# peterdavidfagan/mujoco_robot_environments

Measured on AMD Instinct MI355X. Metric: env steps/sec (whole node), RearrangementEnv batch=4096 at 1/2/4/8 MI355X, higher is better.
Workload: dtype f32

## Files before the change

### mujoco_robot_environments_amd/csrc/mre_api.cpp

```cpp
#include <hip/hip_runtime.h>
#include <chrono>

#include <cmath>
#include <cstdio>
#include <cstdlib>
#include <cstring>
#include <string>
#include <algorithm>
#include <vector>

#include "../../include/mre.h"
#include "mre_dev.h"
#include "mre_records.h"

using namespace mre;

extern "C" void mre_launch_step(const StepArgs* args, hipStream_t stream);
extern "C" void mre_launch_settle(const StepArgs* args, hipStream_t stream);
extern "C" void mre_launch_step_large(const StepArgs* args, hipStream_t stream);
extern "C" void mre_launch_step_newton(const StepArgs* args, hipStream_t stream);
extern "C" void mre_launch_settle_newton(const StepArgs* args, hipStream_t stream);
extern "C" void mre_launch_step_queue(const StepArgs* args, int nwaves, hipStream_t stream);
extern "C" void mre_launch_step_queue_newton(const StepArgs* args, int nwaves, hipStream_t stream);
extern "C" void mre_launch_step_queue_large(const StepArgs* args, int nwaves, hipStream_t stream);
// ... 474 lines not shown
      for (size_t left = ng; left > 0;) {
        size_t pick = ng;
        for (size_t g = 0; g < ng && pick == ng; g++)
          if (!done[g] && (e->groups[g].nout <= (a.nsteps <= 50 ? e->ring - 1 : 0) ||
                           hipEventQuery(e->groups[g].out[e->groups[g].head].ev_info) == hipSuccess)) pick = g;
        (void)hipGetLastError();
        if (pick == ng) {
          for (size_t g = 0; g < ng && pick == ng; g++) if (!done[g]) pick = g;
        }
        int rc = launch_group(e, e->groups[pick], a);
        if (rc) return rc;
        done[pick] = true; left--;
      }
      return MRE_OK;
    }
    DRAIN_PENDING(e);
  }
  hipEvent_t e0 = nullptr, e1 = nullptr;
  if (e->profiling) {
    if (e->events_used == e->events.size()) {
      hipEvent_t x, y;
      HIPCHK(hipEventCreate(&x)); HIPCHK(hipEventCreate(&y));
      e->events.emplace_back(x, y);
    }
    e0 = e->events[e->events_used].first; e1 = e->events[e->events_used].second;
    e->events_used++;
    HIPCHK(hipEventRecord(e0, e->stream));
  }
  const bool guarded = e->fallback && a.nsteps > 0 && (a.flags & F_NO_CONSTRAINTS) == 0;
  if (!guarded) {
    launch_compact(e, a, e->stream, settle);
    HIPCHK(hipGetLastError());
  } else {
    const size_t N = (size_t)e->N;
    if (e->d_large_stale) {
      HIPCHK(hipMemcpyAsync(e->d_large, e->h_large.data(), N, hipMemcpyHostToDevice, e->stream));
      HIPCHK(hipStreamSynchronize(e->stream));
      e->d_large_stale = false;
    }
    StepArgs ac = a;
    guard_args(e, ac);
    ac.want_large = 0;
    e->n_large = 0;
    for (size_t i = 0; i < N; i++) e->n_large += e->h_large[i];
    const bool run_large = e->n_large > 0;
    if (run_large) {
      HIPCHK(hipEventRecord(e->ev_fork, e->stream));
      HIPCHK(hipStreamWaitEvent(e->stream2, e->ev_fork, 0));
      StepArgs al = ac;
      al.want_large = 1;
      launch_large(e, al, e->stream2);
      HIPCHK(hipGetLastError());
      HIPCHK(hipEventRecord(e->ev_join, e->stream2));
    }
    launch_compact(e, ac, e->stream, settle);
    HIPCHK(hipGetLastError());
    if (run_large) HIPCHK(hipStreamWaitEvent(e->stream, e->ev_join, 0));
    HIPCHK(hipStreamSynchronize(e->stream));
    memcpy(e->h_info_last, e->h_launch_info, N * 16);
    int nrerun = 0;
    bool changed = false;
    for (size_t i = 0; i < N; i++) {
      const int* li = e->h_launch_info + 4 * i;
      e->h_rerun[i] = 0;
      if (li[0] < 0) continue;
      const int hw_ncon = li[1] & 0xFFFF, hw_nefc = li[2], hw_nrrow = li[3] & 0xFFFF, hw_npp = li[3] >> 16;
      if (!e->h_large[i]) {
        if (li[0] > 0) {
          e->h_rerun[i] = 1; e->h_large[i] = 1; nrerun++; changed = true; e->n_large++; e->n_promotions++;
        } else if (!e->compact_only && near_compact_caps(e, hw_ncon, hw_nefc, hw_nrrow, hw_npp)) {
          e->h_large[i] = 1; changed = true; e->n_large++; e->n_promotions++;
        }
      } else if (!e->large_only && li[0] == 0 && 8 * hw_ncon <= 5 * NCON_MAX && 8 * hw_nefc <= 5 * NEFC_MAX &&
                 8 * hw_nrrow <= 5 * compact_nrrow_max(e) && 8 * hw_npp <= 5 * NPP_MAX) {
        e->h_large[i] = 0; changed = true; e->n_large--; e->n_demotions++;
      }
    }
    if (!e->use_order) {
      int kmax = 0;
      for (size_t i = 0; i < N; i++)
        if (e->h_launch_info[4 * i] >= 0) { const int k = e->h_launch_info[4 * i + 1] >> 16; if (k > kmax) kmax = k; }
      if (kmax > 0) {
        int count[258] = {0};
        auto bucket = [&](size_t i) {
          const int k = e->h_launch_info[4 * i] < 0 ? 0 : (e->h_launch_info[4 * i + 1] >> 16);
          return (int)((long long)k * 255 / kmax);
        };
        for (size_t i = 0; i < N; i++) count[255 - bucket(i) + 1]++;
        for (int k = 1; k <= 256; k++) count[k] += count[k - 1];
        for (size_t i = 0; i < N; i++) e->h_auto_order[count[255 - bucket(i)]++] = (int)i;
        HIPCHK(hipMemcpyAsync(e->auto_order, e->h_auto_order, N * 4, hipMemcpyHostToDevice, e->stream));
        e->have_auto_order = true;
      } else {
        e->have_auto_order = false;
      }
    }
    if (nrerun > 0) {
      HIPCHK(hipMemcpyAsync(e->mask_r, e->h_rerun.data(), N, hipMemcpyHostToDevice, e->stream));
      mre_launch_restore_rows(e->mask_r, 0, e->N, e->qpos, e->sv_qpos, e->qvel, e->sv_qvel, e->qacc_ws, e->sv_qacc_ws,
                              e->qfine, e->sv_qfine, e->ctrl, e->sv_ctrl, e->nstep, e->sv_nstep, e->status,
                              e->sv_status, e->converged, e->sv_converged, nullptr, e->stream);
      StepArgs ar = a;
      ar.env_mask = e->mask_r; ar.launch_info = nullptr;
      launch_large(e, ar, e->stream);
      HIPCHK(hipGetLastError());
      e->n_reruns += nrerun;
    }
    if (changed) {
      HIPCHK(hipMemcpyAsync(e->d_large, e->h_large.data(), N, hipMemcpyHostToDevice, e->stream));
      HIPCHK(hipStreamSynchronize(e->stream));
    }
  }
  if (e1) HIPCHK(hipEventRecord(e1, e->stream));
  return MRE_OK;
}

namespace {
struct Blob {
  const unsigned char* p;
  size_t n;
  bool find(const char* name, uint32_t* code, uint32_t* count, uint64_t* off) const {
    uint32_t ne;
    memcpy(&ne, p + 8, 4);
    const unsigned char* t = p + 16;
    for (uint32_t k = 0; k < ne; k++, t += 48)
      if (strncmp((const char*)t, name, 32) == 0) {
        memcpy(code, t + 32, 4); memcpy(count, t + 36, 4); memcpy(off, t + 40, 8);
        return *off + (size_t)(*count) * (*code ? 8 : 4) <= n;
      }
    return false;
  }
  bool ints(const char* name, int* dst, int expect) const {
    uint32_t c, cnt; uint64_t off;
    if (!find(name, &c, &cnt, &off) || c != 0 || (int)cnt != expect) return false;
    memcpy(dst, p + off, 4 * (size_t)cnt);
    return true;
  }
  bool flts(const char* name, float* dst, int expect) const {
    uint32_t c, cnt; uint64_t off;
    if (!find(name, &c, &cnt, &off) || c != 1 || (int)cnt != expect) return false;
    for (uint32_t k = 0; k < cnt; k++) {
      double v;
      memcpy(&v, p + off + 8 * (size_t)k, 8);
      dst[k] = (float)v;
    }
    return true;
  }
};
}

#define RI(name, dst, n) if (!b.ints(name, (int*)(dst), n)) return fail(MRE_ERR_MODEL, std::string("model entry ") + name)
#define RF(name, dst, n) if (!b.flts(name, (float*)(dst), n)) return fail(MRE_ERR_MODEL, std::string("model entry ") + name)

static int build_model(const void* blob, size_t nbytes, DevModel& m) {
  if (nbytes < 16) return fail(MRE_ERR_MODEL, "blob too small");
  Blob b{(const unsigned char*)blob, nbytes};
  uint32_t magic;
  memcpy(&magic, b.p, 4);
  if (magic != 0x4D524542u) return fail(MRE_ERR_MODEL, "bad blob magic");
  memset(&m, 0, sizeof(m));
  int nbody, nv, nq, nM, ngeom, nsite, npair, neq, nprop, nu;
  RI("nbody", &nbody, 1); RI("nv", &nv, 1); RI("nq", &nq, 1); RI("nM", &nM, 1); RI("ngeom", &ngeom, 1);
  RI("nsite", &nsite, 1); RI("npair", &npair, 1); RI("neq", &neq, 1); RI("nprop", &nprop, 1);
  RI("nu", &nu, 1);
  if (nbody != NB || nv != NV || nq != NQ || ngeom != NG || nsite != NSITE || npair > NPAIR ||
      neq != NEQ || nprop != NPROP || nu != NU)
    return fail(MRE_ERR_MODEL, "scene dimensions differ from the compiled kernels");
  RI("body_parentid", m.body_parent, NB); RI("body_jnttype", m.body_jnttype, NB);
  RI("body_dofadr", m.body_dofadr, NB); RI("body_qposadr", m.body_qposadr, NB);
  RI("body_propid", m.body_propid, NB);
  RF("body_pos", m.body_pos, NB * 3); RF("body_quat", m.body_quat, NB * 4);
  RF("body_ipos", m.body_ipos, NB * 3); RF("body_iquat", m.body_iquat, NB * 4);
  RF("body_mass", m.body_mass, NB); RF("body_inertia", m.body_inertia, NB * 3);
  RF("body_invweight0", m.body_invweight0, NB * 2);
  RF("jnt_pos", m.jnt_pos, NB * 3); RF("jnt_axis", m.jnt_axis, NB * 3); RF("jnt_range", m.jnt_range, NB * 2);
  RF("jnt_stiffness", m.jnt_stiffness, NB); RF("jnt_springref", m.jnt_springref, NB);
  RF("jnt_solref", m.jnt_solref, NB * 2); RF("jnt_solimp", m.jnt_solimp, NB * 5);
  RI("jnt_limited", m.jnt_limited, NB);
  RI("dof_bodyid", m.dof_body, NV); RI("dof_parentid", m.dof_parent, NV); RI("dof_Madr", m.dof_Madr, NV);
  m.dof_Madr[NV] = nM;
  RF("dof_armature", m.dof_armature, NV); RF("dof_damping", m.dof_damping, NV);
  RF("dof_invweight0", m.dof_invweight0, NV); RF("qpos0", m.qpos0, NQ);
  RI("geom_type", m.geom_type, NG); RI("geom_bodyid", m.geom_body, NG); RI("geom_propid", m.geom_propid, NG);
  RF("geom_size", m.geom_size, NG * 3); RF("geom_pos", m.geom_pos, NG * 3);
  RF("geom_quat", m.geom_quat, NG * 4); RF("geom_rbound", m.geom_rbound, NG);
  {
    std::vector<int> pg(2 * npair);
    RI("pair_geom", pg.data(), 2 * npair);
    for (int k = 0; k < NPAIR; k++) { m.pair_g1[k] = -1; m.pair_g2[k] = -1; }
    for (int k = 0; k < npair; k++) { m.pair_g1[k] = pg[2 * k]; m.pair_g2[k] = pg[2 * k + 1]; }
  }
  RI("pair_single", m.pair_single, npair);
  RF("pair_friction", m.pair_friction, npair * 3); RF("pair_solref", m.pair_solref, npair * 2);
  RF("pair_solimp", m.pair_solimp, npair * 5); RF("pair_margin", m.pair_margin, npair);
  RF("pair_gap", m.pair_gap, npair);
  for (int k = 0; k < NPAIR; k++) {
    PairRec& r = m.pair_rec[k];
    memset(&r, 0, sizeof(r));
    r.g1 = m.pair_g1[k]; r.g2 = m.pair_g2[k];
    if (r.g1 < 0) { r.g2 = -1; r.b1 = r.b2 = 0; r.pid1 = r.pid2 = -1; continue; }
    if (r.g1 >= NG || r.g2 < 0 || r.g2 >= NG) return fail(MRE_ERR_MODEL, "pair table names a geom that does not exist");
    r.b1 = m.geom_body[r.g1]; r.b2 = m.geom_body[r.g2];
    r.pid1 = m.geom_propid[r.g1]; r.pid2 = m.geom_propid[r.g2];
    r.type1 = m.geom_type[r.g1]; r.single = (m.pair_single[k] & 0xFF) | (m.geom_type[r.g2] << 8);
    if (m.geom_type[r.g1] == 2 || (m.geom_type[r.g2] == 2 && m.geom_type[r.g1] != 1))
      return fail(MRE_ERR_MODEL, "cylinder pairs: only box (geom 1) - cylinder (geom 2) is implemented");
    for (int c = 0; c < 3; c++) { r.pos1[c] = m.geom_pos[r.g1][c]; r.pos2[c] = m.geom_pos[r.g2][c];
                                  r.size1[c] = m.geom_size[r.g1][c]; r.size2[c] = m.geom_size[r.g2][c]; }
    for (int c = 0; c < 4; c++) { r.quat1[c] = m.geom_quat[r.g1][c]; r.quat2[c] = m.geom_quat[r.g2][c]; }
    r.rb1 = m.geom_rbound[r.g1]; r.rb2 = m.geom_rbound[r.g2];
    r.margin = m.pair_margin[k]; r.gap = m.pair_gap[k];
  }
  RI("site_bodyid", m.site_body, NSITE); RF("site_pos", m.site_pos, NSITE * 3);
  RF("site_quat", m.site_quat, NSITE * 4);
  RI("eef_site", &m.eef_site, 1); RI("tcp_site", &m.tcp_site, 1);
  RI("eq_type", m.eq_type, NEQ); RI("eq_obj", m.eq_obj, NEQ * 2); RF("eq_data", m.eq_data, NEQ * 8);
  RF("eq_solref", m.eq_solref, NEQ * 2); RF("eq_solimp", m.eq_solimp, NEQ * 5);
  RI("ten_dof", m.ten_dof, 2); RF("ten_coef", m.ten_coef, 2);
  RI("act_dof", m.act_dof, NU); RF("act_ctrlrange", m.act_ctrlrange, NU * 2);
  RF("grip_gainprm", &m.grip_gainprm, 1); RF("grip_biasprm", m.grip_biasprm, 3);
  RF("grip_forcerange", m.grip_forcerange, 2);
  for (int a = 0; a < NU; a++) { m.act_gain[a] = 1.f; m.act_forcelimited[a] = 0; }
  { uint32_t c, cnt; uint64_t off;
    if (b.find("act_gainprm", &c, &cnt, &off)) {
      RF("act_gainprm", m.act_gain, NU); RF("act_biasprm", m.act_bias, NU * 3);
      RF("act_forcerange", m.act_forcerange, NU * 2); RI("act_forcelimited", m.act_forcelimited, NU);
    } }
  RF("opt_timestep", &m.timestep, 1); RF("opt_gravity", m.gravity, 3); RF("opt_impratio", &m.impratio, 1);
  RF("opt_tolerance", &m.tolerance, 1); RI("opt_iterations", &m.iterations, 1);
  m.solver = MRE_SOLVER_PGS;
  { uint32_t c, cnt; uint64_t off; if (b.find("opt_solver", &c, &cnt, &off)) RI("opt_solver", &m.solver, 1); }
  if (m.solver != MRE_SOLVER_PGS && m.solver != MRE_SOLVER_NEWTON) return fail(MRE_ERR_MODEL, "opt_solver must be 0 (PGS) or 2 (Newton)");
  { uint32_t c, cnt; uint64_t off; int cone = 1;
    if (b.find("opt_cone", &c, &cnt, &off)) RI("opt_cone", &cone, 1);
    if (cone != 0 && cone != 1) return fail(MRE_ERR_MODEL, "opt_cone must be 0 (pyramidal) or 1 (elliptic)");
    m.cone = cone; }
  RF("home_qpos", m.home_qpos, 7);
  float M0d[NV];
  RF("M0_diag", M0d, NV);

  for (int bb = 1; bb < NB; bb++) {
    bool ok = bb < NRB ? (m.body_jnttype[bb] == 1 && m.body_dofadr[bb] == bb - 1 && m.body_qposadr[bb] == bb - 1 &&
                          m.body_propid[bb] < 0 && m.body_parent[bb] < bb)
                       : (m.body_jnttype[bb] == 2 && m.body_dofadr[bb] == NRV + 6 * (bb - NRB) &&
                          m.body_qposadr[bb] == NRV + 7 * (bb - NRB) && m.body_propid[bb] == bb - NRB &&
                          m.body_parent[bb] == 0);
    if (!ok) return fail(MRE_ERR_MODEL, "body layout differs from the compiled kernels");
  }
  if (m.dof_Madr[NRV] != NMR) return fail(MRE_ERR_MODEL, "robot mass-matrix size differs");
  for (int a = 0; a < 7; a++)
    if (m.act_dof[a] != a) return fail(MRE_ERR_MODEL, "arm actuators must drive dofs 0..6");

  m.body_level[0] = 0;
  for (int bb = 1; bb < NB; bb++) m.body_level[bb] = m.body_level[m.body_parent[bb]] + 1;
  for (int bb = 0; bb < NB; bb++) {
    if (m.body_level[bb] > MAXCHAIN) return fail(MRE_ERR_MODEL, "tree deeper than MAXCHAIN");
    m.body_desc_mask[bb] = 0;
  }
  for (int c = 1; c < NB; c++)
    for (int a = c; a > 0; a = m.body_parent[a]) m.body_desc_mask[a] |= (1u << c);
  m.robot_mass = 0;
  for (int bb = 1; bb < NRB; bb++) {
    m.robot_mass += m.body_mass[bb];
    int chain[MAXCHAIN], n = 0;
    for (int d = m.body_dofadr[bb]; d >= 0; d = m.dof_parent[d]) {
      if (n >= MAXCHAIN) return fail(MRE_ERR_MODEL, "dof chain too long");
      chain[n++] = d;
    }
    m.chain_len[bb] = n;
    for (int k = 0; k < n; k++) m.chain_dof[bb][k] = chain[n - 1 - k];
  }
  for (int i = 0; i < NRV; i++) {
    int adr = m.dof_Madr[i];
    for (int j = i; j >= 0; j = m.dof_parent[j], adr++) { m.M_i[adr] = i; m.M_j[adr] = j; }
    if (adr != m.dof_Madr[i + 1]) return fail(MRE_ERR_MODEL, "dof_Madr inconsistent");
  }
  for (int i = 0; i < NRV; i++)
    if (m.dof_parent[i] != ROBOT_DOF_PARENT[i] || m.dof_Madr[i] != robot_dof_madr(i))
      return fail(MRE_ERR_MODEL, "robot dof tree differs from the one the kernels are unrolled for (mre_dev.h)");
  {
    int depth[NRV];
    m.sol_maxdepth = 0;
    for (int i = 0; i < NRV; i++) {
      depth[i] = m.dof_parent[i] < 0 ? 0 : depth[m.dof_parent[i]] + 1;
      m.sol_depth[i] = depth[i];
      if (depth[i] > m.sol_maxdepth) m.sol_maxdepth = depth[i];
    }
    m.sol_depth[NRV] = -1;
    for (int i = 0; i <= NRV; i++) {
      uint16_t desc[14], anc[8];
      for (auto& v : desc) v = 0xFFFF;
      for (auto& v : anc) v = 0xFFFF;
      if (i < NRV) {
        int nd = 0, na = 0;
        for (int c = NRV - 1; c > i; c--) {
          bool is_desc = false;
          for (int j = m.dof_parent[c]; j >= 0; j = m.dof_parent[j]) if (j == i) is_desc = true;
          if (!is_desc) continue;
          if (nd >= 14) return fail(MRE_ERR_MODEL, "solve table: too many descendants");
          desc[nd++] = (uint16_t)(c | ((m.dof_Madr[c] + depth[c] - depth[i]) << 8));
        }
        for (int a = m.dof_Madr[i] + 1; a < m.dof_Madr[i + 1]; a++) {
          if (na >= 8) return fail(MRE_ERR_MODEL, "solve table: too many ancestors");
          int j = i;
          for (int k = 0; k < a - m.dof_Madr[i]; k++) j = m.dof_parent[j];
          anc[na++] = (uint16_t)(j | (a << 8));
        }
      }
      for (int k = 0; k < 7; k++) m.sol_desc[i][k] = desc[2 * k] | ((uint32_t)desc[2 * k + 1] << 16);
      for (int k = 0; k < 4; k++) m.sol_anc[i][k] = anc[2 * k] | ((uint32_t)anc[2 * k + 1] << 16);
    }
  }
  for (int k = 0; k < NRV; k++) {
    int anc[MAXCHAIN + 1], n = 0;
    for (int j = m.dof_parent[k]; j >= 0; j = m.dof_parent[j]) anc[++n] = j;
    int cnt = 0;
    for (int p = 1; p <= n; p++)
      for (int q = p; q <= n; q++) {
        if (cnt >= MAXFAC) return fail(MRE_ERR_MODEL, "factor table overflow");
        m.fac_dst[k][cnt] = (uint8_t)(m.dof_Madr[anc[p]] + (q - p));
        m.fac_a[k][cnt] = (uint8_t)p;
        m.fac_b[k][cnt] = (uint8_t)q;
        cnt++;
      }
    m.fac_n[k] = cnt;
  }
  m.M0_diag_robot_sum = 0;
  for (int i = 0; i < NRV; i++) m.M0_diag_robot_sum += M0d[i];
  for (int p = 0; p < NPROP; p++) {
    m.park_pos[p][0] = 2.0f + 0.5f * p; m.park_pos[p][1] = 2.0f; m.park_pos[p][2] = -5.0f;
  }
  return MRE_OK;
}

extern "C" const char* mre_last_error(void) { return g_err.c_str(); }

static int create_buffers(mre_env* e, int num_envs, int device_id) {
  e->N = num_envs;
  e->device = device_id;
  HIPCHK(hipSetDevice(device_id));
  HIPCHK(hipStreamCreateWithFlags(&e->stream, hipStreamNonBlocking));
  const size_t N = (size_t)num_envs;
  HIPCHK(hipMalloc(&e->dM, sizeof(DevModel)));
  HIPCHK(hipMemcpy(e->dM, &e->hM, sizeof(DevModel), hipMemcpyHostToDevice));
  HIPCHK(hipMalloc(&e->qpos, N * NQP * 4)); HIPCHK(hipMalloc(&e->qvel, N * NVP * 4));
  HIPCHK(hipMalloc(&e->qacc_ws, N * NVP * 4)); HIPCHK(hipMalloc(&e->ctrl, N * NU * 4));
  HIPCHK(hipMalloc(&e->qfine, N * QFINE_ROW * 4)); HIPCHK(hipMalloc(&e->sv_qfine, N * QFINE_ROW * 4));
  HIPCHK(hipMemsetAsync(e->qfine, 0, N * QFINE_ROW * 4, e->stream));
  HIPCHK(hipMalloc(&e->nstep, N * 4)); HIPCHK(hipMalloc(&e->sv_nstep, N * 4));
  HIPCHK(hipMemsetAsync(e->nstep, 0, N * 4, e->stream));
  HIPCHK(hipMalloc(&e->nprops, N * 4)); HIPCHK(hipMalloc(&e->prop_size, N * NPROP * 3 * 4));
  HIPCHK(hipMalloc(&e->osc_target, N * 16 * 4)); HIPCHK(hipMalloc(&e->grip_closed, N));
  HIPCHK(hipMalloc(&e->converged, N)); HIPCHK(hipMalloc(&e->mask, N));
  HIPCHK(hipMalloc(&e->sites, N * 16 * 4));
  HIPCHK(hipMalloc(&e->status, N * 4)); HIPCHK(hipMalloc(&e->stats, N * 4 * 4));
  HIPCHK(hipMalloc(&e->order, N * 4)); HIPCHK(hipMalloc(&e->auto_order, N * 4));
  HIPCHK(hipHostMalloc((void**)&e->h_auto_order, N * 4, hipHostMallocDefault));
  HIPCHK(hipStreamCreateWithFlags(&e->stream2, hipStreamNonBlocking));
  HIPCHK(hipEventCreateWithFlags(&e->ev_fork, hipEventDisableTiming));
  HIPCHK(hipEventCreateWithFlags(&e->ev_join, hipEventDisableTiming));
  HIPCHK(hipMalloc(&e->d_large, N)); HIPCHK(hipMalloc(&e->mask_r, N));
  HIPCHK(hipMalloc(&e->sv_qpos, N * NQP * 4)); HIPCHK(hipMalloc(&e->sv_qvel, N * NVP * 4));
  HIPCHK(hipMalloc(&e->sv_qacc_ws, N * NVP * 4)); HIPCHK(hipMalloc(&e->sv_ctrl, N * NU * 4));
  HIPCHK(hipMalloc(&e->sv_status, N * 4));
  HIPCHK(hipMalloc(&e->sv_converged, N));
  HIPCHK(hipHostMalloc((void**)&e->h_launch_info, mre_env::RING * N * 16, hipHostMallocMapped | hipHostMallocCoherent));
  HIPCHK(hipHostGetDevicePointer((void**)&e->d_launch_info, e->h_launch_info, 0));
  memset(e->h_launch_info, 0xFF, mre_env::RING * N * 16);
  HIPCHK(hipHostMalloc((void**)&e->h_info_last, N * 16, hipHostMallocDefault));
  memset(e->h_info_last, 0xFF, N * 16);
  HIPCHK(hipHostMalloc((void**)&e->h_large_stage, mre_env::NSTAGE * N, hipHostMallocMapped | hipHostMallocCoherent));
  HIPCHK(hipHostGetDevicePointer((void**)&e->d_large_stage, e->h_large_stage, 0));
  memset(e->h_large_stage, 0, mre_env::NSTAGE * N);
  HIPCHK(hipMalloc(&e->d_pending, N));
  HIPCHK(hipMemsetAsync(e->d_pending, 0, N, e->stream));
  HIPCHK(hipMemsetAsync(e->d_large, 0, N, e->stream));
  e->h_large.assign(N, 0); e->h_rerun.assign(N, 0);
  {
    int ng = 4, min_envs = 512;
    if (const char* g = getenv("MRE_GROUPS")) ng = atoi(g);
    if (const char* g = getenv("MRE_GROUP_MIN")) min_envs = atoi(g);
    if (ng < 1) ng = 1;
    if (ng > 8) ng = 8;
    if (const char* r = getenv("MRE_RING")) { e->ring = atoi(r); if (e->ring < 2) e->ring = 2; if (e->ring > mre_env::RING) e->ring = mre_env::RING; }
    while (ng > 1 && num_envs < min_envs * ng) ng--;
    HIPCHK(hipHostMalloc((void**)&e->h_grp_order, mre_env::NSTAGE * N * 4, hipHostMallocMapped | hipHostMallocCoherent));
    HIPCHK(hipHostGetDevicePointer((void**)&e->d_grp_order, e->h_grp_order, 0));
    for (int k = 0; k < mre_env::NSTAGE; k++)
      for (int i = 0; i < num_envs; i++) e->h_grp_order[(size_t)k * N + i] = i;
    HIPCHK(hipEventCreateWithFlags(&e->ev_main, hipEventDisableTiming));
    e->groups.resize(ng);
    {
      auto& Q = e->qgroup;
      Q.lo = 0; Q.n = num_envs;
      HIPCHK(hipHostMalloc((void**)&e->h_qgrp_order, mre_env::NSTAGE * N * 4, hipHostMallocMapped | hipHostMallocCoherent));
      Q.h_order = e->h_qgrp_order;
      HIPCHK(hipHostGetDevicePointer((void**)&Q.d_order, Q.h_order, 0));
      for (int k = 0; k < mre_env::NSTAGE; k++)
        for (int i = 0; i < num_envs; i++) Q.h_order[(size_t)k * N + i] = i;
      {
        int least = 0, greatest = 0;
        HIPCHK(hipDeviceGetStreamPriorityRange(&least, &greatest));
        HIPCHK(hipStreamCreateWithPriority(&Q.st, hipStreamNonBlocking, least));
        HIPCHK(hipStreamCreateWithPriority(&Q.st2, hipStreamNonBlocking, greatest));
      }
      HIPCHK(hipEventCreateWithFlags(&Q.ev_fork, hipEventDisableTiming));
      HIPCHK(hipEventCreateWithFlags(&Q.ev_join, hipEventDisableTiming));
      for (auto& o : Q.out) HIPCHK(hipEventCreateWithFlags(&o.ev_info, hipEventDisableTiming));
      if (const char* q = getenv("MRE_QUEUE")) e->queue_ok = atoi(q) != 0;
      if (const char* q = getenv("MRE_QUEUE_TICKS")) { const int v = atoi(q); if (v >= 2 && v <= QUEUE_TICKS_MAX) e->queue_ticks = v; }
      if (e->queue_run_ticks > e->queue_ticks) e->queue_run_ticks = e->queue_ticks;
      hipDeviceProp_t prop;
      HIPCHK(hipGetDeviceProperties(&prop, e->device));
      {
        const int a_ = mre_queue_waves_per_cu(), b_ = mre_queue_waves_per_cu_newton();
        e->queue_waves = prop.multiProcessorCount * (a_ < b_ ? a_ : b_);
      }
      if (const char* q = getenv("MRE_QUEUE_WAVES")) { const int v = atoi(q); if (v > 0) e->queue_waves = v; }
      if (const char* q = getenv("MRE_QUEUE_SHARDS")) { const int v = atoi(q); if (v >= 1 && v <= QUEUE_SHARDS_MAX) e->queue_shards = v; }
      if (const char* q = getenv("MRE_QUEUE_MIN_TICKS")) { const int v = atoi(q); if (v >= 2) e->queue_min_ticks = v; }
      if (const char* q = getenv("MRE_QUEUE_TAIL_MIN")) { const float v = (float)atof(q); if (v > 0.f) e->queue_tail_min = v; }
      if (const char* q = getenv("MRE_QUEUE_TEST_SERIAL")) e->queue_test_serial = atoi(q) != 0;
      if (const char* q = getenv("MRE_QUEUE_SPARE_LARGE")) { const int v = atoi(q); if (v >= 0) e->queue_spare_large = v; }
      e->queue_large_waves_max = 2 * prop.multiProcessorCount;
      if (const char* q = getenv("MRE_QUEUE_LSHARDS")) { const int v = atoi(q); if (v >= 1 && v <= QUEUE_LSHARDS_MAX) e->queue_lshards = v; }
      HIPCHK(hipMalloc(&e->q_ws, ((2 * (size_t)(QUEUE_SHARDS_MAX + QUEUE_LSHARDS_MAX) * QUEUE_TICKS_MAX + 16 + 4 * N +
                                   (size_t)QUEUE_TICKS_MAX * (2 * N + QUEUE_SHARDS_MAX + QUEUE_LSHARDS_MAX)) * 4 + 15) / 16 * 16));
      HIPCHK(hipMalloc(&e->q_gen, 64));
      HIPCHK(hipMemsetAsync(e->q_gen, 0, 64, e->stream));
      HIPCHK(hipHostMalloc((void**)&e->h_qlist, (size_t)(mre_env::RING + 1) * (N + 32) * 4, hipHostMallocDefault));
      HIPCHK(hipHostMalloc((void**)&e->h_q_err, 64, hipHostMallocMapped | hipHostMallocCoherent));
      *e->h_q_err = 0;
    }
    for (int g = 0; g < ng; g++) {
      auto& G = e->groups[g];
      G.h_order = e->h_grp_order; G.d_order = e->d_grp_order;
      G.lo = (int)((long long)num_envs * g / ng);
      G.n = (int)((long long)num_envs * (g + 1) / ng) - G.lo;
      int pr = 0;
      {
        int least = 0, greatest = 0;
        HIPCHK(hipDeviceGetStreamPriorityRange(&least, &greatest));
        const char* gp = getenv("MRE_GROUP_PRIORITY");
        if (!(gp && atoi(gp) == 0)) { pr = greatest + g; if (pr > least) pr = least; }
        if (const char* map = getenv("MRE_GROUP_PRIO_MAP")) {
          if ((int)strlen(map) > g && map[g] >= '0' && map[g] <= '9') { pr = greatest + (map[g] - '0'); if (pr > least) pr = least; }
        }
      }
      HIPCHK(hipStreamCreateWithPriority(&G.st, hipStreamNonBlocking, pr));
      HIPCHK(hipStreamCreateWithPriority(&G.st2, hipStreamNonBlocking, pr));
      HIPCHK(hipEventCreateWithFlags(&G.ev_fork, hipEventDisableTiming));
      HIPCHK(hipEventCreateWithFlags(&G.ev_join, hipEventDisableTiming));
      for (auto& o : G.out) HIPCHK(hipEventCreateWithFlags(&o.ev_info, hipEventDisableTiming));
    }
  }
  if (const char* fb = getenv("MRE_NO_FALLBACK")) e->fallback = atoi(fb) == 0;
  if (const char* fl = getenv("MRE_FORCE_LARGE")) {
    if (atoi(fl) != 0) {
      e->h_large.assign(N, 1); e->n_large = num_envs;
      HIPCHK(hipMemsetAsync(e->d_large, 1, N, e->stream));
    }
  }
  HIPCHK(hipMemsetAsync(e->status, 0, N * 4, e->stream)); HIPCHK(hipMemsetAsync(e->stats, 0, N * 16, e->stream));
  HIPCHK(hipMemsetAsync(e->grip_closed, 0, N, e->stream)); HIPCHK(hipMemsetAsync(e->osc_target, 0, N * 64, e->stream));
  HIPCHK(hipMemsetAsync(e->sites, 0, N * 64, e->stream));
  std::vector<int> np(N, NPROP);
  std::vector<float> ps(N * NPROP * 3, 0.0155f);
  HIPCHK(hipMemcpy(e->nprops, np.data(), N * 4, hipMemcpyHostToDevice));
  HIPCHK(hipMemcpy(e->prop_size, ps.data(), ps.size() * 4, hipMemcpyHostToDevice));
  e->osc = OscConfig{350.f, 20.f, 500.f, 100.f, 200.f, 30.f, {0.f, -0.785f, 0.f, -2.356f, 0.f, 1.571f, 0.785f},
                     5e-3f, 68e-3f, 0};
  HIPCHK(hipMalloc(&e->d_osc, sizeof(OscConfig)));
  HIPCHK(hipMemcpy(e->d_osc, &e->osc, sizeof(OscConfig), hipMemcpyHostToDevice));
  HIPCHK(hipStreamSynchronize(e->stream));
  int rc = mre_reset(e, nullptr);
  if (rc != MRE_OK) return rc;
  return mre_sync(e);
}

extern "C" int mre_create(const void* blob, size_t nbytes, int num_envs, int device_id, mre_env** out) {
  if (!blob || !out || num_envs <= 0) return fail(MRE_ERR_ARG, "mre_create: bad argument");
  *out = nullptr;
  mre_env* e = new mre_env();
  int rc = build_model(blob, nbytes, e->hM);
  if (rc != MRE_OK) { delete e; return rc; }
// ... 1087 lines not shown
```

### mujoco_robot_environments_amd/csrc/mre_dev.h

```cpp
#pragma once
#include <stdint.h>

namespace mre {

constexpr int NB = 20;
constexpr int NRB = 16;
constexpr int GRIP_BODY0 = 8;
constexpr int NV = 39;
constexpr int NRV = 15;
constexpr int NQ = 43;
constexpr int NQP = 44;
constexpr int TRACE_W = 88;
constexpr int TRACE_QVEL = 48;
constexpr int NVP = 40;
constexpr int NU = 8;
constexpr int QFINE = 32;
constexpr int QFINE_ROW = 96;
constexpr int QFINE_CUBE_Q = 32;
constexpr int QFINE_CUBE_V = 60;
static_assert(QFINE_CUBE_Q + 7 * 4 == QFINE_CUBE_V && QFINE_CUBE_V + 6 * 4 <= QFINE_ROW, "qfine row layout");
constexpr int NPROP = 4;
constexpr int NG = 20;
constexpr int PROP_GEOM0 = 12;
constexpr int NPAIR = 128;
constexpr int NMR = 96;
constexpr int NSITE = 2;
constexpr int NEQ = 3;
constexpr int CONTACT_EXPORT = 32;
constexpr int MAXCHAIN = 9;
constexpr int MAXFAC = 45;
constexpr int ROBOT_DOF_PARENT[NRV] = {-1, 0, 1, 2, 3, 4, 5, 6, 7, 6, 9, 6, 11, 6, 13};
constexpr int robot_dof_depth(int i) { return ROBOT_DOF_PARENT[i] < 0 ? 0 : 1 + robot_dof_depth(ROBOT_DOF_PARENT[i]); }
constexpr int robot_dof_madr(int i) { return i == 0 ? 0 : robot_dof_madr(i - 1) + robot_dof_depth(i - 1) + 1; }
constexpr int robot_dof_anc(int i, int k) {
  int j = ROBOT_DOF_PARENT[i];
  for (int t = 0; t < k && j >= 0; t++) j = ROBOT_DOF_PARENT[j];
  return j;
}
static_assert(robot_dof_madr(NRV) == NMR, "robot mass-matrix size");

#if defined(MRE_LARGE_CAPS) && defined(MRE_NEWTON)
constexpr int NCON_MAX = 48;
constexpr int NEFC_MAX = 160;
constexpr int NRROW_MAX = 100;
constexpr int NPP_MAX = 16;
constexpr int MAXBLK = 58;
#elif defined(MRE_LARGE_CAPS)
constexpr int NCON_MAX = 44;
constexpr int NEFC_MAX = 148;
constexpr int NRROW_MAX = 83;
constexpr int NPP_MAX = 16;
constexpr int MAXBLK = 52;
#elif defined(MRE_NEWTON)
constexpr int NCON_MAX = 32;
constexpr int NEFC_MAX = 112;
constexpr int NRROW_MAX = 69;
constexpr int NPP_MAX = 8;
constexpr int MAXBLK = 40;
#else
constexpr int NCON_MAX = 32;
constexpr int NEFC_MAX = 112;
constexpr int NRROW_MAX = 62;
constexpr int NPP_MAX = 8;
constexpr int MAXBLK = 40;
#endif
constexpr int NRROW_MAX_COMPACT_PGS = 62, NRROW_MAX_COMPACT_NEWTON = 69;
#if !defined(MRE_LARGE_CAPS)
static_assert(NRROW_MAX ==
#ifdef MRE_NEWTON
              NRROW_MAX_COMPACT_NEWTON,
#else
              NRROW_MAX_COMPACT_PGS,
#endif
              "host-side copy of the compact robot-row capacity");
#endif
static_assert(NEFC_MAX <= 256 && NRROW_MAX < 127 && NPP_MAX <= 16 && MAXBLK >= 8 + NCON_MAX,
              "capacities must fit the block descriptor fields (mre_solver.h)");

struct alignas(16) PairRec {
  int g1, g2, b1, b2;
  int pid1, pid2, type1, single;
  float pos1[3], rb1;
  float pos2[3], rb2;
  float quat1[4], quat2[4];
  float size1[3], margin;
  float size2[3], gap;
};
static_assert(sizeof(PairRec) == 128, "PairRec is eight 16-byte words");

struct DevModel {
  int body_parent[NB], body_level[NB], body_jnttype[NB], body_dofadr[NB], body_qposadr[NB];
  int body_propid[NB];
  unsigned body_desc_mask[NB];
  int chain_len[NB];
  int chain_dof[NB][MAXCHAIN];
  float body_pos[NB][3], body_quat[NB][4], body_ipos[NB][3], body_iquat[NB][4];
  float body_mass[NB], body_inertia[NB][3], body_invweight0[NB][2];
  float jnt_pos[NB][3], jnt_axis[NB][3], jnt_range[NB][2], jnt_stiffness[NB], jnt_springref[NB];
  float jnt_solref[NB][2], jnt_solimp[NB][5];
  int jnt_limited[NB];
  int dof_body[NV], dof_parent[NV], dof_Madr[NV + 1];
  float dof_armature[NV], dof_damping[NV], dof_invweight0[NV], qpos0[NQP];
  int M_i[NMR], M_j[NMR];
  int fac_n[NRV];
  uint8_t fac_dst[NRV][MAXFAC], fac_a[NRV][MAXFAC], fac_b[NRV][MAXFAC];
  int sol_depth[NRV + 1], sol_maxdepth;
  uint32_t sol_desc[NRV + 1][7], sol_anc[NRV + 1][4];
  float robot_mass;
  float M0_diag_robot_sum;
  int geom_type[NG], geom_body[NG], geom_propid[NG];
  float geom_size[NG][3], geom_pos[NG][3], geom_quat[NG][4], geom_rbound[NG];
  int pair_g1[NPAIR], pair_g2[NPAIR], pair_single[NPAIR];
  float pair_friction[NPAIR][3], pair_solref[NPAIR][2], pair_solimp[NPAIR][5];
  float pair_margin[NPAIR], pair_gap[NPAIR];
  PairRec pair_rec[NPAIR];
  int site_body[NSITE];
  float site_pos[NSITE][3], site_quat[NSITE][4];
  int eef_site, tcp_site;
  int eq_type[NEQ], eq_obj[NEQ][2];
  float eq_data[NEQ][8], eq_solref[NEQ][2], eq_solimp[NEQ][5];
  int ten_dof[2];
  float ten_coef[2];
  int act_dof[NU];
  float act_ctrlrange[NU][2], grip_gainprm, grip_biasprm[3], grip_forcerange[2];
  float act_gain[NU], act_bias[NU][3], act_forcerange[NU][2];
  int act_forcelimited[NU];
  float timestep, gravity[3], impratio, tolerance;
  int iterations;
  int solver;
  int cone;
  float home_qpos[7];
  float park_pos[NPROP][3];
};

struct OscConfig {
  float kp_pos, kd_pos, kp_ori, kd_ori, kp_null, kd_null;
  float null_q[7];
  float pos_thresh, ori_thresh;
  int pinv_always;
};

enum StepFlags : unsigned { F_NO_CONSTRAINTS = 1u, F_FREEZE_ROBOT = 2u, F_CONV_CONTINUE = 4u, F_CONV_OPEN = 8u,
                            F_OSC_EVAL = 16u, F_DETECT = 32u, F_SETTLE_EXIT = 64u };
enum CtrlMode : int { CTRL_HELD = 0, CTRL_SEQ = 1, CTRL_OSC = 2 };

struct StepArgs {
  const DevModel* M;
  int N;
  float* qpos;
  float* qvel;
  float* qacc_ws;
  float* qfine;
  float* ctrl;
  const float* ctrl_seq;
  int seq_stride;
  const int* nprops;
  const float* prop_size;
  int nsteps, control_steps, mode;
  unsigned flags;
  const OscConfig* osc;
  int osc_stride;
  const float* osc_target;
  const uint8_t* grip_closed;
  uint8_t* converged;
  float* sites;
  uint32_t* status;
  int* nstep;
  int* stats;
  float* trace;
  int trace_nenv, trace_max, trace_base;
  const uint8_t* env_mask;
  const int* env_order;
  float* geoms;
  float* contacts;
  int* settle_steps;
  int min_settle_steps;
  const uint8_t* large;
  int want_large;
  float *sv_qpos, *sv_qvel, *sv_qacc_ws, *sv_qfine, *sv_ctrl;
  int* sv_nstep;
  uint32_t* sv_status;
  uint8_t* sv_converged;
  int* launch_info;
  uint8_t* pending;
  int* q_head;
  int* q_tail;
  int* q_buf;
  int* q_acc;
  int* q_done;
  int* q_started;
  const int* q_gen;
  int q_gen_expect;
  int q_wait;
  int* q_err;
  int q_nticks, q_shards, q_cap, q_stride;
  int q_lshards, q_capl;
};
constexpr int QUEUE_TICKS_MAX = 256;
constexpr int QUEUE_SHARDS_MAX = 32;
constexpr int QUEUE_LSHARDS_MAX = 16;

struct SearchArgs {
  const DevModel* M;
  int N;
  float* qpos;
  const int* nprops;
  const float* prop_size;
  const uint8_t* env_mask;
  const long long* env_ids;
  long long env_id_offset;
  unsigned long long seed;
  const int* prop;
  int fixed_prop;
  const double* bounds;
  double shared_bounds[6];
  const int* tick_base;
  long long tick0;
  int max_attempts;
  int yaw_mode;
  double fixed_quat[4];
  float max_dist;
  int commit;
  float* qfine;
  double* pose;
  int* attempts;
};

struct SortArgs {
  const DevModel* M;
  int N;
  const float* qpos;
  const int* nprops;
  const double* zones;
  double place_z;
  int* which;
  double* pick;
  double* bounds;
};

struct RenderArgs {
  int N, height, width;
  const float* geoms;
  const int* nprops;
  const uint8_t* prop_rgb;
  float geom_rgb[NG][3];
  float cam_pos[3], cam_mat[9];
  float fy;
  float light_pos[3];
  float ambient, head_diffuse, light_diffuse;
  float checker[2][3], checker_size;
  float zfar;
  uint8_t* rgb;
  float* depth;
  uint8_t* seg;
  const uint8_t* env_mask;
  int g0, g1;
  const float* bg_depth;
  const uint8_t* bg_rgb;
  const uint8_t* bg_seg;
};

}
```

### mujoco_robot_environments_amd/csrc/mre_kernels.hip

```cpp
#include <hip/hip_runtime.h>

#include "mre_dev.h"
#include "mre_math.h"
#include "mre_collide.h"

namespace mre {
using ModelP = MRE_MODEL_PTR(DevModel);
#if defined(MRE_PHASE_STAMPS) && MRE_PHASE_STAMPS >= 4
__shared__ unsigned long long dbg_acc[4];
#endif

struct OscSm {
  float J[6][7], M[7][7], MiJt[7][6], Li[6][6], Lam[6][6], V[6][6], Jbar[7][6];
  float ep[3], eo[3], F[6], LF[6], tn[7], Jbt[6], xd[6], w[6];
};

struct alignas(8) Blk {
  uint16_t row0;
  uint8_t type, nrows;
  uint8_t rslot;
  uint8_t pa, pb;
  uint8_t primary : 4;
  uint8_t bslot : 4;
};

constexpr int TAB_BYTES = 8 * (MAXBLK * 5 + 1) + 4 * 48;
constexpr int FRAME_BYTES = (int)sizeof(OscSm) > 4 * (NB * 16) ? (int)sizeof(OscSm) : 4 * (NB * 16);
constexpr int R1_MIN = TAB_BYTES - FRAME_BYTES > 0 ? TAB_BYTES - FRAME_BYTES : 4;
constexpr int MD_LD = 17;

struct Sm {
  float qpos[NQP], qvel[NVP], qlo[QFINE], ctrl[NU];
  float qfrc_smooth[NVP], qacc_smooth[NVP], qacc[NVP], qfrc_bias[NVP], qfrc_con[NVP];
  union {
    struct { float xpos[NB][3], xquat[NB][4], xmat[NB][9]; };
    OscSm osc;
#ifdef MRE_NEWTON
    struct { float nw_Ma[NVP], nw_grad[NVP], nw_search[NVP], nw_Mv[NVP]; };
#endif
  };
#ifndef MRE_NEWTON
  char tab_room[R1_MIN];
#endif
  float cdof[NRV][6];
  union {
    struct { float con_pos[NCON_MAX][3], con_frame[NCON_MAX][9], con_dist[NCON_MAX]; };
#ifdef MRE_NEWTON
    struct { float jar[NEFC_MAX], frc[NEFC_MAX], jv[NEFC_MAX]; };
#else
    struct { float jar[NEFC_MAX], frc[NEFC_MAX], pyr_f[4 * NCON_MAX]; };
#endif
  };
  float com_robot[3];
  float site_xpos[NSITE][3], site_xmat[1][9];
#ifdef MRE_NEWTON
  float qM[NMR];
#else
  float qM[NMR], qLD[NMR], qLDinv[NRV + 1];
#endif
  float prop_mass[NPROP], prop_inertia[NPROP][3], prop_size[NPROP][3];
  union { float scratch[64]; int iscr[64]; };
  float osc_tgt[16];
  int nprops;
  int ncon, nefc, nl, nrrow, npp, overflow, solver_iters;
  int finger_contact;
  uint8_t con_pair[NCON_MAX], con_rslot[NCON_MAX], con_bslot[NCON_MAX], con_b1[NCON_MAX], con_b2[NCON_MAX];
  uint16_t lim_info[NRV + 1];
  union {
    float JpA[3 * NCON_MAX][6];
    struct {
      float cinert[NB][10], crb[NRB][10], gP[NRB - GRIP_BODY0][6], gC[NRB - GRIP_BODY0][6];
      double gpose[NRB - GRIP_BODY0][7];
    };
  };
  float JpB[3 * NPP_MAX][6];
  union {
    float Jr[NRROW_MAX][NRV];
    struct {
      float cdof_dot[NV][6], cvel[NB][6], cfrc[NB][6];
      alignas(8) double gI[NRB - GRIP_BODY0][10];
      double gS[NRB - GRIP_BODY0][6];
    };
  };
#ifdef MRE_NEWTON
  float efc_R[NEFC_MAX], efc_aref[NEFC_MAX];
  float frc_r[NRROW_MAX];
  float con_fric[NCON_MAX];
  float hc[NCON_MAX][6];
  float Md[NRV][MD_LD];
  alignas(8) float W[NV * (NV + 1) / 2];
  uint8_t rstate[NEFC_MAX];
  uint8_t clist[NPROP][NCON_MAX];
  uint8_t ccount[NPROP], cpl_robot, cpl_cubes;
  alignas(8) uint16_t jdesc[NEFC_MAX][4];
  float zrow[24];
#else
  float Br[NRROW_MAX][NRV];
  alignas(16) float blkrec[MAXBLK][16];
  Blk blk[MAXBLK];
  uint8_t sched[MAXBLK][8];
#endif
  uint16_t hdr[NEFC_MAX];

  int nblk, nsched;
};

#if defined(MRE_LARGE_CAPS)
static_assert(sizeof(Sm) <= 27136, "large-capacity Sm must fit 6 workgroups per CU");
#else
static_assert(sizeof(Sm) <= 20480, "compact Sm must fit 8 workgroups per CU");
#endif

#ifdef MRE_NEWTON
MRE_DEV float* mh_store(Sm& s) { return &s.JpA[0][0]; }
static_assert(sizeof(((Sm*)0)->JpA) >= sizeof(float) * NMR, "M - h dF/dv fits the head of the constraint block");
#else
MRE_DEV float* mh_store(Sm& s) { return s.qLD; }
#endif

struct BodyRegs {
  float anchor[3], axis[3], xipos[3], ximat[9];
};

MRE_DEV double robot_q(const Sm& s, int d) { return (double)s.qpos[d] + (double)s.qlo[d]; }
MRE_DEV double robot_v(const Sm& s, int d) { return (double)s.qvel[d] + (double)s.qlo[QFINE / 2 + d]; }

MRE_DEV bool body_is_active(ModelP M, const Sm& s, int b) {
  int p = M->body_propid[b];
  return p < 0 || p < s.nprops;
}

MRE_DEV void sincos_poly_d(double x, double& sn, double& cs) {
  const double z = x * x;
  double ps = -1.0 / 1307674368000.0;
  ps = ps * z + 1.0 / 6227020800.0;
  ps = ps * z - 1.0 / 39916800.0;
  ps = ps * z + 1.0 / 362880.0;
  ps = ps * z - 1.0 / 5040.0;
  ps = ps * z + 1.0 / 120.0;
  ps = ps * z - 1.0 / 6.0;
  sn = x + x * (z * ps);
  double pc = 1.0 / 20922789888000.0;
  pc = pc * z - 1.0 / 87178291200.0;
  pc = pc * z + 1.0 / 479001600.0;
  pc = pc * z - 1.0 / 3628800.0;
  pc = pc * z + 1.0 / 40320.0;
  pc = pc * z - 1.0 / 720.0;
  pc = pc * z + 1.0 / 24.0;
  pc = pc * z - 0.5;
  cs = 1.0 + z * pc;
}
MRE_DEV void dq_mul(double* r, const double* a, const double* b) {
  const double w = a[0] * b[0] - a[1] * b[1] - a[2] * b[2] - a[3] * b[3];
  const double x = a[0] * b[1] + a[1] * b[0] + a[2] * b[3] - a[3] * b[2];
  const double y = a[0] * b[2] - a[1] * b[3] + a[2] * b[0] + a[3] * b[1];
  const double z = a[0] * b[3] + a[1] * b[2] - a[2] * b[1] + a[3] * b[0];
  r[0] = w; r[1] = x; r[2] = y; r[3] = z;
}
MRE_DEV void dq_rot(double* r, const double* q, const double* v) {
  const double ux = q[1], uy = q[2], uz = q[3], w = q[0];
  const double cx = uy * v[2] - uz * v[1], cy = uz * v[0] - ux * v[2], cz = ux * v[1] - uy * v[0];
  const double dx = uy * cz - uz * cy, dy = uz * cx - ux * cz, dz = ux * cy - uy * cx;
  r[0] = v[0] + 2.0 * (w * cx + dx); r[1] = v[1] + 2.0 * (w * cy + dy); r[2] = v[2] + 2.0 * (w * cz + dz);
}
MRE_DEV void hinge_local_d(ModelP M, const Sm& s, int b, double* p, double* q) {
  double q0[4], ql[4], ax[3], jp[3], t0[3], t1[3];
  for (int k = 0; k < 4; k++) q0[k] = (double)M->body_quat[b][k];
  for (int k = 0; k < 3; k++) { ax[k] = (double)M->jnt_axis[b][k]; jp[k] = (double)M->jnt_pos[b][k]; }
  const int qa = M->body_qposadr[b];
  double s4, c4;
  sincos_poly_d(0.25 * (robot_q(s, qa) - (double)M->qpos0[qa]), s4, c4);
  const double sn = 2.0 * s4 * c4, cs = 1.0 - 2.0 * s4 * s4;
  ql[0] = cs; ql[1] = ax[0] * sn; ql[2] = ax[1] * sn; ql[3] = ax[2] * sn;
  dq_mul(q, q0, ql);
  const double n = rsq64(q[0] * q[0] + q[1] * q[1] + q[2] * q[2] + q[3] * q[3]);
  for (int k = 0; k < 4; k++) q[k] *= n;
  dq_rot(t0, q0, jp);
  dq_rot(t1, q, jp);
  for (int k = 0; k < 3; k++) p[k] = (double)M->body_pos[b][k] + t0[k] - t1[k];
}
template <int CTRL>
MRE_DEV double dpp_row_d(double v, double fill) {
  const long long b = __builtin_bit_cast(long long, v), f = __builtin_bit_cast(long long, fill);
  const int lo = __builtin_amdgcn_update_dpp((int)(f & 0xFFFFFFFFll), (int)(b & 0xFFFFFFFFll), CTRL, 0xF, 0xF, false);
  const int hi = __builtin_amdgcn_update_dpp((int)(f >> 32), (int)(b >> 32), CTRL, 0xF, 0xF, false);
  return __builtin_bit_cast(double, ((long long)hi << 32) | (long long)(unsigned)lo);
}
MRE_DEV double readlane_d(double v, int lane) {
  const long long b = __builtin_bit_cast(long long, v);
  const int lo = __builtin_amdgcn_readlane((int)(b & 0xFFFFFFFFll), lane), hi = __builtin_amdgcn_readlane((int)(b >> 32), lane);
  return __builtin_bit_cast(double, ((long long)hi << 32) | (long long)(unsigned)lo);
}
MRE_DEV void dq2mat(double* m, const double* q) {
  const double w = q[0], x = q[1], y = q[2], z = q[3];
  m[0] = w * w + x * x - y * y - z * z; m[1] = 2 * (x * y - w * z); m[2] = 2 * (x * z + w * y);
  m[3] = 2 * (x * y + w * z); m[4] = w * w - x * x + y * y - z * z; m[5] = 2 * (y * z - w * x);
  m[6] = 2 * (x * z - w * y); m[7] = 2 * (y * z + w * x); m[8] = w * w - x * x - y * y + z * z;
}
MRE_DEV double dpp_shr1_d(double v) {
  const long long b = __builtin_bit_cast(long long, v);
  const int lo = __builtin_amdgcn_update_dpp(0, (int)(b & 0xFFFFFFFFll), 0x111, 0xF, 0xF, false);
  const int hi = __builtin_amdgcn_update_dpp(0, (int)(b >> 32), 0x111, 0xF, 0xF, false);
  return __builtin_bit_cast(double, ((long long)hi << 32) | (long long)(unsigned)lo);
}
MRE_DEV double dpp_shl1_d(double v) {
  const long long b = __builtin_bit_cast(long long, v);
  const int lo = __builtin_amdgcn_update_dpp(0, (int)(b & 0xFFFFFFFFll), 0x101, 0xF, 0xF, false);
  const int hi = __builtin_amdgcn_update_dpp(0, (int)(b >> 32), 0x101, 0xF, 0xF, false);
  return __builtin_bit_cast(double, ((long long)hi << 32) | (long long)(unsigned)lo);
}

struct Frame { float p[3], q[4], m[9]; };

MRE_DEV float dpp_shr(float v, float fill, int sh) {
  int r;
  const int vi = __builtin_bit_cast(int, v), fi = __builtin_bit_cast(int, fill);
  if (sh == 1) r = __builtin_amdgcn_update_dpp(fi, vi, 0x111, 0xF, 0xF, false);
  else if (sh == 2) r = __builtin_amdgcn_update_dpp(fi, vi, 0x112, 0xF, 0xF, false);
  else r = __builtin_amdgcn_update_dpp(fi, vi, 0x114, 0xF, 0xF, false);
  return __builtin_bit_cast(float, r);
}
template <int CTRL>
MRE_DEV void chain_step_d(double (&q)[4], double (&p)[3]) {
  double aq[4], ap[3], nq[4], t[3];
  aq[0] = dpp_row_d<CTRL>(q[0], 1.0);
#pragma unroll
  for (int c = 1; c < 4; c++) aq[c] = dpp_row_d<CTRL>(q[c], 0.0);
#pragma unroll
  for (int c = 0; c < 3; c++) ap[c] = dpp_row_d<CTRL>(p[c], 0.0);
  dq_mul(nq, aq, q);
  dq_rot(t, aq, p);
#pragma unroll
  for (int c = 0; c < 4; c++) q[c] = nq[c];
#pragma unroll
  for (int c = 0; c < 3; c++) p[c] = ap[c] + t[c];
}
template <bool WRITEBACK>
MRE_DEV void kinematics(ModelP M, Sm& s, int l, BodyRegs& br) {
  constexpr int LINK7 = GRIP_BODY0 - 1;
  const bool arm = l >= 1 && l <= LINK7, fin = l >= GRIP_BODY0 && l < NRB;
  double q[4] = {1.0, 0.0, 0.0, 0.0}, p[3] = {0.0, 0.0, 0.0};
  if (arm || fin) hinge_local_d(M, s, l, p, q);
  {
    double pp[3], pq[4];
#pragma unroll
    for (int k = 0; k < 3; k++) pp[k] = dpp_shr1_d(p[k]);
#pragma unroll
    for (int k = 0; k < 4; k++) pq[k] = dpp_shr1_d(q[k]);
    if (fin) {
      if (M->body_parent[l] >= GRIP_BODY0) {
        double t[3], q2[4];
        dq_rot(t, pq, p);
#pragma unroll
        for (int k = 0; k < 3; k++) p[k] = pp[k] + t[k];
        dq_mul(q2, pq, q);
#pragma unroll
        for (int k = 0; k < 4; k++) q[k] = q2[k];
      }
#pragma unroll
      for (int k = 0; k < 3; k++) s.gpose[l - GRIP_BODY0][k] = p[k];
#pragma unroll
      for (int k = 0; k < 4; k++) s.gpose[l - GRIP_BODY0][3 + k] = q[k];
    }
  }
  double wq[4], wp[3];
#pragma unroll
  for (int k = 0; k < 4; k++) wq[k] = arm ? q[k] : (k == 0 ? 1.0 : 0.0);
#pragma unroll
  for (int k = 0; k < 3; k++) wp[k] = arm ? p[k] : 0.0;
  chain_step_d<0x111>(wq, wp);
  chain_step_d<0x112>(wq, wp);
  chain_step_d<0x114>(wq, wp);
  {
    double q7[4], p7[3];
#pragma unroll
    for (int k = 0; k < 4; k++) q7[k] = readlane_d(wq[k], LINK7);
#pragma unroll
    for (int k = 0; k < 3; k++) p7[k] = readlane_d(wp[k], LINK7);
    if (fin) {
      double t[3];
      dq_rot(t, q7, p);
      dq_mul(wq, q7, q);
#pragma unroll
      for (int k = 0; k < 3; k++) wp[k] = p7[k] + t[k];
    }
  }
  Frame mine;
  v3zero(br.anchor); v3zero(br.axis);
  v3zero(br.xipos);
  const int b = l < NB ? l : 0;
  if (arm || fin) {
    const double n = rsq64(wq[0] * wq[0] + wq[1] * wq[1] + wq[2] * wq[2] + wq[3] * wq[3]);
#pragma unroll
    for (int k = 0; k < 4; k++) wq[k] *= n;
    double Rm[9], t[3], qi[4];
    dq2mat(Rm, wq);
#pragma unroll
    for (int k = 0; k < 4; k++) mine.q[k] = (float)wq[k];
#pragma unroll
    for (int k = 0; k < 3; k++) mine.p[k] = (float)wp[k];
#pragma unroll
    for (int k = 0; k < 9; k++) mine.m[k] = (float)Rm[k];
    const double jp[3] = {(double)M->jnt_pos[b][0], (double)M->jnt_pos[b][1], (double)M->jnt_pos[b][2]};
    const double ax[3] = {(double)M->jnt_axis[b][0], (double)M->jnt_axis[b][1], (double)M->jnt_axis[b][2]};
    const double ip[3] = {(double)M->body_ipos[b][0], (double)M->body_ipos[b][1], (double)M->body_ipos[b][2]};
    const double iq[4] = {(double)M->body_iquat[b][0], (double)M->body_iquat[b][1], (double)M->body_iquat[b][2], (double)M->body_iquat[b][3]};
#pragma unroll
    for (int r = 0; r < 3; r++) {
      br.anchor[r] = (float)(wp[r] + Rm[3 * r] * jp[0] + Rm[3 * r + 1] * jp[1] + Rm[3 * r + 2] * jp[2]);
      br.axis[r] = (float)(Rm[3 * r] * ax[0] + Rm[3 * r + 1] * ax[1] + Rm[3 * r + 2] * ax[2]);
      br.xipos[r] = (float)(wp[r] + Rm[3 * r] * ip[0] + Rm[3 * r + 1] * ip[1] + Rm[3 * r + 2] * ip[2]);
    }
    dq_mul(qi, wq, iq);
    dq2mat(Rm, qi);
#pragma unroll
    for (int k = 0; k < 9; k++) br.ximat[k] = (float)Rm[k];
    (void)t;
  }
  if (l >= NRB && l < NB) {
    const int qa = M->body_qposadr[b];
    v3copy(mine.p, &s.qpos[qa]);
    for (int k = 0; k < 4; k++) mine.q[k] = s.qpos[qa + 3 + k];
    const float n2 = mine.q[0] * mine.q[0] + mine.q[1] * mine.q[1] + mine.q[2] * mine.q[2] + mine.q[3] * mine.q[3];
    qnormalize(mine.q);
    if (WRITEBACK && fabsf(n2 - 1.f) > 1e-5f) for (int k = 0; k < 4; k++) s.qpos[qa + 3 + k] = mine.q[k];
    q2mat(mine.m, mine.q);
    v3copy(br.anchor, mine.p);
    br.axis[0] = 0.f; br.axis[1] = 0.f; br.axis[2] = 1.f;
  }
  if (l == 0) {
    v3zero(mine.p);
    mine.q[0] = 1.f; mine.q[1] = mine.q[2] = mine.q[3] = 0.f;
    q2mat(mine.m, mine.q);
    q2mat(br.ximat, mine.q);
  }
  if (l < NB) {
    v3copy(s.xpos[b], mine.p);
    for (int k = 0; k < 4; k++) s.xquat[b][k] = mine.q[k];
    for (int k = 0; k < 9; k++) s.xmat[b][k] = mine.m[k];
    if (l >= NRB) {
      float tmp[3], qi[4];
      m3mulv(tmp, mine.m, M->body_ipos[b]);
      v3add(br.xipos, mine.p, tmp);
      qmul(qi, mine.q, M->body_iquat[b]);
      q2mat(br.ximat, qi);
    }
  }
  MRE_SYNC();
  if (l < NSITE) {
    const int b = M->site_body[l];
    float tmp[3], q[4];
    m3mulv(tmp, s.xmat[b], M->site_pos[l]);
    v3add(s.site_xpos[l], s.xpos[b], tmp);
    qmul(q, s.xquat[b], M->site_quat[l]);
    if (l == M->eef_site) q2mat(s.site_xmat[0], q);
  }
}

MRE_DEV void com_pos(ModelP M, Sm& s, int l, const BodyRegs& br) {
  const bool robot = (l >= 1 && l < NRB);
  float mass = 0.f;
  if (l < NB) mass = (M->body_propid[l] >= 0) ? s.prop_mass[M->body_propid[l]] : M->body_mass[l];
  float c0 = robot ? mass * br.xipos[0] : 0.f;
  float c1 = robot ? mass * br.xipos[1] : 0.f;
  float c2 = robot ? mass * br.xipos[2] : 0.f;
  wave_sum3(c0, c1, c2);
  const float inv = 1.0f / M->robot_mass;
  float com[3] = {c0 * inv, c1 * inv, c2 * inv};
  if (l == 0) v3copy(s.com_robot, com);
  if (l >= 1 && l < NB) {
    const int b = l, pid = M->body_propid[b];
    if (pid >= 0) v3copy(com, br.xipos);
    float inertia[3];
    if (pid >= 0) v3copy(inertia, s.prop_inertia[pid]); else v3copy(inertia, M->body_inertia[b]);
    float dif[3], tmp[9];
    v3sub(dif, br.xipos, com);
    const float* mat = br.ximat;
#pragma unroll
    for (int r = 0; r < 3; r++)
#pragma unroll
      for (int c = 0; c < 3; c++)
        tmp[3 * r + c] = mat[3 * r] * inertia[0] * mat[3 * c] + mat[3 * r + 1] * inertia[1] * mat[3 * c + 1] +
                         mat[3 * r + 2] * inertia[2] * mat[3 * c + 2];
    float* ci = s.cinert[b];
    ci[0] = tmp[0] + mass * (dif[1] * dif[1] + dif[2] * dif[2]);
    ci[1] = tmp[4] + mass * (dif[0] * dif[0] + dif[2] * dif[2]);
    ci[2] = tmp[8] + mass * (dif[0] * dif[0] + dif[1] * dif[1]);
    ci[3] = tmp[1] - mass * dif[0] * dif[1];
    ci[4] = tmp[2] - mass * dif[0] * dif[2];
    ci[5] = tmp[5] - mass * dif[1] * dif[2];
    ci[6] = mass * dif[0]; ci[7] = mass * dif[1]; ci[8] = mass * dif[2]; ci[9] = mass;
    const int da = M->body_dofadr[b];
    float off[3];
    v3sub(off, com, br.anchor);
    if (pid < 0) {
      v3copy(s.cdof[da], br.axis);
      v3cross(s.cdof[da] + 3, br.axis, off);
    }
  }
  if (l == 0) for (int k = 0; k < 10; k++) s.cinert[0][k] = 0.f;
}

MRE_PHASE_FN void position_stage(ModelP M, Sm& s, int l) {
  MRE_DBG_T0();
  BodyRegs br;
  kinematics<true>(M, s, l, br);
  MRE_DBG_STAMP(5, 0);
  com_pos(M, s, l, br);
  MRE_SYNC();
  MRE_DBG_STAMP(5, 1);
}
MRE_PHASE_FN void kinematics_only(ModelP M, Sm& s, int l) {
  BodyRegs br;
  kinematics<false>(M, s, l, br);
  MRE_SYNC();
}

MRE_DEV void prop_cdof(const Sm& s, int b, int j, float* c) {
  c[0] = c[1] = c[2] = c[3] = c[4] = c[5] = 0.f;
  if (j < 3) {
    c[3 + j] = 1.f;
  } else {
    const int k = j - 3;
    c[0] = s.xmat[b][k]; c[1] = s.xmat[b][3 + k]; c[2] = s.xmat[b][6 + k];
  }
}

MRE_DEV void inert_about_d(ModelP M, int c, const double* p, const double* q, const double* O, double* ci) {
  double ip[3] = {(double)M->body_ipos[c][0], (double)M->body_ipos[c][1], (double)M->body_ipos[c][2]}, t[3], qi[4];
  double iq[4] = {(double)M->body_iquat[c][0], (double)M->body_iquat[c][1], (double)M->body_iquat[c][2], (double)M->body_iquat[c][3]};
  dq_rot(t, q, ip);
  const double d[3] = {p[0] + t[0] - O[0], p[1] + t[1] - O[1], p[2] + t[2] - O[2]};
  dq_mul(qi, q, iq);
  double R[9];
  {
    const double w = qi[0], x = qi[1], y = qi[2], z = qi[3];
    R[0] = w * w + x * x - y * y - z * z; R[1] = 2 * (x * y - w * z); R[2] = 2 * (x * z + w * y);
    R[3] = 2 * (x * y + w * z); R[4] = w * w - x * x + y * y - z * z; R[5] = 2 * (y * z - w * x);
    R[6] = 2 * (x * z - w * y); R[7] = 2 * (y * z + w * x); R[8] = w * w - x * x - y * y + z * z;
  }
  const double m = (double)M->body_mass[c];
  const double in[3] = {(double)M->body_inertia[c][0], (double)M->body_inertia[c][1], (double)M->body_inertia[c][2]};
  double T[9];
  for (int r = 0; r < 3; r++)
    for (int k = 0; k < 3; k++)
      T[3 * r + k] = R[3 * r] * in[0] * R[3 * k] + R[3 * r + 1] * in[1] * R[3 * k + 1] + R[3 * r + 2] * in[2] * R[3 * k + 2];
  ci[0] += T[0] + m * (d[1] * d[1] + d[2] * d[2]);
  ci[1] += T[4] + m * (d[0] * d[0] + d[2] * d[2]);
  ci[2] += T[8] + m * (d[0] * d[0] + d[1] * d[1]);
  ci[3] += T[1] - m * d[0] * d[1];
  ci[4] += T[2] - m * d[0] * d[2];
  ci[5] += T[5] - m * d[1] * d[2];
  ci[6] += m * d[0]; ci[7] += m * d[1]; ci[8] += m * d[2]; ci[9] += m;
}

MRE_PHASE_FN void gripper_local(ModelP M, Sm& s, int l) {
  const bool fin = l >= GRIP_BODY0 && l < NRB;
  const int b = fin ? l : GRIP_BODY0;
  const double* pose = s.gpose[b - GRIP_BODY0];
  const double p[3] = {pose[0], pose[1], pose[2]}, q[4] = {pose[3], pose[4], pose[5], pose[6]};
  const int ts = M->tcp_site;
  const double O[3] = {(double)M->site_pos[ts][0], (double)M->site_pos[ts][1], (double)M->site_pos[ts][2]};
  double ci[10] = {0, 0, 0, 0, 0, 0, 0, 0, 0, 0};
  if (fin) inert_about_d(M, b, p, q, O, ci);
  double up[10];
#pragma unroll
  for (int k = 0; k < 10; k++) up[k] = dpp_shl1_d(ci[k]);
  if (fin) {
#pragma unroll
    for (int k = 0; k < 10; k++) s.gI[b - GRIP_BODY0][k] = ci[k];
    if (M->body_parent[b] < GRIP_BODY0 && b + 1 < NRB && M->body_parent[b + 1] == b) {
#pragma unroll
      for (int k = 0; k < 10; k++) ci[k] += up[k];
    }
    double ax[3] = {(double)M->jnt_axis[b][0], (double)M->jnt_axis[b][1], (double)M->jnt_axis[b][2]};
    double jp[3] = {(double)M->jnt_pos[b][0], (double)M->jnt_pos[b][1], (double)M->jnt_pos[b][2]};
    double u[3], a[3];
    dq_rot(u, q, ax);
    dq_rot(a, q, jp);
    const double r[3] = {O[0] - p[0] - a[0], O[1] - p[1] - a[1], O[2] - p[2] - a[2]};
    const double cd[6] = {u[0], u[1], u[2], u[1] * r[2] - u[2] * r[1], u[2] * r[0] - u[0] * r[2], u[0] * r[1] - u[1] * r[0]};
    double P[6];
    P[0] = ci[0] * cd[0] + ci[3] * cd[1] + ci[4] * cd[2] - ci[8] * cd[4] + ci[7] * cd[5];
    P[1] = ci[3] * cd[0] + ci[1] * cd[1] + ci[5] * cd[2] + ci[8] * cd[3] - ci[6] * cd[5];
    P[2] = ci[4] * cd[0] + ci[5] * cd[1] + ci[2] * cd[2] - ci[7] * cd[3] + ci[6] * cd[4];
    P[3] = ci[8] * cd[1] - ci[7] * cd[2] + ci[9] * cd[3];
    P[4] = ci[6] * cd[2] - ci[8] * cd[0] + ci[9] * cd[4];
    P[5] = ci[7] * cd[0] - ci[6] * cd[1] + ci[9] * cd[5];
    for (int k = 0; k < 6; k++) { s.gC[b - GRIP_BODY0][k] = (float)cd[k]; s.gP[b - GRIP_BODY0][k] = (float)P[k]; s.gS[b - GRIP_BODY0][k] = cd[k]; }
  }
  MRE_SYNC();
}

MRE_DEV void connect_side_d(ModelP M, const Sm& s, int b, const float* a, double sign, double* x,
                            double (*vec)[3]) {
  const double* pose = s.gpose[b - GRIP_BODY0];
  const double al[3] = {(double)a[0], (double)a[1], (double)a[2]};
  double t[3];
  dq_rot(t, pose + 3, al);
  for (int k = 0; k < 3; k++) x[k] = pose[k] + t[k];
  const int par = M->body_parent[b];
  for (int m = 0; m < 2; m++) {
    vec[m][0] = vec[m][1] = vec[m][2] = 0.0;
    const int c = m == 0 ? b : par;
    if (c < GRIP_BODY0) break;
    const double* cp = s.gpose[c - GRIP_BODY0];
    const double ax[3] = {(double)M->jnt_axis[c][0], (double)M->jnt_axis[c][1], (double)M->jnt_axis[c][2]};
    const double jp[3] = {(double)M->jnt_pos[c][0], (double)M->jnt_pos[c][1], (double)M->jnt_pos[c][2]};
    double u[3], ja[3];
    dq_rot(u, cp + 3, ax);
    dq_rot(ja, cp + 3, jp);
    const double r[3] = {x[0] - cp[0] - ja[0], x[1] - cp[1] - ja[1], x[2] - cp[2] - ja[2]};
    vec[m][0] = sign * (u[1] * r[2] - u[2] * r[1]);
    vec[m][1] = sign * (u[2] * r[0] - u[0] * r[2]);
    vec[m][2] = sign * (u[0] * r[1] - u[1] * r[0]);
  }
}

MRE_PHASE_FN void connect_rows_local(ModelP M, Sm& s, int l) {
  if (l < 2 && M->eq_type[l] == 0) {
    double x1[3], x2[3], v1[2][3], v2[2][3];
    connect_side_d(M, s, M->eq_obj[l][0], M->eq_data[l], 1.0, x1, v1);
    connect_side_d(M, s, M->eq_obj[l][1], M->eq_data[l] + 3, -1.0, x2, v2);
    float* o = &s.qfrc_con[16 * l];
    for (int k = 0; k < 3; k++) {
      o[k] = (float)(x1[k] - x2[k]);
      o[4 + k] = (float)v1[0][k]; o[7 + k] = (float)v1[1][k];
      o[10 + k] = (float)v2[0][k]; o[13 + k] = (float)v2[1][k];
    }
  }
  MRE_SYNC();
}

constexpr bool robot_tree_is_chain_plus_two_body_fingers() {
  for (int d = 0; d < NRV; d++) {
    const int b = d + 1;
    const int want = b < GRIP_BODY0 ? d - 1 : ((b & 1) ? d - 1 : GRIP_BODY0 - 2);
    if (ROBOT_DOF_PARENT[d] != want) return false;
  }
  return true;
}
static_assert(GRIP_BODY0 % 2 == 0 && NRB == 16 && robot_tree_is_chain_plus_two_body_fingers(),
              "tree_prefix / tree_suffix / the prefix kinematics are written for this body tree");
template <int CTRL>
MRE_DEV float dpp_row(float v) {
  return __builtin_bit_cast(float, __builtin_amdgcn_update_dpp(0, __builtin_bit_cast(int, v), CTRL, 0xF, 0xF, false));
}
template <int N>
MRE_DEV void tree_prefix(float (&x)[N], int l) {
  constexpr int LINK7 = GRIP_BODY0 - 1;
  float own[N], par[N];
#pragma unroll
  for (int c = 0; c < N; c++) { own[c] = x[c]; par[c] = dpp_row<0x111>(x[c]); }
#pragma unroll
  for (int c = 0; c < N; c++) x[c] += dpp_row<0x111>(x[c]);
#pragma unroll
  for (int c = 0; c < N; c++) x[c] += dpp_row<0x112>(x[c]);
#pragma unroll
  for (int c = 0; c < N; c++) x[c] += dpp_row<0x114>(x[c]);
  const bool finger = l >= GRIP_BODY0 && l < NRB, leaf = (l & 1) != 0;
#pragma unroll
  for (int c = 0; c < N; c++) {
    const float p7 = __builtin_bit_cast(float, __builtin_amdgcn_readlane(__builtin_bit_cast(int, x[c]), LINK7));
    x[c] = finger ? (p7 + (leaf ? par[c] : 0.f)) + own[c] : x[c];
  }
}
template <int N>
MRE_DEV void tree_suffix(float (&x)[N], int l) {
  float own[N], nxt[N];
#pragma unroll
  for (int c = 0; c < N; c++) { own[c] = x[c]; nxt[c] = dpp_row<0x101>(x[c]); }
#pragma unroll
  for (int c = 0; c < N; c++) x[c] += dpp_row<0x101>(x[c]);
#pragma unroll
  for (int c = 0; c < N; c++) x[c] += dpp_row<0x102>(x[c]);
#pragma unroll
  for (int c = 0; c < N; c++) x[c] += dpp_row<0x104>(x[c]);
#pragma unroll
  for (int c = 0; c < N; c++) x[c] += dpp_row<0x108>(x[c]);
  const bool finger = l >= GRIP_BODY0 && l < NRB, leaf = (l & 1) != 0;
#pragma unroll
  for (int c = 0; c < N; c++) x[c] = finger ? (leaf ? own[c] : own[c] + nxt[c]) : x[c];
}

MRE_DEV void crb_mass_matrix(ModelP M, Sm& s, int l) {
  {
    float acc[10];
#pragma unroll
    for (int k = 0; k < 10; k++) acc[k] = (l >= 1 && l < NRB) ? s.cinert[l][k] : 0.f;
    tree_suffix(acc, l);
    if (l >= 1 && l < NRB) {
#pragma unroll
      for (int k = 0; k < 10; k++) s.crb[l][k] = acc[k];
    }
  }
  MRE_SYNC();
  for (int e = l; e < NMR; e += 64) {
    const int i = M->M_i[e], j = M->M_j[e];
    float v;
    if (i >= GRIP_BODY0 - 1) {
      const int root = GRIP_BODY0 - 1;
      float cj[6];
      if (j >= GRIP_BODY0 - 1) {
        for (int k = 0; k < 6; k++) cj[k] = s.gC[j - (GRIP_BODY0 - 1)][k];
      } else {
        float off[3], t[3], lin[3];
        v3sub(off, s.site_xpos[M->tcp_site], s.com_robot);
        v3cross(t, s.cdof[j], off);
        v3add(lin, s.cdof[j] + 3, t);
        m3tmulv(cj, s.xmat[root], s.cdof[j]);
        m3tmulv(cj + 3, s.xmat[root], lin);
      }
      v = dot6(cj, s.gP[i - (GRIP_BODY0 - 1)]);
    } else {
      float buf[6];
      mul_inert_vec(buf, s.crb[M->dof_body[i]], s.cdof[i]);
      v = dot6(s.cdof[j], buf);
    }
    if (i == j) v += M->dof_armature[i];
    s.qM[e] = v;
  }
}

typedef const __attribute__((address_space(3))) float* lds_cfloat_p;
template <int I, int K, class F>
MRE_DEV void solve_regs_back(float (&x)[NRV], const F& LD, float xi) {
  constexpr int j = robot_dof_anc(I, K);
  if constexpr (j >= 0) {
    constexpr int adr = robot_dof_madr(I) + 1 + K;
    x[j] -= LD[adr] * xi;
    solve_regs_back<I, K + 1, F>(x, LD, xi);
  }
}
template <int I, class F>
MRE_DEV void solve_regs_back_rows(float (&x)[NRV], const F& LD) {
  solve_regs_back<I, 0, F>(x, LD, x[I]);
  __builtin_amdgcn_sched_barrier(0);
  if constexpr (I > 0) solve_regs_back_rows<I - 1, F>(x, LD);
}
template <int I, int K, class F>
MRE_DEV void solve_regs_fwd(float (&x)[NRV], const F& LD, float& xi) {
  constexpr int j = robot_dof_anc(I, K);
  if constexpr (j >= 0) {
    constexpr int adr = robot_dof_madr(I) + 1 + K;
    xi -= LD[adr] * x[j];
    solve_regs_fwd<I, K + 1, F>(x, LD, xi);
  }
}
template <int I, class F>
MRE_DEV void solve_regs_fwd_rows(float (&x)[NRV], const F& LD) {
  float xi = x[I];
  solve_regs_fwd<I, 0, F>(x, LD, xi);
  x[I] = xi;
  __builtin_amdgcn_sched_barrier(0);
  if constexpr (I + 1 < NRV) solve_regs_fwd_rows<I + 1, F>(x, LD);
}
MRE_DEV void solve_robot_regs(const float* LD_, const float* dinv_, float (&x)[NRV]) {
  lds_cfloat_p LD = (lds_cfloat_p)LD_;
  lds_cfloat_p dinv = (lds_cfloat_p)dinv_;
  asm volatile("" : "+v"(LD), "+v"(dinv));
  solve_regs_back_rows<NRV - 1, lds_cfloat_p>(x, LD);
#pragma unroll
  for (int i = 0; i < NRV; i++) x[i] *= dinv[i];
  solve_regs_fwd_rows<0, lds_cfloat_p>(x, LD);
}

typedef __attribute__((address_space(3))) float* lds_float_p;
template <int K, int P, int Q>
MRE_DEV void factor_regs_upd(float (&A)[NMR], float tmp) {
  if constexpr (Q <= robot_dof_depth(K)) {
    constexpr int i = robot_dof_anc(K, P - 1);
    constexpr int dst = robot_dof_madr(i) + (Q - P), src = robot_dof_madr(K) + Q;
    A[dst] -= tmp * A[src];
    factor_regs_upd<K, P, Q + 1>(A, tmp);
  }
}
template <int K, int P>
MRE_DEV void factor_regs_anc(float (&A)[NMR], float inv) {
  if constexpr (P <= robot_dof_depth(K)) {
    constexpr int kp = robot_dof_madr(K) + P;
    const float tmp = A[kp] * inv;
    factor_regs_upd<K, P, P>(A, tmp);
    A[kp] = tmp;
    factor_regs_anc<K, P + 1>(A, inv);
  }
}
template <int K, class D>
MRE_DEV void factor_regs_rows(float (&A)[NMR], D& dinv) {
  constexpr int kk = robot_dof_madr(K);
  const float inv = 1.0f / A[kk];
  dinv[K] = inv;
  factor_regs_anc<K, 1>(A, inv);
  if constexpr (K > 0) factor_regs_rows<K - 1, D>(A, dinv);
}
MRE_DEV void factor_robot_regs(const float* src_, float* LD_, float* dinv_) {
  lds_cfloat_p src = (lds_cfloat_p)src_;
  lds_float_p LD = (lds_float_p)LD_, dinv = (lds_float_p)dinv_;
  asm volatile("" : "+v"(src), "+v"(LD), "+v"(dinv));
  float A[NMR];
#pragma unroll
  for (int e = 0; e < NMR; e++) A[e] = src[e];
  factor_regs_rows<NRV - 1, lds_float_p>(A, dinv);
#pragma unroll
  for (int e = 0; e < NMR; e++) LD[e] = A[e];
  MRE_SYNC();
}

MRE_DEV void solve_robot_one(const float* LD, const float* dinv, float* xv, int l) {
  float x[NRV];
#pragma unroll
  for (int i = 0; i < NRV; i++) x[i] = xv[i];
  solve_robot_regs(LD, dinv, x);
  MRE_SYNC();
  float mine = 0.f;
#pragma unroll
  for (int i = 0; i < NRV; i++) mine = (l == i) ? x[i] : mine;
  if (l < NRV) xv[l] = mine;
  MRE_SYNC();
}

MRE_DEV void factor_solve_robot(const float* src_, float* xv, int l) {
  lds_cfloat_p src = (lds_cfloat_p)src_;
  asm volatile("" : "+v"(src));
  float A[NMR], dv[NRV], x[NRV];
#pragma unroll
  for (int e = 0; e < NMR; e++) A[e] = src[e];
#pragma unroll
  for (int i = 0; i < NRV; i++) x[i] = xv[i];
  factor_regs_rows<NRV - 1, float[NRV]>(A, dv);
  solve_regs_back_rows<NRV - 1, float[NMR]>(x, A);
#pragma unroll
  for (int i = 0; i < NRV; i++) x[i] *= dv[i];
  solve_regs_fwd_rows<0, float[NMR]>(x, A);
  MRE_SYNC();
  float mine = 0.f;
#pragma unroll
  for (int i = 0; i < NRV; i++) mine = (l == i) ? x[i] : mine;
  if (l < NRV) xv[l] = mine;
  MRE_SYNC();
}

}
#include "mre_solver.h"
#ifdef MRE_NEWTON
#include "mre_newton.h"
#endif
#include "mre_osc.h"
namespace mre {

MRE_PHASE_FN void velocity_stage(ModelP M, Sm& s, int l) {
  constexpr int LINK7 = GRIP_BODY0 - 1;
  const bool rob = l >= 1 && l < NRB;
  float cd[6] = {0.f, 0.f, 0.f, 0.f, 0.f, 0.f}, qv = 0.f;
  if (rob) {
#pragma unroll
    for (int t = 0; t < 6; t++) cd[t] = s.cdof[l - 1][t];
    qv = s.qvel[l - 1];
  }
  float cv[6];
#pragma unroll
  for (int t = 0; t < 6; t++) cv[t] = cd[t] * qv;
  tree_prefix(cv, l);
  float pv[6];
  {
    const bool off7 = l >= GRIP_BODY0 && l < NRB && (l & 1) == 0;
#pragma unroll
    for (int t = 0; t < 6; t++) {
      const float below = dpp_row<0x111>(cv[t]);
      const float v7 = __builtin_bit_cast(float, __builtin_amdgcn_readlane(__builtin_bit_cast(int, cv[t]), LINK7));
      pv[t] = off7 ? v7 : below;
    }
  }
  float cdd[6], ca[6];
  cross_motion(cdd, pv, cd);
#pragma unroll
  for (int t = 0; t < 6; t++) ca[t] = cdd[t] * qv;
  tree_prefix(ca, l);
  if (l >= NRB && l < NB) {
    const int b = l;
#pragma unroll
    for (int t = 0; t < 6; t++) { cv[t] = 0.f; ca[t] = 0.f; }
    const int da = M->body_dofadr[b];
#pragma unroll
    for (int j = 0; j < 3; j++) cv[3 + j] += s.qvel[da + j];
    float cdot[3][6];
#pragma unroll
    for (int j = 3; j < 6; j++) {
      float c6[6];
      prop_cdof(s, b, j, c6);
      cross_motion(cdot[j - 3], cv, c6);
    }
#pragma unroll
    for (int j = 3; j < 6; j++) {
      float c6[6];
      prop_cdof(s, b, j, c6);
      const float q = s.qvel[da + j];
      for (int t = 0; t < 3; t++) cv[t] += c6[t] * q;
      for (int t = 0; t < 6; t++) ca[t] += cdot[j - 3][t] * q;
    }
  }
  float f[6] = {0.f, 0.f, 0.f, 0.f, 0.f, 0.f};
  if (l >= 1 && l < NB) {
    const int b = l;
    ca[3] -= M->gravity[0]; ca[4] -= M->gravity[1]; ca[5] -= M->gravity[2];
    if (l == LINK7) {
#pragma unroll
      for (int t = 0; t < 6; t++) { s.scratch[t] = cv[t]; s.scratch[6 + t] = ca[t]; }
    }
    float t0[6], t1[6], g[6];
    mul_inert_vec(t0, s.cinert[b], cv);
    cross_force(t1, cv, t0);
    mul_inert_vec(g, s.cinert[b], ca);
#pragma unroll
    for (int t = 0; t < 6; t++) f[t] = g[t] + t1[t];
    if (b >= NRB) {
#pragma unroll
      for (int t = 0; t < 6; t++) s.cfrc[b][t] = f[t];
    }
  }
  tree_suffix(f, l);
  float tot[6];
#pragma unroll
  for (int t = 0; t < 6; t++) tot[t] = dpp_row<0x101>(f[t]);
  MRE_SYNC();
  if (l < NV) {
    const int b = M->dof_body[l];
    float c6[6];
    if (b < NRB) {
#pragma unroll
      for (int t = 0; t < 6; t++) c6[t] = s.cdof[l][t];
    } else {
#pragma unroll
      for (int t = 0; t < 6; t++) tot[t] = s.cfrc[b][t];
      prop_cdof(s, b, l - M->body_dofadr[b], c6);
    }
    const bool act = body_is_active(M, s, b);
    s.qfrc_bias[l] = act ? dot6(c6, tot) : 0.f;
  }
}

MRE_DEV void dcross3(double* r, const double* a, const double* b) {
  const double x = a[1] * b[2] - a[2] * b[1], y = a[2] * b[0] - a[0] * b[2], z = a[0] * b[1] - a[1] * b[0];
  r[0] = x; r[1] = y; r[2] = z;
}
MRE_DEV void dcross_motion(double* r, const double* vel, const double* v) {
  double a[3], b[3];
  dcross3(r, vel, v);
  dcross3(a, vel, v + 3);
  dcross3(b, vel + 3, v);
  for (int k = 0; k < 3; k++) r[3 + k] = a[k] + b[k];
}
MRE_DEV void dcross_force(double* r, const double* vel, const double* f) {
  double a[3], b[3];
  dcross3(a, vel, f);
  dcross3(b, vel + 3, f + 3);
  for (int k = 0; k < 3; k++) r[k] = a[k] + b[k];
  dcross3(r + 3, vel, f + 3);
}
MRE_DEV void dmul_inert_vec(double* r, const double* i, const double* v) {
  r[0] = i[0] * v[0] + i[3] * v[1] + i[4] * v[2] - i[8] * v[4] + i[7] * v[5];
  r[1] = i[3] * v[0] + i[1] * v[1] + i[5] * v[2] + i[8] * v[3] - i[6] * v[5];
  r[2] = i[4] * v[0] + i[5] * v[1] + i[2] * v[2] - i[7] * v[3] + i[6] * v[4];
  r[3] = i[8] * v[1] - i[7] * v[2] + i[9] * v[3];
  r[4] = i[6] * v[2] - i[8] * v[0] + i[9] * v[4];
  r[5] = i[7] * v[0] - i[6] * v[1] + i[9] * v[5];
}
MRE_PHASE_FN void finger_bias(ModelP M, Sm& s, int l) {
  constexpr int LINK7 = GRIP_BODY0 - 1;
  const bool fin = l >= GRIP_BODY0 && l < NRB;
  const int i = fin ? l - GRIP_BODY0 : 0;
  double V7[6], A7[6];
  {
    const float* R = s.xmat[LINK7];
    float r[3];
    v3sub(r, s.site_xpos[M->tcp_site], s.com_robot);
    const double rd[3] = {(double)r[0], (double)r[1], (double)r[2]};
    for (int h = 0; h < 2; h++) {
      const float* c = &s.scratch[6 * h];
      const double w[3] = {(double)c[0], (double)c[1], (double)c[2]};
      double t[3];
      dcross3(t, w, rd);
      const double lin[3] = {(double)c[3] + t[0], (double)c[4] + t[1], (double)c[5] + t[2]};
      double* o = h == 0 ? V7 : A7;
      for (int k = 0; k < 3; k++) {
        o[k] = (double)R[k] * w[0] + (double)R[3 + k] * w[1] + (double)R[6 + k] * w[2];
        o[3 + k] = (double)R[k] * lin[0] + (double)R[3 + k] * lin[1] + (double)R[6 + k] * lin[2];
      }
    }
  }
  double S[6], I[10];
#pragma unroll
  for (int k = 0; k < 6; k++) S[k] = fin ? s.gS[i][k] : 0.0;
#pragma unroll
  for (int k = 0; k < 10; k++) I[k] = fin ? s.gI[i][k] : 0.0;
  const double qd = fin ? robot_v(s, l - 1) : 0.0;
  const bool child = fin && M->body_parent[l] >= GRIP_BODY0;
  double v[6], a0[6], sd[6];
  dcross_motion(sd, V7, S);
#pragma unroll
  for (int k = 0; k < 6; k++) { v[k] = V7[k] + S[k] * qd; a0[k] = A7[k] + sd[k] * qd; }
  double pv[6], pa[6];
#pragma unroll
  for (int k = 0; k < 6; k++) { pv[k] = dpp_shr1_d(v[k]); pa[k] = dpp_shr1_d(a0[k]); }
  if (child) {
    dcross_motion(sd, pv, S);
#pragma unroll
    for (int k = 0; k < 6; k++) { v[k] = pv[k] + S[k] * qd; a0[k] = pa[k] + sd[k] * qd; }
  }
  double f[6], t0[6], t1[6];
  dmul_inert_vec(t0, I, v);
  dcross_force(t1, v, t0);
  dmul_inert_vec(f, I, a0);
#pragma unroll
  for (int k = 0; k < 6; k++) f[k] += t1[k];
  double up[6];
#pragma unroll
  for (int k = 0; k < 6; k++) up[k] = dpp_shl1_d(f[k]);
  if (fin && !child) {
#pragma unroll
    for (int k = 0; k < 6; k++) f[k] += up[k];
  }
  if (fin) {
    double b = 0.0;
#pragma unroll
    for (int k = 0; k < 6; k++) b += S[k] * f[k];
    s.qfrc_bias[l - 1] = (float)b;
  }
  MRE_SYNC();
}

MRE_PHASE_FN unsigned arm_actuation(ModelP M, Sm& s, int l) {
  bool arm_clamped = false;
  if (l < 7) {
    float fa = (float)((double)(M->act_gain[l] * clampf(s.ctrl[l], M->act_ctrlrange[l][0], M->act_ctrlrange[l][1]) + M->act_bias[l][0]) +
                       (double)M->act_bias[l][1] * robot_q(s, l) + (double)M->act_bias[l][2] * robot_v(s, l));
    if (M->act_forcelimited[l]) {
      if (fa <= M->act_forcerange[l][0]) { fa = M->act_forcerange[l][0]; arm_clamped = true; }
      if (fa >= M->act_forcerange[l][1]) { fa = M->act_forcerange[l][1]; arm_clamped = true; }
    }
    s.qfrc_smooth[l] = fa;
  }
  return (unsigned)__ballot(arm_clamped) & 0x7Fu;
}

MRE_PHASE_FN unsigned smooth_forces_assemble(ModelP M, Sm& s, int l, unsigned arm_mask) {
  const double ten_len = (double)M->ten_coef[0] * robot_q(s, M->ten_dof[0]) + (double)M->ten_coef[1] * robot_q(s, M->ten_dof[1]);
  const double ten_vel = (double)M->ten_coef[0] * robot_v(s, M->ten_dof[0]) + (double)M->ten_coef[1] * robot_v(s, M->ten_dof[1]);
  const float cg = clampf(s.ctrl[NU - 1], M->act_ctrlrange[NU - 1][0], M->act_ctrlrange[NU - 1][1]);
  float fg = (float)((double)(M->grip_gainprm * cg + M->grip_biasprm[0]) + (double)M->grip_biasprm[1] * ten_len +
                     (double)M->grip_biasprm[2] * ten_vel);
  bool clamped = false;
  if (fg <= M->grip_forcerange[0]) { fg = M->grip_forcerange[0]; clamped = true; }
  if (fg >= M->grip_forcerange[1]) { fg = M->grip_forcerange[1]; clamped = true; }
  if (l < NV) {
    const int b = M->dof_body[l];
    float f = 0.f;
    if (b < NRB) {
      double fd = -(double)M->jnt_stiffness[b] * (robot_q(s, l) - (double)M->jnt_springref[b]) - (double)M->dof_damping[l] * robot_v(s, l);
      if (l < 7) fd += (double)s.qfrc_smooth[l];
      if (l == M->ten_dof[0]) fd += (double)M->ten_coef[0] * (double)fg;
      if (l == M->ten_dof[1]) fd += (double)M->ten_coef[1] * (double)fg;
      f = (float)(fd - (double)s.qfrc_bias[l]);
    }
    const bool act = body_is_active(M, s, b);
    f = act ? (b < NRB ? f : f - s.qfrc_bias[l]) : 0.f;
    s.qfrc_smooth[l] = f;
    s.qacc_smooth[l] = f;
  }
  MRE_SYNC();
  return arm_mask | (clamped ? 1u << (NU - 1) : 0u);
}
MRE_DEV unsigned smooth_forces(ModelP M, Sm& s, int l) {
  const unsigned arm_mask = arm_actuation(M, s, l);
  const unsigned mask = smooth_forces_assemble(M, s, l, arm_mask);
#ifndef MRE_NEWTON
  solve_robot_one(s.qLD, s.qLDinv, s.qacc_smooth, l);
#else
  factor_solve_robot(s.qM, s.qacc_smooth, l);
#endif
  if (l >= NRV && l < NV) {
    const int p = (l - NRV) / 6, k = (l - NRV) % 6;
    const float md = (k < 3) ? s.prop_mass[p] : s.prop_inertia[p][k - 3];
    s.qacc_smooth[l] = s.qacc_smooth[l] / md;
  }
  MRE_SYNC();
  return mask;
}

MRE_PHASE_FN void integrate_setup(ModelP M, Sm& s, int l, unsigned act_clamped) {
  const bool grip_clamped = (act_clamped >> (NU - 1)) & 1u;
  const float h = M->timestep;
  for (int e = l; e < NMR; e += 64) {
    float v = s.qM[e];
    const int i = M->M_i[e];
    if (i == M->M_j[e]) {
      v += h * M->dof_damping[i];
      if (i < 7 && ((act_clamped >> i) & 1u) == 0u) v -= h * M->act_bias[i][2];
      if (!grip_clamped) {
        if (i == M->ten_dof[0]) v -= h * M->grip_biasprm[2] * M->ten_coef[0] * M->ten_coef[0];
        if (i == M->ten_dof[1]) v -= h * M->grip_biasprm[2] * M->ten_coef[1] * M->ten_coef[1];
      }
    }
    mh_store(s)[e] = v;
#ifdef MRE_NEWTON
    if (i == M->M_j[e]) s.scratch[i] = (s.qM[e] - v) * s.qacc[i];
#endif
  }
#ifndef MRE_NEWTON
  if (l < NRV) s.scratch[l] = s.qfrc_smooth[l] + s.qfrc_con[l];
#endif
  MRE_SYNC();
}

MRE_PHASE_FN void integrate(ModelP M, Sm& s, int l, unsigned flags, bool polished, float* clo) {
  const float h = M->timestep;
  const bool freeze = (flags & F_FREEZE_ROBOT) != 0;
  if (l < NV) {
    const int b = M->dof_body[l];
    if (b < NRB) {
      if (!freeze) {
#ifdef MRE_NEWTON
        const double acc = polished ? reinterpret_cast<const double*>(&s.nw_Mv[0])[l] : (double)s.qacc[l];
        const double v = robot_v(s, l) + (double)h * (acc + (double)s.scratch[l]);
#else
        const double v = robot_v(s, l) + (double)h * (double)s.scratch[l];
#endif
        const float hi = (float)v;
        s.qvel[l] = hi; s.qlo[QFINE / 2 + l] = (float)(v - (double)hi);
      }
    } else if (body_is_active(M, s, b)) {
      if (clo != nullptr) {
        float* const vl = clo + (QFINE_CUBE_V - QFINE_CUBE_Q) + (l - NRV);
        const double v = (double)s.qvel[l] + (double)*vl + (double)h * (double)s.qacc[l];
        const float hi = (float)v, lo = (float)(v - (double)hi);
        s.qvel[l] = hi; *vl = lo;
        s.scratch[l] = lo;
      } else {
        s.qvel[l] += h * s.qacc[l];
      }
    }
  }
  MRE_SYNC();
  if (l >= 1 && l < NB) {
    const int b = l, qa = M->body_qposadr[b], da = M->body_dofadr[b];
    if (b < NRB) {
      if (!freeze) {
        const double q = robot_q(s, qa) + (double)h * robot_v(s, da);
        const float hi = (float)q;
        s.qpos[qa] = hi; s.qlo[qa] = (float)(q - (double)hi);
      }
    } else if (body_is_active(M, s, b) && clo != nullptr) {
      float* const ql = clo + 7 * (b - NRB);
      double vv[6];
      for (int k = 0; k < 6; k++) vv[k] = (double)s.qvel[da + k] + (double)s.scratch[da + k];
      for (int k = 0; k < 3; k++) {
        const double x = (double)s.qpos[qa + k] + (double)ql[k] + (double)h * vv[k];
        const float hi = (float)x;
        s.qpos[qa + k] = hi; ql[k] = (float)(x - (double)hi);
      }
      double q0[4], qn[4];
      for (int k = 0; k < 4; k++) q0[k] = (double)s.qpos[qa + 3 + k] + (double)ql[3 + k];
      const double wn2 = vv[3] * vv[3] + vv[4] * vv[4] + vv[5] * vv[5];
      if (wn2 > 1e-60) {
        const double inv = rsq64(wn2), half = 0.5 * (double)h * wn2 * inv;
        double sn, cs;
        sincos_poly_d(half, sn, cs);
        const double ax = vv[3] * inv * sn, ay = vv[4] * inv * sn, az = vv[5] * inv * sn;
        qn[0] = q0[0] * cs - q0[1] * ax - q0[2] * ay - q0[3] * az;
        qn[1] = q0[0] * ax + q0[1] * cs + q0[2] * az - q0[3] * ay;
        qn[2] = q0[0] * ay - q0[1] * az + q0[2] * cs + q0[3] * ax;
        qn[3] = q0[0] * az + q0[1] * ay - q0[2] * ax + q0[3] * cs;
      } else {
        for (int k = 0; k < 4; k++) qn[k] = q0[k];
      }
      const double nn = qn[0] * qn[0] + qn[1] * qn[1] + qn[2] * qn[2] + qn[3] * qn[3];
      const double sc = nn > 1e-30 ? rsq64(nn) : 1.0;
      for (int k = 0; k < 4; k++) {
        const double x = qn[k] * sc;
        const float hi = (float)x;
        s.qpos[qa + 3 + k] = hi; ql[3 + k] = (float)(x - (double)hi);
      }
    } else if (body_is_active(M, s, b)) {
      for (int k = 0; k < 3; k++) s.qpos[qa + k] += h * s.qvel[da + k];
      float w[3] = {s.qvel[da + 3], s.qvel[da + 4], s.qvel[da + 5]};
      const float ang = v3normalize(w) * h;
      float qr[4], qn[4], q0[4];
      axisangle2q(qr, w, ang);
      for (int k = 0; k < 4; k++) q0[k] = s.qpos[qa + 3 + k];
      qmul(qn, q0, qr);
      qnormalize(qn);
      for (int k = 0; k < 4; k++) s.qpos[qa + 3 + k] = qn[k];
    }
  }
  MRE_SYNC();
}

#ifdef MRE_PHASE_STAMPS
#define MRE_STAMP(k)                                                         \
  do {                                                                       \
    if ((k) < 12 || MRE_PHASE_STAMPS == 3) {                                 \
      const unsigned long long now_ = __builtin_amdgcn_s_memtime();          \
      if ((k) / 4 == MRE_PHASE_STAMPS) stamp_acc[(k) % 4] += now_ - stamp_t; \
      stamp_t = now_;                                                        \
    }                                                                        \
  } while (0)
#else
#define MRE_STAMP(k) do {} while (0)
#endif

MRE_DEV int q_load(const int* p) { return __hip_atomic_load(p, __ATOMIC_RELAXED, __HIP_MEMORY_SCOPE_AGENT); }

#ifdef MRE_LARGE_CAPS
constexpr bool Q_LARGE = true;
#else
constexpr bool Q_LARGE = false;
#endif
MRE_DEV int* q_bucket(const StepArgs& a, int t, int sh) {
  const int S = a.q_shards;
  return a.q_buf + (size_t)t * a.q_stride + (sh < S ? (size_t)sh * a.q_cap : (size_t)S * a.q_cap + (size_t)(sh - S) * a.q_capl);
}

MRE_DEV int queue_pop_shard(const StepArgs& a, int l, int sh, int& env, int& tick) {
  const int S = a.q_shards;
  const bool order0 = sh < S;
  const int n0 = (a.N - sh + S - 1) / S;
  int* const head = a.q_head + sh * QUEUE_TICKS_MAX;
  const int* const tail = a.q_tail + sh * QUEUE_TICKS_MAX;
  for (;;) {
    int h[QUEUE_TICKS_MAX / 64], tl[QUEUE_TICKS_MAX / 64];
#pragma unroll
    for (int c = 0; c < QUEUE_TICKS_MAX / 64; c++) {
      const int b = c * 64 + l;
      h[c] = 0; tl[c] = 0;
      if (b < a.q_nticks) { h[c] = q_load(head + b); tl[c] = (b == 0 && order0) ? n0 : q_load(tail + b); }
    }
    int t = -1, ht = 0;
#pragma unroll
    for (int c = 0; c < QUEUE_TICKS_MAX / 64; c++) {
      if (t < 0 && c * 64 < a.q_nticks) {
        const unsigned long long ready = __ballot(h[c] < tl[c]);
        if (ready != 0ull) {
          const int k = __ffsll((long long)ready) - 1;
          t = c * 64 + k;
          ht = __builtin_amdgcn_readlane(h[c], k);
        }
      }
    }
    if (t < 0) return 0;
    int got = -1;
    if (l == 0) {
      if (t == 0 && order0) {
        const int i = __hip_atomic_fetch_add(head, 1, __ATOMIC_RELAXED, __HIP_MEMORY_SCOPE_AGENT);
        if (i < n0) got = a.env_order != nullptr ? a.env_order[sh + S * i] : sh + S * i;
      } else {
        int expect = ht;
        if (__hip_atomic_compare_exchange_strong(head + t, &expect, ht + 1, __ATOMIC_RELAXED, __ATOMIC_RELAXED,
                                                 __HIP_MEMORY_SCOPE_AGENT)) {
          const int* slot = q_bucket(a, t, sh) + ht;
          int v = q_load(slot);
          for (unsigned spin = 0; v == 0; ++spin) {
            if (spin > (1u << 20)) { *a.q_err = 1; v = -1; break; }
            __builtin_amdgcn_s_sleep(4);
            v = q_load(slot);
          }
          got = v < 0 ? -2 : v - 1;
        }
      }
    }
    got = __builtin_amdgcn_readfirstlane(got);
    if (got == -2) return -1;
    if (got < 0) continue;
    env = got; tick = t;
    return 1;
  }
}
MRE_DEV bool queue_pop(const StepArgs& a, int l, int home, int& env, int& tick, int& shard) {
  const int S = a.q_shards;
  if (Q_LARGE) {
    const int SL = a.q_lshards;
    for (unsigned idle = 0;; ++idle) {
      int r = 0;
      for (int k = 0; k < SL && r == 0; ++k) {
        const int sh = S + (home + k < SL ? home + k : home + k - SL);
        r = queue_pop_shard(a, l, sh, env, tick);
        if (r != 0) shard = sh;
      }
      if (r != 0) return r > 0;
      if (a.q_wait == 0 || q_load(a.q_done) >= a.N) return false;
      if (idle > 512u && q_load(a.q_started) == 0) return false;
      if (idle > (1u << 18)) return false;
      __builtin_amdgcn_s_sleep(127);
    }
  }
  for (int k = 0; k < S; ++k) {
    const int sh = home + k < S ? home + k : home + k - S;
    const int r = queue_pop_shard(a, l, sh, env, tick);
    if (r != 0) { shard = sh; return r > 0; }
  }
  return false;
}
MRE_DEV void queue_push(const StepArgs& a, int l, int env, int tick, int shard) {
  __builtin_amdgcn_fence(__ATOMIC_RELEASE, "agent");
  asm volatile("s_waitcnt vmcnt(0)" ::: "memory");
  if (l == 0) {
    const int i = __hip_atomic_fetch_add(a.q_tail + shard * QUEUE_TICKS_MAX + tick, 1, __ATOMIC_RELAXED, __HIP_MEMORY_SCOPE_AGENT);
    __hip_atomic_store(q_bucket(a, tick, shard) + i, env + 1, __ATOMIC_RELAXED, __HIP_MEMORY_SCOPE_AGENT);
  }
}

template <bool QUEUE>
MRE_DEV void step_body(const StepArgs& a, Sm& s) {
  OscSm& osc = s.osc;
  const int l = threadIdx.x;
  int env = 0, qtick = 0, qshard = 0;
  if (!QUEUE) {
    if ((int)blockIdx.x >= a.N) return;
    env = a.env_order != nullptr ? a.env_order[blockIdx.x] : (int)blockIdx.x;
  }
  if (QUEUE && !Q_LARGE && l == 0) __hip_atomic_fetch_add(a.q_started, 1, __ATOMIC_RELAXED, __HIP_MEMORY_SCOPE_AGENT);
  if (QUEUE && Q_LARGE && a.q_wait != 0) {
    for (unsigned idle = 0; q_load(a.q_gen) != a.q_gen_expect; ++idle) {
      if (idle > 1024u) return;
      __builtin_amdgcn_s_sleep(127);
    }
  }
 for (;;) {
  if (QUEUE) {
    if (!queue_pop(a, l, (int)(blockIdx.x % (unsigned)(Q_LARGE ? a.q_lshards : a.q_shards)), env, qtick, qshard)) return;
    if (qtick > 0 || Q_LARGE) __builtin_amdgcn_fence(__ATOMIC_ACQUIRE, "agent");
  }
  const int step_lo = QUEUE ? qtick * a.control_steps : 0, step_hi = QUEUE ? step_lo + a.control_steps : a.nsteps;
  if (QUEUE && !Q_LARGE && qtick == 0 && a.large != nullptr && a.large[env] != 0) continue;
  if (!QUEUE || (!Q_LARGE && qtick == 0)) {
#define MRE_PASS_SKIP { if (QUEUE) { if (l == 0) __hip_atomic_fetch_add(a.q_done, 1, __ATOMIC_RELAXED, __HIP_MEMORY_SCOPE_AGENT); continue; } return; }
  if (!QUEUE && a.large != nullptr && (a.large[env] != 0) != (a.want_large != 0)) return;
// ... 646 lines not shown
```

### mujoco_robot_environments_amd/csrc/mre_math.h

```cpp
#pragma once
#include <hip/hip_runtime.h>

#define MRE_DEV __device__ __forceinline__
#if defined(MRE_PHASE_STAMPS) && MRE_PHASE_STAMPS >= 4
#define MRE_DBG_T0() unsigned long long dbg_t_ = __builtin_amdgcn_s_memtime()
#define MRE_DBG_STAMP(SET, K)                                                      \
  do {                                                                             \
    const unsigned long long n_ = __builtin_amdgcn_s_memtime();                    \
    if (MRE_PHASE_STAMPS == (SET) && threadIdx.x == 0) dbg_acc[K] += n_ - dbg_t_;  \
    dbg_t_ = n_;                                                                   \
  } while (0)
#else
#define MRE_DBG_T0() do {} while (0)
#define MRE_DBG_STAMP(SET, K) do {} while (0)
#endif
#define MRE_PHASE_FN __device__ __attribute__((noinline))
#define MRE_SYNC()                                        \
  do {                                                    \
    __builtin_amdgcn_fence(__ATOMIC_ACQ_REL, "wavefront"); \
    __builtin_amdgcn_wave_barrier();                      \
  } while (0)
#if defined(__HIP_DEVICE_COMPILE__)
#define MRE_MODEL_PTR(T) const T __attribute__((address_space(1)))*
#else
#define MRE_MODEL_PTR(T) const T*
#endif

namespace mre {

constexpr float kMinVal = 1e-15f;

MRE_DEV void v3copy(float* r, const float* a) { r[0] = a[0]; r[1] = a[1]; r[2] = a[2]; }
MRE_DEV void v3zero(float* r) { r[0] = r[1] = r[2] = 0.f; }
MRE_DEV void v3add(float* r, const float* a, const float* b) {
  r[0] = a[0] + b[0]; r[1] = a[1] + b[1]; r[2] = a[2] + b[2];
}
MRE_DEV void v3sub(float* r, const float* a, const float* b) {
  r[0] = a[0] - b[0]; r[1] = a[1] - b[1]; r[2] = a[2] - b[2];
}
MRE_DEV float v3dot(const float* a, const float* b) { return a[0] * b[0] + a[1] * b[1] + a[2] * b[2]; }
MRE_DEV void v3cross(float* r, const float* a, const float* b) {
  float x = a[1] * b[2] - a[2] * b[1], y = a[2] * b[0] - a[0] * b[2], z = a[0] * b[1] - a[1] * b[0];
  r[0] = x; r[1] = y; r[2] = z;
}
MRE_DEV void v3addscl(float* r, const float* a, float s) { r[0] += a[0] * s; r[1] += a[1] * s; r[2] += a[2] * s; }
MRE_DEV float v3norm(const float* a) { return sqrtf(v3dot(a, a)); }
MRE_DEV float v3normalize(float* a) {
  float n = v3norm(a);
  if (n < kMinVal) { a[0] = 1.f; a[1] = 0.f; a[2] = 0.f; return n; }
  float inv = 1.0f / n;
  a[0] *= inv; a[1] *= inv; a[2] *= inv;
  return n;
}
MRE_DEV void m3mulv(float* r, const float* m, const float* v) {
  float x = m[0] * v[0] + m[1] * v[1] + m[2] * v[2];
  float y = m[3] * v[0] + m[4] * v[1] + m[5] * v[2];
  float z = m[6] * v[0] + m[7] * v[1] + m[8] * v[2];
  r[0] = x; r[1] = y; r[2] = z;
}
MRE_DEV void m3tmulv(float* r, const float* m, const float* v) {
  float x = m[0] * v[0] + m[3] * v[1] + m[6] * v[2];
  float y = m[1] * v[0] + m[4] * v[1] + m[7] * v[2];
  float z = m[2] * v[0] + m[5] * v[1] + m[8] * v[2];
  r[0] = x; r[1] = y; r[2] = z;
}
MRE_DEV void qmul(float* r, const float* a, const float* b) {
  float w = a[0] * b[0] - a[1] * b[1] - a[2] * b[2] - a[3] * b[3];
  float x = a[0] * b[1] + a[1] * b[0] + a[2] * b[3] - a[3] * b[2];
  float y = a[0] * b[2] - a[1] * b[3] + a[2] * b[0] + a[3] * b[1];
  float z = a[0] * b[3] + a[1] * b[2] - a[2] * b[1] + a[3] * b[0];
  r[0] = w; r[1] = x; r[2] = y; r[3] = z;
}
MRE_DEV void qnormalize(float* q) {
  float n = sqrtf(q[0] * q[0] + q[1] * q[1] + q[2] * q[2] + q[3] * q[3]);
  if (n < kMinVal) { q[0] = 1.f; q[1] = q[2] = q[3] = 0.f; return; }
  float inv = 1.0f / n;
  q[0] *= inv; q[1] *= inv; q[2] *= inv; q[3] *= inv;
}
MRE_DEV void q2mat(float* m, const float* q) {
  float w = q[0], x = q[1], y = q[2], z = q[3];
  m[0] = w * w + x * x - y * y - z * z; m[1] = 2 * (x * y - w * z); m[2] = 2 * (x * z + w * y);
  m[3] = 2 * (x * y + w * z); m[4] = w * w - x * x + y * y - z * z; m[5] = 2 * (y * z - w * x);
  m[6] = 2 * (x * z - w * y); m[7] = 2 * (y * z + w * x); m[8] = w * w - x * x - y * y + z * z;
}
MRE_DEV void qrotv(float* r, const float* q, const float* v) {
  float m[9];
  q2mat(m, q);
  m3mulv(r, m, v);
}
MRE_DEV void sincos_small(float x, float* sn, float* cs) {
  const float j = rintf(x * 0.6366197723675814f);
  float r = fmaf(-j, 1.5703125f, x);
  r = fmaf(-j, 4.837512969970703125e-4f, r);
  r = fmaf(-j, 7.54978995489188192e-8f, r);
  const float z = r * r;
  const float ps = fmaf(fmaf(fmaf(-1.9515295891e-4f, z, 8.3321608736e-3f), z, -1.6666654611e-1f), z * r, r);
  const float pc = fmaf(fmaf(fmaf(2.443315711809948e-5f, z, -1.388731625493765e-3f), z, 4.166664568298827e-2f), z * z,
                        fmaf(-0.5f, z, 1.0f));
  const int q = (int)j & 3;
  const float a = (q & 1) ? pc : ps, b = (q & 1) ? ps : pc;
  *sn = (q & 2) ? -a : a;
  *cs = ((q + 1) & 2) ? -b : b;
}
MRE_DEV void axisangle2q(float* q, const float* axis, float angle) {
  float s, c;
  sincos_small(0.5f * angle, &s, &c);
  q[0] = c; q[1] = axis[0] * s; q[2] = axis[1] * s; q[3] = axis[2] * s;
}
MRE_DEV void mat2q(float* q, const float* m) {
  float t = m[0] + m[4] + m[8];
  if (t > 0) {
    float s = sqrtf(t + 1.0f) * 2;
    q[0] = 0.25f * s; q[1] = (m[7] - m[5]) / s; q[2] = (m[2] - m[6]) / s; q[3] = (m[3] - m[1]) / s;
  } else if (m[0] > m[4] && m[0] > m[8]) {
    float s = sqrtf(1.0f + m[0] - m[4] - m[8]) * 2;
    q[0] = (m[7] - m[5]) / s; q[1] = 0.25f * s; q[2] = (m[1] + m[3]) / s; q[3] = (m[2] + m[6]) / s;
  } else if (m[4] > m[8]) {
    float s = sqrtf(1.0f + m[4] - m[0] - m[8]) * 2;
    q[0] = (m[2] - m[6]) / s; q[1] = (m[1] + m[3]) / s; q[2] = 0.25f * s; q[3] = (m[5] + m[7]) / s;
  } else {
    float s = sqrtf(1.0f + m[8] - m[0] - m[4]) * 2;
    q[0] = (m[3] - m[1]) / s; q[1] = (m[2] + m[6]) / s; q[2] = (m[5] + m[7]) / s; q[3] = 0.25f * s;
  }
  qnormalize(q);
}
MRE_DEV void mul_inert_vec(float* r, const float* i, const float* v) {
  r[0] = i[0] * v[0] + i[3] * v[1] + i[4] * v[2] - i[8] * v[4] + i[7] * v[5];
  r[1] = i[3] * v[0] + i[1] * v[1] + i[5] * v[2] + i[8] * v[3] - i[6] * v[5];
  r[2] = i[4] * v[0] + i[5] * v[1] + i[2] * v[2] - i[7] * v[3] + i[6] * v[4];
  r[3] = i[8] * v[1] - i[7] * v[2] + i[9] * v[3];
  r[4] = i[6] * v[2] - i[8] * v[0] + i[9] * v[4];
  r[5] = i[7] * v[0] - i[6] * v[1] + i[9] * v[5];
}
MRE_DEV void cross_motion(float* r, const float* vel, const float* v) {
  float a[3], b[3];
  v3cross(r, vel, v);
  v3cross(a, vel, v + 3);
  v3cross(b, vel + 3, v);
  v3add(r + 3, a, b);
}
MRE_DEV void cross_force(float* r, const float* vel, const float* f) {
  float a[3], b[3];
  v3cross(a, vel, f);
  v3cross(b, vel + 3, f + 3);
  v3add(r, a, b);
  v3cross(r + 3, vel, f + 3);
}
MRE_DEV float dot6(const float* a, const float* b) {
  return a[0] * b[0] + a[1] * b[1] + a[2] * b[2] + a[3] * b[3] + a[4] * b[4] + a[5] * b[5];
}
template <int CTRL, int ROW_MASK>
MRE_DEV float dpp_add(float v) {
  const int t = __builtin_amdgcn_update_dpp(0, __builtin_bit_cast(int, v), CTRL, ROW_MASK, 0xF, false);
  return v + __builtin_bit_cast(float, t);
}
MRE_DEV float wave_sum(float v) {
  v = dpp_add<0xB1, 0xF>(v);
  v = dpp_add<0x4E, 0xF>(v);
  v = dpp_add<0x141, 0xF>(v);
  v = dpp_add<0x140, 0xF>(v);
  v = dpp_add<0x142, 0xA>(v);
  v = dpp_add<0x143, 0xC>(v);
  return __builtin_bit_cast(float, __builtin_amdgcn_readlane(__builtin_bit_cast(int, v), 63));
}
MRE_DEV void wave_sum3(float& a, float& b, float& c) {
  asm volatile(
      "s_nop 1\n\t"
      "v_add_f32_dpp %0, %0, %0 quad_perm:[1,0,3,2] row_mask:0xf bank_mask:0xf bound_ctrl:1\n\t"
      "v_add_f32_dpp %1, %1, %1 quad_perm:[1,0,3,2] row_mask:0xf bank_mask:0xf bound_ctrl:1\n\t"
      "v_add_f32_dpp %2, %2, %2 quad_perm:[1,0,3,2] row_mask:0xf bank_mask:0xf bound_ctrl:1\n\t"
      "v_add_f32_dpp %0, %0, %0 quad_perm:[2,3,0,1] row_mask:0xf bank_mask:0xf bound_ctrl:1\n\t"
      "v_add_f32_dpp %1, %1, %1 quad_perm:[2,3,0,1] row_mask:0xf bank_mask:0xf bound_ctrl:1\n\t"
      "v_add_f32_dpp %2, %2, %2 quad_perm:[2,3,0,1] row_mask:0xf bank_mask:0xf bound_ctrl:1\n\t"
      "v_add_f32_dpp %0, %0, %0 row_half_mirror row_mask:0xf bank_mask:0xf bound_ctrl:1\n\t"
      "v_add_f32_dpp %1, %1, %1 row_half_mirror row_mask:0xf bank_mask:0xf bound_ctrl:1\n\t"
      "v_add_f32_dpp %2, %2, %2 row_half_mirror row_mask:0xf bank_mask:0xf bound_ctrl:1\n\t"
      "v_add_f32_dpp %0, %0, %0 row_mirror row_mask:0xf bank_mask:0xf bound_ctrl:1\n\t"
      "v_add_f32_dpp %1, %1, %1 row_mirror row_mask:0xf bank_mask:0xf bound_ctrl:1\n\t"
      "v_add_f32_dpp %2, %2, %2 row_mirror row_mask:0xf bank_mask:0xf bound_ctrl:1\n\t"
      "v_add_f32_dpp %0, %0, %0 row_bcast:15 row_mask:0xa bank_mask:0xf\n\t"
      "v_add_f32_dpp %1, %1, %1 row_bcast:15 row_mask:0xa bank_mask:0xf\n\t"
      "v_add_f32_dpp %2, %2, %2 row_bcast:15 row_mask:0xa bank_mask:0xf\n\t"
      "v_add_f32_dpp %0, %0, %0 row_bcast:31 row_mask:0xc bank_mask:0xf\n\t"
// ... 38 lines not shown
```

### mujoco_robot_environments_amd/csrc/mre_solver.h

```cpp
#pragma once

namespace mre {

constexpr int HDR_NONE = 0xFF;
constexpr int BLK_NONE = 0x7F;
constexpr int SCHED_NONE = 0xFF;
constexpr int TAB_OFF = MAXBLK * 5;
constexpr int TAB_ZEROS = 48;
static_assert(TAB_BYTES == 8 * (TAB_OFF + 1) + 4 * TAB_ZEROS, "operand table size");

#ifndef MRE_NEWTON
MRE_DEV void build_schedule(ModelP M, Sm& s);
#endif
MRE_DEV constexpr int cube_pair_bit(int p, int q) {
  const int a = p < q ? p : q, b = p < q ? q : p;
  return a == 0 ? b - 1 : (a == 1 ? b + 1 : 5);
}

MRE_DEV float prop_invM(const Sm& s, int p, int k) {
  return 1.0f / ((k < 3) ? s.prop_mass[p] : s.prop_inertia[p][k - 3]);
}

MRE_DEV void geom_pose(ModelP M, const Sm& s, int g, float* p, float* R, float* size,
                       float* rbound) {
// ... 111 lines not shown
      tot += __popcll(m) << bit;
    }
    if (l == 0) {
      s.ncon = tot < NCON_MAX ? tot : NCON_MAX;
      if (tot > NCON_MAX) s.overflow = 1;
    }
    if (single) {
      const float incw = M->pair_rec[pr].margin - M->pair_rec[pr].gap;
      float wsum = 0.f, px = 0.f, py = 0.f, pz = 0.f, dmin = cand_dist(buf, 0);
      int best = 0;
      for (int c = 0; c < ncand; c++) {
        const float dc = cand_dist(buf, c);
        if (dc < dmin) { dmin = dc; best = c; }
        const float w = incw - dc;
        if (w > 0.f) { wsum += w; px += w * cand_xyz(buf, c)[0]; py += w * cand_xyz(buf, c)[1]; pz += w * cand_xyz(buf, c)[2]; }
      }
      if (wsum > 0.f) { const float iw = 1.0f / wsum; px *= iw; py *= iw; pz *= iw; }
      else { px = cand_xyz(buf, best)[0]; py = cand_xyz(buf, best)[1]; pz = cand_xyz(buf, best)[2]; }
      cand_xyz(buf, 0)[0] = px; cand_xyz(buf, 0)[1] = py; cand_xyz(buf, 0)[2] = pz;
      cand_dist(buf, 0) = dmin;
    }
    if (n > 0) {
      float f[9];
      v3copy(f, normal);
      make_frame(f);
      for (int c = 0; c < n; c++) {
        const int id = off + c;
        if (id >= NCON_MAX) break;
        const float cx0 = cand_xyz(buf, c)[0], cx1 = cand_xyz(buf, c)[1], cx2 = cand_xyz(buf, c)[2];
        s.con_pos[id][0] = cx0; s.con_pos[id][1] = cx1; s.con_pos[id][2] = cx2;
        for (int k = 0; k < 9; k++) s.con_frame[id][k] = f[k];
        s.con_dist[id] = cand_dist(buf, c);
        s.con_pair[id] = (uint8_t)pr;
      }
    }
    MRE_SYNC();
    MRE_DBG_STAMP(6, 3);
    if (tot > NCON_MAX) break;
    base = tot;
  }
}

MRE_DEV float impedance(const float* solimp, float pos, float margin) {
  const float dmin = clampf(solimp[0], 0.0001f, 0.9999f), dmax = clampf(solimp[1], 0.0001f, 0.9999f);
  const float width = fmaxf(solimp[2], kMinVal), mid = clampf(solimp[3], 0.0001f, 0.9999f);
  const float power = fmaxf(solimp[4], 1.0f);
  if (dmin == dmax) return 0.5f * (dmin + dmax);
  const float x = fabsf((pos - margin) / width);
  if (x >= 1.0f) return dmax;
  if (x <= 0.0f) return dmin;
  float y;
  if (power == 1.0f) y = x;
  else if (power == 2.0f) {
    y = (x <= mid) ? x * x / mid : 1.0f - (1.0f - x) * (1.0f - x) / (1.0f - mid);
  }
  else if (x <= mid) y = powf(x, power) / powf(mid, power - 1.0f);
  else y = 1.0f - powf(1.0f - x, power) / powf(1.0f - mid, power - 1.0f);
  return dmin + y * (dmax - dmin);
}

MRE_DEV void jac_robot(ModelP M, Sm& s, int rs, int b, const float* p, const float* ax, float sg) {
  float off[3];
  v3sub(off, p, s.com_robot);
  const int n = M->chain_len[b];
  for (int k = 0; k < n; k++) {
    const int j = M->chain_dof[b][k];
    const float* c = s.cdof[j];
    float t[3];
    v3cross(t, c, off);
    s.Jr[rs][j] += sg * (ax[0] * (c[3] + t[0]) + ax[1] * (c[4] + t[1]) + ax[2] * (c[5] + t[2]));
  }
}
MRE_DEV int row_blk(const Sm& s, int i, int& r) {
  const int ns = 7 + s.nl;
  if (i < ns) { r = i % 3; return i / 3; }
  const int cr = i - ns;
  r = cr % 3;
  return 8 + cr / 3;
}
#ifdef MRE_NEWTON
MRE_DEV float& rowR(Sm& s, int i) { return s.efc_R[i]; }
MRE_DEV float& rowB(Sm& s, int i) { return s.efc_aref[i]; }
#else
MRE_DEV float& rowR(Sm& s, int i) { int r; const int b = row_blk(s, i, r); return s.blkrec[b][r]; }
MRE_DEV float& rowB(Sm& s, int i) { int r; const int b = row_blk(s, i, r); return s.blkrec[b][3 + r]; }
MRE_DEV float& rowAinv(Sm& s, int i) { int r; const int b = row_blk(s, i, r); return s.blkrec[b][6 + r]; }
#endif

MRE_DEV float* jpA(Sm& s, int i) { return s.JpA[i - 7 - s.nl]; }
MRE_DEV const float* jpA(const Sm& s, int i) { return s.JpA[i - 7 - s.nl]; }
MRE_DEV float* jpB(Sm& s, int i) { const int cr = i - 7 - s.nl; return s.JpB[3 * s.con_bslot[cr / 3] + cr % 3]; }
MRE_DEV const float* jpB(const Sm& s, int i) { const int cr = i - 7 - s.nl; return s.JpB[3 * s.con_bslot[cr / 3] + cr % 3]; }
MRE_DEV void jac_prop(Sm& s, int i, int slot, int b, const float* p, const float* ax, float sg) {
  float off[3];
  v3sub(off, p, s.xpos[b]);
  float* J = slot == 0 ? jpA(s, i) : jpB(s, i);
  for (int k = 0; k < 3; k++) {
    J[k] = sg * ax[k];
    float axk[3] = {s.xmat[b][k], s.xmat[b][3 + k], s.xmat[b][6 + k]}, t[3];
    v3cross(t, axk, off);
    J[3 + k] = sg * v3dot(ax, t);
  }
}

MRE_DEV float row_dot(const Sm& s, int i, const float* vec) {
  const int h = s.hdr[i];
  const int rs = h & 0xFF, pa = (h >> 8) & 0xF, pb = (h >> 12) & 0xF;
  float acc = 0.f;
  if (rs != HDR_NONE)
    for (int j = 0; j < NRV; j++) acc += s.Jr[rs][j] * vec[j];
  if (pa < NPROP)
    { const float* ja = jpA(s, i); for (int k = 0; k < 6; k++) acc += ja[k] * vec[NRV + 6 * pa + k]; }
  if (pb < NPROP)
    { const float* jb = jpB(s, i); for (int k = 0; k < 6; k++) acc += jb[k] * vec[NRV + 6 * pb + k]; }
  return acc;
}

MRE_DEV void row_dot2(const Sm& s, int i, const float* v1, const float* v2, float& r1, float& r2) {
  const int h = s.hdr[i];
  const int rs = h & 0xFF, pa = (h >> 8) & 0xF, pb = (h >> 12) & 0xF;
  float a1 = 0.f, a2 = 0.f;
  if (rs != HDR_NONE)
    for (int j = 0; j < NRV; j++) { const float jv = s.Jr[rs][j]; a1 += jv * v1[j]; a2 += jv * v2[j]; }
  if (pa < NPROP) {
    const float* ja = jpA(s, i);
    for (int k = 0; k < 6; k++) { const float jv = ja[k]; a1 += jv * v1[NRV + 6 * pa + k]; a2 += jv * v2[NRV + 6 * pa + k]; }
  }
  if (pb < NPROP) {
    const float* jb = jpB(s, i);
    for (int k = 0; k < 6; k++) { const float jv = jb[k]; a1 += jv * v1[NRV + 6 * pb + k]; a2 += jv * v2[NRV + 6 * pb + k]; }
  }
  r1 = a1; r2 = a2;
}

#ifndef MRE_NEWTON
MRE_PHASE_FN void solve_robot_rows(Sm& s, int l) {
  for (int rs = l; rs < s.nrrow; rs += 64) {
    float x[NRV];
#pragma unroll
    for (int k = 0; k < NRV; k++) x[k] = s.Jr[rs][k];
    solve_robot_regs(s.qLD, s.qLDinv, x);
#pragma unroll
    for (int k = 0; k < NRV; k++) s.Br[rs][k] = x[k];
  }
  MRE_SYNC();
}

#endif

constexpr int GRIP0 = GRIP_BODY0;

MRE_PHASE_FN void assemble_constraints(ModelP M, Sm& s, int l) {
  int lim = 0, lim_side = 0;
  if (l >= 1 && l < NRB && M->jnt_limited[l]) {
    const double q = robot_q(s, l - 1);
    if (q - (double)M->jnt_range[l][0] < 0.0) { lim = 1; lim_side = -1; }
    else if ((double)M->jnt_range[l][1] - q < 0.0) { lim = 1; lim_side = 1; }
  }
  const unsigned long long limm = __ballot(lim != 0);
  const int lim_idx = __popcll(limm & ((1ull << l) - 1ull));
  if (l == 0) s.nl = __popcll(limm);
  if (lim) s.lim_info[lim_idx] = l | ((lim_side > 0 ? 1 : 0) << 8);
  if (l < s.ncon) {
    const int pr = s.con_pair[l];
    s.con_b1[l] = (uint8_t)M->pair_rec[pr].b1;
    s.con_b2[l] = (uint8_t)M->pair_rec[pr].b2;
  }
  MRE_SYNC();
#ifndef MRE_NEWTON
  {
    static_assert(sizeof(s.sched) % 4 == 0, "schedule cleared by words");
    unsigned* w = reinterpret_cast<unsigned*>(&s.sched[0][0]);
    for (int e = l; e < (int)(sizeof(s.sched) / 4); e += 64) w[e] = 0x01010101u * (unsigned)SCHED_NONE;
  }
#endif
  {
    const int base = 7 + s.nl, ncon0 = s.ncon;
    const bool on = l < ncon0;
    const int cb1 = on ? s.con_b1[l] : 0, cb2 = on ? s.con_b2[l] : 0;
    const bool rob_any = on && ((cb1 < NRB && cb1 > 0) || (cb2 < NRB && cb2 > 0));
    const bool fing = on && ((cb1 >= GRIP_BODY0 && cb1 < NRB) || (cb2 >= GRIP_BODY0 && cb2 < NRB));
    const unsigned long long fingm = __ballot(fing);
    const bool two_props = on && cb1 >= NRB && cb2 >= NRB;
    const unsigned long long lt = (1ull << l) - 1ull;
    const unsigned long long rmask = __ballot(rob_any), tmask = __ballot(two_props);
    const int my_r = base + 3 * __popcll(rmask & lt), my_b = __popcll(tmask & lt);
    const bool fail = on && (base + 3 * (l + 1) > NEFC_MAX || (rob_any && my_r + 3 > NRROW_MAX) ||
                             (two_props && my_b >= NPP_MAX));
    const unsigned long long fmask = __ballot(fail);
    const int kept = fmask != 0ull ? (int)__builtin_ctzll(fmask) : ncon0;
    if (l < kept) {
      s.con_rslot[l] = rob_any ? my_r : HDR_NONE;
      s.con_bslot[l] = two_props ? my_b : 0;
    }
    MRE_SYNC();
    if (l == 0) {
      const unsigned long long below = kept >= 64 ? ~0ull : ((1ull << kept) - 1ull);
      if (fmask != 0ull) s.overflow = 1;
      s.ncon = kept;
      s.nefc = base + 3 * kept;
      s.nrrow = base + 3 * __popcll(rmask & below);
      s.npp = __popcll(tmask & below);
      s.finger_contact = (fingm & below) != 0ull;
#ifdef MRE_NEWTON
      s.nsched = 0; s.nblk = 0;
#else
      build_schedule(M, s);
#endif
    }
  }
  MRE_SYNC();
  const int nefc = s.nefc, nl = s.nl;
  for (int e = l; e < s.nrrow * NRV; e += 64) (&s.Jr[0][0])[e] = 0.f;
#ifndef MRE_NEWTON
  for (int e = l; e < 8 * 16; e += 64) (&s.blkrec[0][0])[e] = 0.f;
#endif
  MRE_SYNC();
  for (int i = l; i < nefc; i += 64) {
    int rs = HDR_NONE, pa = 0xF, pb = 0xF;
    float pos = 0.f, margin = 0.f, diag = 0.f, imp_pos = 0.f;
    const float *solref, *solimp;
    bool fric_row = false;
    float R0scale = 1.0f;
    if (i < 7) {
      rs = i;
      const int e = i < 6 ? i / 3 : 2;
      solref = M->eq_solref[e]; solimp = M->eq_solimp[e];
      if (e < 2) {
        const int b1 = M->eq_obj[e][0], b2 = M->eq_obj[e][1], k = i % 3;
        int root = b1;
        while (root >= GRIP0) root = M->body_parent[root];
        const float* loc = &s.qfrc_con[16 * e];
        const float* R = s.xmat[root];
        float cp[3];
        m3mulv(cp, R, loc);
        const float rk[3] = {R[3 * k], R[3 * k + 1], R[3 * k + 2]};
        const int pb1 = M->body_parent[b1], pb2 = M->body_parent[b2];
        s.Jr[rs][b1 - 1] += v3dot(rk, loc + 4);
        if (pb1 >= GRIP0) s.Jr[rs][pb1 - 1] += v3dot(rk, loc + 7);
        s.Jr[rs][b2 - 1] += v3dot(rk, loc + 10);
        if (pb2 >= GRIP0) s.Jr[rs][pb2 - 1] += v3dot(rk, loc + 13);
        {
          const int n = M->chain_len[root];
          for (int c = 0; c < n; c++) {
            const int j = M->chain_dof[root][c];
            float t[3];
            v3cross(t, s.cdof[j], cp);
            s.Jr[rs][j] += sel3(t, k);
          }
        }
        pos = sel3(cp, k);
        imp_pos = v3norm(cp);
        diag = M->body_invweight0[b1][0] + M->body_invweight0[b2][0];
      } else {
        const int b1 = M->eq_obj[e][0], b2 = M->eq_obj[e][1];
        const int d1 = b1 - 1, d2 = b2 - 1;
        const float* pc = M->eq_data[e];
        const double dif64 = robot_q(s, d2) - (double)M->qpos0[d2];
        pos = (float)(robot_q(s, d1) - (double)M->qpos0[d1] -
                      ((double)pc[0] + dif64 * ((double)pc[1] + dif64 * ((double)pc[2] + dif64 * ((double)pc[3] + dif64 * (double)pc[4])))));
        const float dif = (float)dif64;
        const float deriv = pc[1] + dif * (2.f * pc[2] + dif * (3.f * pc[3] + dif * 4.f * pc[4]));
        s.Jr[rs][d1] += 1.f;
        s.Jr[rs][d2] -= deriv;
        imp_pos = pos;
        diag = M->dof_invweight0[d1] + M->dof_invweight0[d2];
      }
    } else if (i < 7 + nl) {
      rs = i;
      const int info = s.lim_info[i - 7], b = info & 0xFF, hi = (info >> 8) & 1;
      const double q = robot_q(s, b - 1);
      pos = (float)(hi ? ((double)M->jnt_range[b][1] - q) : (q - (double)M->jnt_range[b][0]));
      s.Jr[rs][b - 1] = hi ? -1.f : 1.f;
      imp_pos = pos;
      diag = M->dof_invweight0[b - 1];
      solref = M->jnt_solref[b]; solimp = M->jnt_solimp[b];
    } else {
      const int c = (i - 7 - nl) / 3, r = (i - 7 - nl) % 3;
      const int pr = s.con_pair[c];
      const int b1 = s.con_b1[c], b2 = s.con_b2[c];
      const float* ax = &s.con_frame[c][3 * r];
      const float* p = s.con_pos[c];
      const int rs0 = s.con_rslot[c];
      if (rs0 != HDR_NONE) rs = rs0 + r;
      int slot = 0;
      float dg = 0.f;
      if (b1 > 0) {
        if (b1 < NRB) { jac_robot(M, s, rs, b1, p, ax, -1.f); dg += M->body_invweight0[b1][0]; }
        else { pa = b1 - NRB; jac_prop(s, i, slot++, b1, p, ax, -1.f); dg += 1.0f / s.prop_mass[pa]; }
      }
      if (b2 > 0) {
        if (b2 < NRB) { jac_robot(M, s, rs, b2, p, ax, 1.f); dg += M->body_invweight0[b2][0]; }
        else {
          const int pid = b2 - NRB;
          if (slot == 0) pa = pid; else pb = pid;
          jac_prop(s, i, slot++, b2, p, ax, 1.f);
          dg += 1.0f / s.prop_mass[pid];
        }
      }
      diag = dg;
      solref = M->pair_solref[pr]; solimp = M->pair_solimp[pr];
      margin = M->pair_margin[pr] - M->pair_gap[pr];
      imp_pos = s.con_dist[c];
      if (r == 0) pos = s.con_dist[c];
      else {
        fric_row = true;
        pos = 0.f;
        R0scale = 1.0f / fmaxf(M->impratio, kMinVal);
      }
      if (M->cone == 0) {
        const float fr = M->pair_friction[pr][0];
        diag = dg * (1.f + fr * fr);
        R0scale = 2.f * fr * fr / fmaxf(M->impratio, kMinVal);
      }
    }
    s.hdr[i] = rs | (pa << 8) | (pb << 12);
    const float imp = impedance(solimp, imp_pos, margin);
    float tc = solref[0];
    const float dr = solref[1], dmax = clampf(solimp[1], 0.0001f, 0.9999f);
    float K, B;
    if (tc > 0.f) {
      tc = fmaxf(tc, 2.f * M->timestep);
      K = 1.0f / (dmax * dmax * tc * tc * dr * dr);
      B = 2.0f / (dmax * tc);
    } else { K = -tc / (dmax * dmax); B = -dr / dmax; }
    if (fric_row) K = 0.f;
    float R = fmaxf((1.f - imp) * diag / imp, kMinVal) * R0scale;
    if (M->cone == 0) R = fmaxf(R, kMinVal);
    const float vel = row_dot(s, i, s.qvel);
    const float efc_margin = fric_row ? 0.f : margin;
    const float aref = -B * vel - K * imp * (pos - efc_margin);
    rowR(s, i) = R; rowB(s, i) = aref;
#ifdef MRE_NEWTON
    if (i >= 7 + nl && (i - 7 - nl) % 3 == 0) s.con_fric[(i - 7 - nl) / 3] = M->pair_friction[s.con_pair[(i - 7 - nl) / 3]][0];
#else
    if (i >= 7 + nl && (i - 7 - nl) % 3 == 0) s.blkrec[8 + (i - 7 - nl) / 3][15] = M->pair_friction[s.con_pair[(i - 7 - nl) / 3]][0];
#endif
  }
  MRE_SYNC();
}

#ifndef MRE_NEWTON
MRE_PHASE_FN void assemble_blocks(ModelP M, Sm& s, int l) {
  const int nefc = s.nefc, nl = s.nl;
  for (int i = l; i < nefc; i += 64) {
    const int h = s.hdr[i];
    const int rs = h & 0xFF, pa = (h >> 8) & 0xF, pb = (h >> 12) & 0xF;
    const bool scalar = i < 7 + nl;
    const int r = scalar ? i % 3 : (i - 7 - nl) % 3;
    const int i0 = i - r;
    const int nb = scalar ? ((7 + nl - i0) < 3 ? (7 + nl - i0) : 3) : 3;
    const int slot = scalar ? i / 3 : 8 + (i - 7 - nl) / 3;
    float acc[3] = {0.f, 0.f, 0.f};
#pragma unroll
    for (int cc = 0; cc < 3; cc++) {
      float a = 0.f;
      if (cc < nb) {
        if (rs != HDR_NONE) {
          const int rs2 = rs - r + cc;
          for (int j = 0; j < NRV; j++) a += s.Jr[rs][j] * s.Br[rs2][j];
        }
        if (pa < NPROP)
          { const float *x = jpA(s, i), *y = jpA(s, i0 + cc); for (int k = 0; k < 6; k++) a += x[k] * y[k] * prop_invM(s, pa, k); }
        if (pb < NPROP)
          { const float *x = jpB(s, i), *y = jpB(s, i0 + cc); for (int k = 0; k < 6; k++) a += x[k] * y[k] * prop_invM(s, pb, k); }
      }
      acc[cc] = a;
    }
    const float diag = (r == 0 ? acc[0] : (r == 1 ? acc[1] : acc[2])) + rowR(s, i);
    if (r == 0) acc[0] = scalar ? acc[0] : diag;
    if (r == 1) acc[1] = scalar ? acc[1] : diag;
    if (r == 2) acc[2] = scalar ? acc[2] : diag;
    if (r == 0) { s.blkrec[slot][9] = acc[0]; s.blkrec[slot][10] = acc[1]; s.blkrec[slot][11] = acc[2]; }
    if (r == 1) { s.blkrec[slot][12] = acc[1]; s.blkrec[slot][13] = acc[2]; }
    if (r == 2) { s.blkrec[slot][14] = acc[2]; }
    s.blkrec[slot][6 + r] = 1.0f / diag;
  }
  MRE_SYNC();
}

MRE_DEV float fast_rcp(float x) { return __builtin_amdgcn_rcpf(x); }

MRE_DEV bool qcqp2(float* res, const float* A, const float* b, float d0, float d1, float r) {
  const float b1 = b[0] * d0, b2 = b[1] * d1;
  const float A11 = A[0] * d0 * d0, A22 = A[3] * d1 * d1, A12 = A[1] * d0 * d1;
  float la = 0.f, v1 = 0.f, v2 = 0.f;
  const float r2 = r * r;
  for (int iter = 0; iter < 20; iter++) {
    const float det = (A11 + la) * (A22 + la) - A12 * A12;
    if (det < 1e-10f) { res[0] = res[1] = 0.f; return false; }
    const float di = fast_rcp(det);
    const float P11 = (A22 + la) * di, P22 = (A11 + la) * di, P12 = -A12 * di;
    v1 = -P11 * b1 - P12 * b2;
    v2 = -P12 * b1 - P22 * b2;
    const float val = v1 * v1 + v2 * v2 - r * r;
    if (val < fmaxf(1e-10f, 1e-6f * r2)) break;
    const float deriv = -2.0f * (P11 * v1 * v1 + 2.0f * P12 * v1 * v2 + P22 * v2 * v2);
    const float delta = -val * fast_rcp(deriv);
    if (delta < 1e-10f) break;
    la += delta;
  }
  res[0] = v1 * d0;
  res[1] = v2 * d1;
  return la != 0.f;
}

MRE_DEV int lane_island(int l) { return l < 16 ? 0 : (l < 48 ? 1 + ((l - 16) >> 3) : -1); }
MRE_DEV int lane_dof(int l) {
  if (l < NRV) return l;
  if (l >= 16 && l < 48 && ((l - 16) & 7) < 6) return NRV + 6 * ((l - 16) >> 3) + ((l - 16) & 7);
  return -1;
}
MRE_DEV void island_sum3(float& x, float& y, float& z) {
  asm volatile(
      "s_nop 1\n\t"
      "v_add_f32_dpp %0, %0, %0 quad_perm:[1,0,3,2] row_mask:0xf bank_mask:0xf bound_ctrl:1\n\t"
      "v_add_f32_dpp %1, %1, %1 quad_perm:[1,0,3,2] row_mask:0xf bank_mask:0xf bound_ctrl:1\n\t"
      "v_add_f32_dpp %2, %2, %2 quad_perm:[1,0,3,2] row_mask:0xf bank_mask:0xf bound_ctrl:1\n\t"
      "v_add_f32_dpp %0, %0, %0 quad_perm:[2,3,0,1] row_mask:0xf bank_mask:0xf bound_ctrl:1\n\t"
      "v_add_f32_dpp %1, %1, %1 quad_perm:[2,3,0,1] row_mask:0xf bank_mask:0xf bound_ctrl:1\n\t"
      "v_add_f32_dpp %2, %2, %2 quad_perm:[2,3,0,1] row_mask:0xf bank_mask:0xf bound_ctrl:1\n\t"
      "v_add_f32_dpp %0, %0, %0 row_half_mirror row_mask:0xf bank_mask:0xf bound_ctrl:1\n\t"
      "v_add_f32_dpp %1, %1, %1 row_half_mirror row_mask:0xf bank_mask:0xf bound_ctrl:1\n\t"
      "v_add_f32_dpp %2, %2, %2 row_half_mirror row_mask:0xf bank_mask:0xf bound_ctrl:1\n\t"
      "v_add_f32_dpp %0, %0, %0 row_mirror row_mask:0x1 bank_mask:0xf\n\t"
      "v_add_f32_dpp %1, %1, %1 row_mirror row_mask:0x1 bank_mask:0xf\n\t"
      "v_add_f32_dpp %2, %2, %2 row_mirror row_mask:0x1 bank_mask:0xf\n\t"
      "s_nop 1"
      : "+v"(x), "+v"(y), "+v"(z));
}

MRE_DEV void lane_JB(const Sm& s, int row, int rs, int l, int lk, int slot, float linvM, float& j, float& b) {
  j = 0.f; b = 0.f;
  if (l < NRV) {
    if (rs != BLK_NONE) { j = s.Jr[rs][l]; b = s.Br[rs][l]; }
  } else if (slot >= 0) {
    j = (slot == 0 ? jpA(s, row) : jpB(s, row))[lk];
    b = j * linvM;
  }
}


MRE_DEV void build_schedule(ModelP M, Sm& s) {
  int* last = s.iscr;
  for (int k = 0; k < 5; k++) last[k] = 0;
  const int nscalar = 7 + s.nl;
  int nb = 0, nst = 0;
  for (int i = 0; i < nscalar; i += 3) {
    Blk b;
    b.row0 = (uint16_t)i; b.type = 0; b.nrows = (uint8_t)((nscalar - i) < 3 ? (nscalar - i) : 3);
    b.rslot = (uint8_t)i; b.pa = 0xF; b.pb = 0xF; b.primary = 0; b.bslot = 0;
    const int st = last[0]++;
    s.sched[st][0] = (uint8_t)nb;
    s.blk[nb++] = b;
    if (last[0] > nst) nst = last[0];
  }
  for (int c = 0; c < s.ncon; c++) {
    const int b1 = s.con_b1[c], b2 = s.con_b2[c];
    const int rs = s.con_rslot[c];
    int pa = 0xF, pb = 0xF;
    if (b1 >= NRB) pa = b1 - NRB;
    if (b2 >= NRB) { if (pa == 0xF) pa = b2 - NRB; else pb = b2 - NRB; }
    const bool hr = rs != HDR_NONE, ha = pa != 0xF, hb = pb != 0xF;
    int st = 0;
    if (hr && last[0] > st) st = last[0];
    if (ha && last[1 + pa] > st) st = last[1 + pa];
    if (hb && last[1 + pb] > st) st = last[1 + pb];
    Blk b;
    b.row0 = (uint16_t)(nscalar + 3 * c); b.type = 2; b.nrows = 3;
    b.rslot = (uint8_t)(hr ? rs : BLK_NONE); b.pa = (uint8_t)pa; b.pb = (uint8_t)pb;
    b.primary = (uint8_t)(hr ? 0 : 1 + pa); b.bslot = (uint8_t)(hb ? s.con_bslot[c] : 0);
    if (hr) { last[0] = st + 1; s.sched[st][0] = (uint8_t)nb; }
    if (ha) { last[1 + pa] = st + 1; s.sched[st][1 + pa] = (uint8_t)nb; }
    if (hb) { last[1 + pb] = st + 1; s.sched[st][1 + pb] = (uint8_t)nb; }
    if (st + 1 > nst) nst = st + 1;
    s.blk[nb++] = b;
  }
  s.nblk = nb;
  s.nsched = nst;
}

template <bool PYR>
MRE_DEV void solve_constraints_impl(ModelP M, Sm& s, int l) {
  const int nefc = s.nefc, nl = s.nl;
  const int isl = lane_island(l);
  const int ldof = lane_dof(l);
  const int lp = (isl > 0) ? isl - 1 : -1;
  const int lk = (isl > 0) ? ((l - 16) & 7) : 0;
  const bool lvalid = ldof >= 0;
// ... 398 lines not shown
```

Measured before the change: 23.79 million.

## Pack per-body, per-dof and per-row model parameters into aligned device records

Adds 16-byte-aligned packed record structs (body, dof, mass-matrix entry, constraint row, equality, site, options) to the device model, filled and bit-verified on the host. Kernels load each record up front, so scattered per-field loads from many separate arrays become a few contiguous loads. Equality chains become fully unrolled bounded loops, and keep_live hints stop the compiler from re-materialising values. This costs a larger model struct and possibly more registers from loading all fields eagerly, including fields a given branch does not use.

Measured after the change: 24.49 million, median of 6. 3.0% higher.

```diff
diff --git a/mujoco_robot_environments_amd/csrc/mre_api.cpp b/mujoco_robot_environments_amd/csrc/mre_api.cpp
--- a/mujoco_robot_environments_amd/csrc/mre_api.cpp
+++ b/mujoco_robot_environments_amd/csrc/mre_api.cpp
@@ -650,6 +650,193 @@
 #define RI(name, dst, n) if (!b.ints(name, (int*)(dst), n)) return fail(MRE_ERR_MODEL, std::string("model entry ") + name)
 #define RF(name, dst, n) if (!b.flts(name, (float*)(dst), n)) return fail(MRE_ERR_MODEL, std::string("model entry ") + name)
 
+static bool same_bits(const void* a, const void* b, size_t n) { return memcmp(a, b, n) == 0; }
+static int pack_records(DevModel& m) {
+  if (m.ten_dof[0] == m.ten_dof[1] || m.ten_dof[0] < 0 || m.ten_dof[0] >= NRV || m.ten_dof[1] < 0 || m.ten_dof[1] >= NRV)
+    return fail(MRE_ERR_MODEL, "the gripper tendon must couple two different robot dofs");
+  for (int e = 0; e < NEQ; e++)
+    for (int k = 0; k < 2; k++)
+      if (m.eq_obj[e][k] < 1 || m.eq_obj[e][k] >= NRB) return fail(MRE_ERR_MODEL, "equality constraints must couple robot bodies");
+  if (m.tcp_site < 0 || m.tcp_site >= NSITE || m.eef_site < 0 || m.eef_site >= NSITE) return fail(MRE_ERR_MODEL, "tcp_site / eef_site name no site");
+  for (int b = 1; b < NRB; b++)
+    if (m.body_parent[b] != ROBOT_DOF_PARENT[b - 1] + 1) return fail(MRE_ERR_MODEL, "robot body tree differs from the one the kernels are unrolled for (mre_dev.h)");
+  for (int d = 0; d < NV; d++)
+    if (m.dof_body[d] != (d < NRV ? d + 1 : NRB + (d - NRV) / 6)) return fail(MRE_ERR_MODEL, "dof layout differs from the compiled kernels");
+  auto ten_of = [&](int d) { return d == m.ten_dof[0] ? 0 : (d == m.ten_dof[1] ? 1 : -1); };
+  for (int b = 0; b < NB; b++) {
+    BodyRec& r = m.body_rec[b];
+    memset(&r, 0, sizeof(r));
+    for (int c = 0; c < 4; c++) { r.quat[c] = m.body_quat[b][c]; r.iquat[c] = m.body_iquat[b][c]; }
+    for (int c = 0; c < 3; c++) { r.pos[c] = m.body_pos[b][c]; r.ipos[c] = m.body_ipos[b][c]; r.jnt_pos[c] = m.jnt_pos[b][c];
+                                  r.jnt_axis[c] = m.jnt_axis[b][c]; r.inertia[c] = m.body_inertia[b][c]; }
+    for (int c = 0; c < 2; c++) { r.jnt_range[c] = m.jnt_range[b][c]; r.invweight0[c] = m.body_invweight0[b][c]; }
+    r.mass = m.body_mass[b]; r.qposadr = m.body_qposadr[b]; r.dofadr = m.body_dofadr[b]; r.propid = m.body_propid[b];
+    r.qpos0 = (r.qposadr >= 0 && r.qposadr < NQ) ? m.qpos0[r.qposadr] : 0.f;
+    r.jnt_stiffness = m.jnt_stiffness[b]; r.jnt_springref = m.jnt_springref[b];
+    r.parent = m.body_parent[b]; r.jnt_limited = m.jnt_limited[b];
+  }
+  for (int d = 0; d < NV; d++) {
+    DofRec& r = m.dof_rec[d];
+    memset(&r, 0, sizeof(r));
+    const int b = m.dof_body[d];
+    if (b < 0 || b >= NB) return fail(MRE_ERR_MODEL, "dof_bodyid names a body that does not exist");
+    r.body = b; r.propid = m.body_propid[b]; r.dofadr = m.body_dofadr[b]; r.ten = ten_of(d);
+    r.armature = m.dof_armature[d]; r.damping = m.dof_damping[d]; r.invweight0 = m.dof_invweight0[d];
+    r.ten_coef = r.ten >= 0 ? m.ten_coef[r.ten] : 0.f;
+    r.jnt_stiffness = m.jnt_stiffness[b]; r.jnt_springref = m.jnt_springref[b];
+    if (d < 7) {
+      r.act_gain = m.act_gain[d]; r.act_bias0 = m.act_bias[d][0]; r.act_bias1 = m.act_bias[d][1]; r.act_bias2 = m.act_bias[d][2];
+      r.act_ctrl_lo = m.act_ctrlrange[d][0]; r.act_ctrl_hi = m.act_ctrlrange[d][1];
+      r.act_force_lo = m.act_forcerange[d][0]; r.act_force_hi = m.act_forcerange[d][1];
+      r.act_forcelimited = m.act_forcelimited[d];
+    }
+  }
+  for (int e = 0; e < NMR; e++) {
+    MEntryRec& r = m.m_rec[e];
+    memset(&r, 0, sizeof(r));
+    r.i = m.M_i[e]; r.j = m.M_j[e];
+    r.armature = m.dof_armature[r.i]; r.damping = m.dof_damping[r.i];
+    r.act_bias2 = r.i < 7 ? m.act_bias[r.i][2] : 0.f;
+    r.ten = ten_of(r.i); r.ten_coef = r.ten >= 0 ? m.ten_coef[r.ten] : 0.f;
+  }
+  for (int k = 0; k < NROWREC; k++) memset(&m.row_rec[k], 0, sizeof(RowRec));
+  for (int e = 0; e < NEQ; e++) {
+    RowRec& r = m.row_rec[e];
+    const int b1 = m.eq_obj[e][0], b2 = m.eq_obj[e][1];
+    for (int c = 0; c < 2; c++) r.solref[c] = m.eq_solref[e][c];
+    for (int c = 0; c < 5; c++) r.solimp[c] = m.eq_solimp[e][c];
+    r.invw1 = e < 2 ? m.body_invweight0[b1][0] : m.dof_invweight0[b1 - 1];
+    r.invw2 = e < 2 ? m.body_invweight0[b2][0] : m.dof_invweight0[b2 - 1];
+    EqRec& q = m.eq_rec[e];
+    memset(&q, 0, sizeof(q));
+    q.type = m.eq_type[e]; q.b1 = b1; q.b2 = b2; q.pb1 = m.body_parent[b1]; q.pb2 = m.body_parent[b2];
+    q.root = b1;
+    while (q.root >= GRIP_BODY0) q.root = m.body_parent[q.root];
+    for (int c = 0; c < 8; c++) q.data[c] = m.eq_data[e][c];
+    q.qpos0_1 = m.qpos0[b1 - 1]; q.qpos0_2 = m.qpos0[b2 - 1];
+    q.root_chain_len = m.chain_len[q.root];
+    for (int c = 0; c < MAXCHAIN; c++) q.root_chain[c] = m.chain_dof[q.root][c];
+  }
+  for (int b = 1; b < NRB; b++) {
+    RowRec& r = m.row_rec[ROWREC_JNT + b];
+    for (int c = 0; c < 2; c++) r.solref[c] = m.jnt_solref[b][c];
+    for (int c = 0; c < 5; c++) r.solimp[c] = m.jnt_solimp[b][c];
+    r.invw1 = m.dof_invweight0[b - 1];
+  }
+  for (int k = 0; k < NPAIR; k++) {
+    if (m.pair_g1[k] < 0) continue;
+    RowRec& r = m.row_rec[ROWREC_PAIR + k];
+    const int b1 = m.pair_rec[k].b1, b2 = m.pair_rec[k].b2;
+    for (int c = 0; c < 2; c++) r.solref[c] = m.pair_solref[k][c];
+    for (int c = 0; c < 5; c++) r.solimp[c] = m.pair_solimp[k][c];
+    r.margin = m.pair_margin[k]; r.gap = m.pair_gap[k]; r.friction = m.pair_friction[k][0];
+    r.invw1 = (b1 > 0 && b1 < NRB) ? m.body_invweight0[b1][0] : 0.f;
+    r.invw2 = (b2 > 0 && b2 < NRB) ? m.body_invweight0[b2][0] : 0.f;
+  }
+  for (int k = 0; k < NSITE; k++) {
+    SiteRec& r = m.site_rec[k];
+    memset(&r, 0, sizeof(r));
+    if (m.site_body[k] < 0 || m.site_body[k] >= NB) return fail(MRE_ERR_MODEL, "site_bodyid names a body that does not exist");
+    r.body = m.site_body[k];
+    for (int c = 0; c < 3; c++) r.pos[c] = m.site_pos[k][c];
+    for (int c = 0; c < 4; c++) r.quat[c] = m.site_quat[k][c];
+  }
+  {
+    OptRec& o = m.opt_rec;
+    memset(&o, 0, sizeof(o));
+    o.timestep = m.timestep; o.impratio = m.impratio; o.tolerance = m.tolerance; o.iterations = m.iterations;
+    for (int c = 0; c < 3; c++) { o.gravity[c] = m.gravity[c]; o.grip_biasprm[c] = m.grip_biasprm[c]; }
+    o.cone = m.cone;
+    for (int c = 0; c < 2; c++) { o.ten_coef[c] = m.ten_coef[c]; o.ten_dof[c] = m.ten_dof[c]; o.grip_forcerange[c] = m.grip_forcerange[c];
+                                  o.grip_ctrlrange[c] = m.act_ctrlrange[NU - 1][c]; }
+    o.grip_gainprm = m.grip_gainprm; o.robot_mass = m.robot_mass; o.M0_diag_robot_sum = m.M0_diag_robot_sum;
+    o.tcp_site = m.tcp_site; o.eef_site = m.eef_site;
+    for (int c = 0; c < 3; c++) o.tcp_pos[c] = m.site_pos[m.tcp_site][c];
+  }
+
+  bool ok = true;
+#define SAME(a, b) ok = ok && sizeof(a) == sizeof(b) && same_bits(&(a), &(b), sizeof(a))
+  for (int b = 0; b < NB && ok; b++) {
+    const BodyRec& r = m.body_rec[b];
+    SAME(r.quat, m.body_quat[b]); SAME(r.pos, m.body_pos[b]); SAME(r.mass, m.body_mass[b]); SAME(r.jnt_pos, m.jnt_pos[b]);
+    SAME(r.jnt_axis, m.jnt_axis[b]); SAME(r.qposadr, m.body_qposadr[b]); SAME(r.ipos, m.body_ipos[b]);
+    SAME(r.propid, m.body_propid[b]); SAME(r.iquat, m.body_iquat[b]); SAME(r.inertia, m.body_inertia[b]);
+    SAME(r.dofadr, m.body_dofadr[b]); SAME(r.jnt_range, m.jnt_range[b]); SAME(r.invweight0, m.body_invweight0[b]);
+    SAME(r.jnt_stiffness, m.jnt_stiffness[b]); SAME(r.jnt_springref, m.jnt_springref[b]); SAME(r.parent, m.body_parent[b]);
+    SAME(r.jnt_limited, m.jnt_limited[b]);
+    if (b >= 1) SAME(r.qpos0, m.qpos0[m.body_qposadr[b]]);
+  }
+  for (int d = 0; d < NV && ok; d++) {
+    const DofRec& r = m.dof_rec[d];
+    const int b = m.dof_body[d];
+    SAME(r.body, m.dof_body[d]); SAME(r.propid, m.body_propid[b]); SAME(r.dofadr, m.body_dofadr[b]);
+    ok = ok && r.ten == (d == m.ten_dof[0] ? 0 : (d == m.ten_dof[1] ? 1 : -1));
+    SAME(r.armature, m.dof_armature[d]); SAME(r.damping, m.dof_damping[d]); SAME(r.invweight0, m.dof_invweight0[d]);
+    if (r.ten >= 0) SAME(r.ten_coef, m.ten_coef[r.ten]);
+    SAME(r.jnt_stiffness, m.jnt_stiffness[b]); SAME(r.jnt_springref, m.jnt_springref[b]);
+    if (d < 7) {
+      SAME(r.act_gain, m.act_gain[d]); SAME(r.act_bias0, m.act_bias[d][0]); SAME(r.act_bias1, m.act_bias[d][1]);
+      SAME(r.act_bias2, m.act_bias[d][2]); SAME(r.act_ctrl_lo, m.act_ctrlrange[d][0]); SAME(r.act_ctrl_hi, m.act_ctrlrange[d][1]);
+      SAME(r.act_force_lo, m.act_forcerange[d][0]); SAME(r.act_force_hi, m.act_forcerange[d][1]);
+      SAME(r.act_forcelimited, m.act_forcelimited[d]);
+    }
+  }
+  for (int e = 0; e < NMR && ok; e++) {
+    const MEntryRec& r = m.m_rec[e];
+    SAME(r.i, m.M_i[e]); SAME(r.j, m.M_j[e]);
+    const int i = m.M_i[e];
+    SAME(r.armature, m.dof_armature[i]); SAME(r.damping, m.dof_damping[i]);
+    if (i < 7) SAME(r.act_bias2, m.act_bias[i][2]);
+    ok = ok && r.ten == (i == m.ten_dof[0] ? 0 : (i == m.ten_dof[1] ? 1 : -1));
+    if (r.ten >= 0) SAME(r.ten_coef, m.ten_coef[r.ten]);
+  }
+  for (int e = 0; e < NEQ && ok; e++) {
+    const RowRec& r = m.row_rec[e];
+    const EqRec& q = m.eq_rec[e];
+    const int b1 = m.eq_obj[e][0], b2 = m.eq_obj[e][1];
+    SAME(r.solref, m.eq_solref[e]); SAME(r.solimp, m.eq_solimp[e]);
+    if (e < 2) { SAME(r.invw1, m.body_invweight0[b1][0]); SAME(r.invw2, m.body_invweight0[b2][0]); }
+    else { SAME(r.invw1, m.dof_invweight0[b1 - 1]); SAME(r.invw2, m.dof_invweight0[b2 - 1]); }
+    SAME(q.type, m.eq_type[e]); SAME(q.b1, m.eq_obj[e][0]); SAME(q.b2, m.eq_obj[e][1]);
+    SAME(q.pb1, m.body_parent[b1]); SAME(q.pb2, m.body_parent[b2]); SAME(q.data, m.eq_data[e]);
+    SAME(q.qpos0_1, m.qpos0[b1 - 1]); SAME(q.qpos0_2, m.qpos0[b2 - 1]);
+    int root = b1;
+    while (root >= GRIP_BODY0) root = m.body_parent[root];
+    ok = ok && q.root == root;
+    SAME(q.root_chain_len, m.chain_len[root]);
+    for (int c = 0; c < MAXCHAIN; c++) SAME(q.root_chain[c], m.chain_dof[root][c]);
+  }
+  for (int b = 1; b < NRB && ok; b++) {
+    const RowRec& r = m.row_rec[ROWREC_JNT + b];
+    SAME(r.solref, m.jnt_solref[b]); SAME(r.solimp, m.jnt_solimp[b]); SAME(r.invw1, m.dof_invweight0[b - 1]);
+  }
+  for (int k = 0; k < NPAIR && ok; k++) {
+    if (m.pair_g1[k] < 0) continue;
+    const RowRec& r = m.row_rec[ROWREC_PAIR + k];
+    const int b1 = m.geom_body[m.pair_g1[k]], b2 = m.geom_body[m.pair_g2[k]];
+    SAME(r.solref, m.pair_solref[k]); SAME(r.solimp, m.pair_solimp[k]); SAME(r.margin, m.pair_margin[k]);
+    SAME(r.gap, m.pair_gap[k]); SAME(r.friction, m.pair_friction[k][0]);
+    if (b1 > 0 && b1 < NRB) SAME(r.invw1, m.body_invweight0[b1][0]);
+    if (b2 > 0 && b2 < NRB) SAME(r.invw2, m.body_invweight0[b2][0]);
+  }
+  for (int k = 0; k < NSITE && ok; k++) {
+    const SiteRec& r = m.site_rec[k];
+    SAME(r.body, m.site_body[k]); SAME(r.pos, m.site_pos[k]); SAME(r.quat, m.site_quat[k]);
+  }
+  {
+    const OptRec& o = m.opt_rec;
+    SAME(o.timestep, m.timestep); SAME(o.impratio, m.impratio); SAME(o.tolerance, m.tolerance); SAME(o.iterations, m.iterations);
+    SAME(o.gravity, m.gravity); SAME(o.cone, m.cone); SAME(o.ten_coef, m.ten_coef); SAME(o.ten_dof, m.ten_dof);
+    SAME(o.grip_gainprm, m.grip_gainprm); SAME(o.grip_biasprm, m.grip_biasprm); SAME(o.grip_forcerange, m.grip_forcerange);
+    SAME(o.grip_ctrlrange, m.act_ctrlrange[NU - 1]); SAME(o.robot_mass, m.robot_mass);
+    SAME(o.M0_diag_robot_sum, m.M0_diag_robot_sum); SAME(o.tcp_site, m.tcp_site); SAME(o.eef_site, m.eef_site);
+    SAME(o.tcp_pos, m.site_pos[m.tcp_site]);
+  }
+#undef SAME
+  if (!ok) return fail(MRE_ERR_MODEL, "a packed model record differs from the table it was filled from");
+  return MRE_OK;
+}
+
 static int build_model(const void* blob, size_t nbytes, DevModel& m) {
   if (nbytes < 16) return fail(MRE_ERR_MODEL, "blob too small");
   Blob b{(const unsigned char*)blob, nbytes};
@@ -828,7 +1015,7 @@
   for (int p = 0; p < NPROP; p++) {
     m.park_pos[p][0] = 2.0f + 0.5f * p; m.park_pos[p][1] = 2.0f; m.park_pos[p][2] = -5.0f;
   }
-  return MRE_OK;
+  return pack_records(m);
 }
 
 extern "C" const char* mre_last_error(void) { return g_err.c_str(); }
diff --git a/mujoco_robot_environments_amd/csrc/mre_dev.h b/mujoco_robot_environments_amd/csrc/mre_dev.h
--- a/mujoco_robot_environments_amd/csrc/mre_dev.h
+++ b/mujoco_robot_environments_amd/csrc/mre_dev.h
@@ -87,6 +87,62 @@
   float size2[3], gap;
 };
 static_assert(sizeof(PairRec) == 128, "PairRec is eight 16-byte words");
+
+struct alignas(16) BodyRec {
+  float quat[4];
+  float pos[3], mass;
+  float jnt_pos[3], qpos0;
+  float jnt_axis[3]; int qposadr;
+  float ipos[3]; int propid;
+  float iquat[4];
+  float inertia[3]; int dofadr;
+  float jnt_range[2], invweight0[2];
+  float jnt_stiffness, jnt_springref; int parent, jnt_limited;
+};
+static_assert(sizeof(BodyRec) == 144, "BodyRec is nine 16-byte words");
+struct alignas(16) DofRec {
+  int body, propid, dofadr, ten;
+  float armature, damping, invweight0, ten_coef;
+  float jnt_stiffness, jnt_springref, act_gain, act_bias0;
+  float act_bias1, act_bias2, act_ctrl_lo, act_ctrl_hi;
+  float act_force_lo, act_force_hi; int act_forcelimited, pad;
+};
+static_assert(sizeof(DofRec) == 80, "DofRec is five 16-byte words");
+struct alignas(16) MEntryRec {
+  int i, j; float armature, damping;
+  float act_bias2, ten_coef; int ten, pad;
+};
+static_assert(sizeof(MEntryRec) == 32, "MEntryRec is two 16-byte words");
+struct alignas(16) RowRec {
+  float solref[2], margin, gap;
+  float solimp[5], friction;
+  float invw1, invw2;
+};
+static_assert(sizeof(RowRec) == 48, "RowRec is three 16-byte words");
+constexpr int ROWREC_JNT = NEQ, ROWREC_PAIR = NEQ + NB, NROWREC = NEQ + NB + NPAIR;
+struct alignas(16) EqRec {
+  int type, b1, b2, pb1;
+  int pb2, root, pad0, pad1;
+  float data[8];
+  float qpos0_1, qpos0_2; int pad2, root_chain_len;
+  int root_chain[12];
+};
+static_assert(sizeof(EqRec) == 128 && MAXCHAIN <= 12, "EqRec is eight 16-byte words");
+struct alignas(16) SiteRec {
+  float pos[3]; int body;
+  float quat[4];
+};
+static_assert(sizeof(SiteRec) == 32, "SiteRec is two 16-byte words");
+struct alignas(16) OptRec {
+  float timestep, impratio, tolerance; int iterations;
+  float gravity[3]; int cone;
+  float ten_coef[2]; int ten_dof[2];
+  float grip_gainprm, grip_biasprm[3];
+  float grip_forcerange[2], grip_ctrlrange[2];
+  float robot_mass, M0_diag_robot_sum; int tcp_site, eef_site;
+  float tcp_pos[3]; int pad;
+};
+static_assert(sizeof(OptRec) == 112, "OptRec is seven 16-byte words");
 
 struct DevModel {
   int body_parent[NB], body_level[NB], body_jnttype[NB], body_dofadr[NB], body_qposadr[NB];
@@ -131,6 +187,13 @@
   int cone;
   float home_qpos[7];
   float park_pos[NPROP][3];
+  BodyRec body_rec[NB];
+  DofRec dof_rec[NV];
+  MEntryRec m_rec[NMR];
+  RowRec row_rec[NROWREC];
+  EqRec eq_rec[NEQ];
+  SiteRec site_rec[NSITE];
+  OptRec opt_rec;
 };
 
 struct OscConfig {
diff --git a/mujoco_robot_environments_amd/csrc/mre_kernels.hip b/mujoco_robot_environments_amd/csrc/mre_kernels.hip
--- a/mujoco_robot_environments_amd/csrc/mre_kernels.hip
+++ b/mujoco_robot_environments_amd/csrc/mre_kernels.hip
@@ -125,6 +125,25 @@
 MRE_DEV double robot_q(const Sm& s, int d) { return (double)s.qpos[d] + (double)s.qlo[d]; }
 MRE_DEV double robot_v(const Sm& s, int d) { return (double)s.qvel[d] + (double)s.qlo[QFINE / 2 + d]; }
 
+MRE_DEV bool prop_is_active(const Sm& s, int propid) { return propid < 0 || propid < s.nprops; }
+
+struct BodyK {
+  float quat[4], pos[3], mass, jnt_pos[3], qpos0, jnt_axis[3], ipos[3], iquat[4], inertia[3];
+  int qposadr, propid, dofadr, parent;
+};
+MRE_DEV BodyK load_body(ModelP M, int b) {
+  const auto* R = &M->body_rec[b];
+  BodyK B;
+#pragma unroll
+  for (int k = 0; k < 4; k++) { B.quat[k] = R->quat[k]; B.iquat[k] = R->iquat[k]; }
+#pragma unroll
+  for (int k = 0; k < 3; k++) { B.pos[k] = R->pos[k]; B.jnt_pos[k] = R->jnt_pos[k]; B.jnt_axis[k] = R->jnt_axis[k];
+                                B.ipos[k] = R->ipos[k]; B.inertia[k] = R->inertia[k]; }
+  B.mass = R->mass; B.qpos0 = R->qpos0; B.qposadr = R->qposadr; B.propid = R->propid; B.dofadr = R->dofadr;
+  B.parent = R->parent;
+  return B;
+}
+
 MRE_DEV bool body_is_active(ModelP M, const Sm& s, int b) {
   int p = M->body_propid[b];
   return p < 0 || p < s.nprops;
@@ -163,13 +182,13 @@
   const double dx = uy * cz - uz * cy, dy = uz * cx - ux * cz, dz = ux * cy - uy * cx;
   r[0] = v[0] + 2.0 * (w * cx + dx); r[1] = v[1] + 2.0 * (w * cy + dy); r[2] = v[2] + 2.0 * (w * cz + dz);
 }
-MRE_DEV void hinge_local_d(ModelP M, const Sm& s, int b, double* p, double* q) {
+MRE_DEV void hinge_local_d(const BodyK& B, const Sm& s, double* p, double* q) {
   double q0[4], ql[4], ax[3], jp[3], t0[3], t1[3];
-  for (int k = 0; k < 4; k++) q0[k] = (double)M->body_quat[b][k];
-  for (int k = 0; k < 3; k++) { ax[k] = (double)M->jnt_axis[b][k]; jp[k] = (double)M->jnt_pos[b][k]; }
-  const int qa = M->body_qposadr[b];
+  for (int k = 0; k < 4; k++) q0[k] = (double)B.quat[k];
+  for (int k = 0; k < 3; k++) { ax[k] = (double)B.jnt_axis[k]; jp[k] = (double)B.jnt_pos[k]; }
+  const int qa = B.qposadr;
   double s4, c4;
-  sincos_poly_d(0.25 * (robot_q(s, qa) - (double)M->qpos0[qa]), s4, c4);
+  sincos_poly_d(0.25 * (robot_q(s, qa) - (double)B.qpos0), s4, c4);
   const double sn = 2.0 * s4 * c4, cs = 1.0 - 2.0 * s4 * s4;
   ql[0] = cs; ql[1] = ax[0] * sn; ql[2] = ax[1] * sn; ql[3] = ax[2] * sn;
   dq_mul(q, q0, ql);
@@ -177,7 +196,7 @@
   for (int k = 0; k < 4; k++) q[k] *= n;
   dq_rot(t0, q0, jp);
   dq_rot(t1, q, jp);
-  for (int k = 0; k < 3; k++) p[k] = (double)M->body_pos[b][k] + t0[k] - t1[k];
+  for (int k = 0; k < 3; k++) p[k] = (double)B.pos[k] + t0[k] - t1[k];
 }
 template <int CTRL>
 MRE_DEV double dpp_row_d(double v, double fill) {
@@ -236,11 +255,15 @@
   for (int c = 0; c < 3; c++) p[c] = ap[c] + t[c];
 }
 template <bool WRITEBACK>
-MRE_DEV void kinematics(ModelP M, Sm& s, int l, BodyRegs& br) {
+MRE_DEV void kinematics(ModelP M, Sm& s, int l, BodyRegs& br, const BodyK& B) {
   constexpr int LINK7 = GRIP_BODY0 - 1;
   const bool arm = l >= 1 && l <= LINK7, fin = l >= GRIP_BODY0 && l < NRB;
+  const auto* SR = &M->site_rec[l < NSITE ? l : 0];
+  const int site_b = SR->body, eef_site = M->opt_rec.eef_site;
+  const float site_pos[3] = {SR->pos[0], SR->pos[1], SR->pos[2]};
+  const float site_quat[4] = {SR->quat[0], SR->quat[1], SR->quat[2], SR->quat[3]};
   double q[4] = {1.0, 0.0, 0.0, 0.0}, p[3] = {0.0, 0.0, 0.0};
-  if (arm || fin) hinge_local_d(M, s, l, p, q);
+  if (arm || fin) hinge_local_d(B, s, p, q);
   {
     double pp[3], pq[4];
 #pragma unroll
@@ -248,7 +271,7 @@
 #pragma unroll
     for (int k = 0; k < 4; k++) pq[k] = dpp_shr1_d(q[k]);
     if (fin) {
-      if (M->body_parent[l] >= GRIP_BODY0) {
+      if (B.parent >= GRIP_BODY0) {
         double t[3], q2[4];
         dq_rot(t, pq, p);
 #pragma unroll
@@ -301,10 +324,10 @@
     for (int k = 0; k < 3; k++) mine.p[k] = (float)wp[k];
 #pragma unroll
     for (int k = 0; k < 9; k++) mine.m[k] = (float)Rm[k];
-    const double jp[3] = {(double)M->jnt_pos[b][0], (double)M->jnt_pos[b][1], (double)M->jnt_pos[b][2]};
-    const double ax[3] = {(double)M->jnt_axis[b][0], (double)M->jnt_axis[b][1], (double)M->jnt_axis[b][2]};
-    const double ip[3] = {(double)M->body_ipos[b][0], (double)M->body_ipos[b][1], (double)M->body_ipos[b][2]};
-    const double iq[4] = {(double)M->body_iquat[b][0], (double)M->body_iquat[b][1], (double)M->body_iquat[b][2], (double)M->body_iquat[b][3]};
+    const double jp[3] = {(double)B.jnt_pos[0], (double)B.jnt_pos[1], (double)B.jnt_pos[2]};
+    const double ax[3] = {(double)B.jnt_axis[0], (double)B.jnt_axis[1], (double)B.jnt_axis[2]};
+    const double ip[3] = {(double)B.ipos[0], (double)B.ipos[1], (double)B.ipos[2]};
+    const double iq[4] = {(double)B.iquat[0], (double)B.iquat[1], (double)B.iquat[2], (double)B.iquat[3]};
 #pragma unroll
     for (int r = 0; r < 3; r++) {
       br.anchor[r] = (float)(wp[r] + Rm[3 * r] * jp[0] + Rm[3 * r + 1] * jp[1] + Rm[3 * r + 2] * jp[2]);
@@ -318,7 +341,7 @@
     (void)t;
   }
   if (l >= NRB && l < NB) {
-    const int qa = M->body_qposadr[b];
+    const int qa = B.qposadr;
     v3copy(mine.p, &s.qpos[qa]);
     for (int k = 0; k < 4; k++) mine.q[k] = s.qpos[qa + 3 + k];
     const float n2 = mine.q[0] * mine.q[0] + mine.q[1] * mine.q[1] + mine.q[2] * mine.q[2] + mine.q[3] * mine.q[3];
@@ -340,39 +363,44 @@
     for (int k = 0; k < 9; k++) s.xmat[b][k] = mine.m[k];
     if (l >= NRB) {
       float tmp[3], qi[4];
-      m3mulv(tmp, mine.m, M->body_ipos[b]);
+      m3mulv(tmp, mine.m, B.ipos);
       v3add(br.xipos, mine.p, tmp);
-      qmul(qi, mine.q, M->body_iquat[b]);
+      qmul(qi, mine.q, B.iquat);
       q2mat(br.ximat, qi);
     }
   }
   MRE_SYNC();
   if (l < NSITE) {
-    const int b = M->site_body[l];
+    const int b = site_b;
     float tmp[3], q[4];
-    m3mulv(tmp, s.xmat[b], M->site_pos[l]);
+    m3mulv(tmp, s.xmat[b], site_pos);
     v3add(s.site_xpos[l], s.xpos[b], tmp);
-    qmul(q, s.xquat[b], M->site_quat[l]);
-    if (l == M->eef_site) q2mat(s.site_xmat[0], q);
-  }
-}
-
-MRE_DEV void com_pos(ModelP M, Sm& s, int l, const BodyRegs& br) {
+    qmul(q, s.xquat[b], site_quat);
+    if (l == eef_site) q2mat(s.site_xmat[0], q);
+  }
+  keep_live(site_b); keep_live(eef_site);
+#pragma unroll
+  for (int k = 0; k < 3; k++) keep_live(site_pos[k]);
+#pragma unroll
+  for (int k = 0; k < 4; k++) keep_live(site_quat[k]);
+}
+
+MRE_DEV void com_pos(ModelP M, Sm& s, int l, const BodyRegs& br, const BodyK& B, float robot_mass) {
   const bool robot = (l >= 1 && l < NRB);
   float mass = 0.f;
-  if (l < NB) mass = (M->body_propid[l] >= 0) ? s.prop_mass[M->body_propid[l]] : M->body_mass[l];
+  if (l < NB) mass = (B.propid >= 0) ? s.prop_mass[B.propid] : B.mass;
   float c0 = robot ? mass * br.xipos[0] : 0.f;
   float c1 = robot ? mass * br.xipos[1] : 0.f;
   float c2 = robot ? mass * br.xipos[2] : 0.f;
   wave_sum3(c0, c1, c2);
-  const float inv = 1.0f / M->robot_mass;
+  const float inv = 1.0f / robot_mass;
   float com[3] = {c0 * inv, c1 * inv, c2 * inv};
   if (l == 0) v3copy(s.com_robot, com);
   if (l >= 1 && l < NB) {
-    const int b = l, pid = M->body_propid[b];
+    const int b = l, pid = B.propid;
     if (pid >= 0) v3copy(com, br.xipos);
     float inertia[3];
-    if (pid >= 0) v3copy(inertia, s.prop_inertia[pid]); else v3copy(inertia, M->body_inertia[b]);
+    if (pid >= 0) v3copy(inertia, s.prop_inertia[pid]); else v3copy(inertia, B.inertia);
     float dif[3], tmp[9];
     v3sub(dif, br.xipos, com);
     const float* mat = br.ximat;
@@ -390,7 +418,7 @@
     ci[4] = tmp[2] - mass * dif[0] * dif[2];
     ci[5] = tmp[5] - mass * dif[1] * dif[2];
     ci[6] = mass * dif[0]; ci[7] = mass * dif[1]; ci[8] = mass * dif[2]; ci[9] = mass;
-    const int da = M->body_dofadr[b];
+    const int da = B.dofadr;
     float off[3];
     v3sub(off, com, br.anchor);
     if (pid < 0) {
@@ -404,15 +432,18 @@
 MRE_PHASE_FN void position_stage(ModelP M, Sm& s, int l) {
   MRE_DBG_T0();
   BodyRegs br;
-  kinematics<true>(M, s, l, br);
+  const BodyK B = load_body(M, l < NB ? l : 0);
+  const float robot_mass = M->opt_rec.robot_mass;
+  kinematics<true>(M, s, l, br, B);
   MRE_DBG_STAMP(5, 0);
-  com_pos(M, s, l, br);
+  com_pos(M, s, l, br, B, robot_mass);
   MRE_SYNC();
   MRE_DBG_STAMP(5, 1);
 }
 MRE_PHASE_FN void kinematics_only(ModelP M, Sm& s, int l) {
   BodyRegs br;
-  kinematics<false>(M, s, l, br);
+  const BodyK B = load_body(M, l < NB ? l : 0);
+  kinematics<false>(M, s, l, br, B);
   MRE_SYNC();
 }
 
@@ -426,9 +457,9 @@
   }
 }
 
-MRE_DEV void inert_about_d(ModelP M, int c, const double* p, const double* q, const double* O, double* ci) {
-  double ip[3] = {(double)M->body_ipos[c][0], (double)M->body_ipos[c][1], (double)M->body_ipos[c][2]}, t[3], qi[4];
-  double iq[4] = {(double)M->body_iquat[c][0], (double)M->body_iquat[c][1], (double)M->body_iquat[c][2], (double)M->body_iquat[c][3]};
+MRE_DEV void inert_about_d(const BodyK& B, const double* p, const double* q, const double* O, double* ci) {
+  double ip[3] = {(double)B.ipos[0], (double)B.ipos[1], (double)B.ipos[2]}, t[3], qi[4];
+  double iq[4] = {(double)B.iquat[0], (double)B.iquat[1], (double)B.iquat[2], (double)B.iquat[3]};
   dq_rot(t, q, ip);
   const double d[3] = {p[0] + t[0] - O[0], p[1] + t[1] - O[1], p[2] + t[2] - O[2]};
   dq_mul(qi, q, iq);
@@ -439,8 +470,8 @@
     R[3] = 2 * (x * y + w * z); R[4] = w * w - x * x + y * y - z * z; R[5] = 2 * (y * z - w * x);
     R[6] = 2 * (x * z - w * y); R[7] = 2 * (y * z + w * x); R[8] = w * w - x * x - y * y + z * z;
   }
-  const double m = (double)M->body_mass[c];
-  const double in[3] = {(double)M->body_inertia[c][0], (double)M->body_inertia[c][1], (double)M->body_inertia[c][2]};
+  const double m = (double)B.mass;
+  const double in[3] = {(double)B.inertia[0], (double)B.inertia[1], (double)B.inertia[2]};
   double T[9];
   for (int r = 0; r < 3; r++)
     for (int k = 0; k < 3; k++)
@@ -457,24 +488,25 @@
 MRE_PHASE_FN void gripper_local(ModelP M, Sm& s, int l) {
   const bool fin = l >= GRIP_BODY0 && l < NRB;
   const int b = fin ? l : GRIP_BODY0;
+  const BodyK B = load_body(M, b);
+  const float tcp[3] = {M->opt_rec.tcp_pos[0], M->opt_rec.tcp_pos[1], M->opt_rec.tcp_pos[2]};
   const double* pose = s.gpose[b - GRIP_BODY0];
   const double p[3] = {pose[0], pose[1], pose[2]}, q[4] = {pose[3], pose[4], pose[5], pose[6]};
-  const int ts = M->tcp_site;
-  const double O[3] = {(double)M->site_pos[ts][0], (double)M->site_pos[ts][1], (double)M->site_pos[ts][2]};
+  const double O[3] = {(double)tcp[0], (double)tcp[1], (double)tcp[2]};
   double ci[10] = {0, 0, 0, 0, 0, 0, 0, 0, 0, 0};
-  if (fin) inert_about_d(M, b, p, q, O, ci);
+  if (fin) inert_about_d(B, p, q, O, ci);
   double up[10];
 #pragma unroll
   for (int k = 0; k < 10; k++) up[k] = dpp_shl1_d(ci[k]);
   if (fin) {
 #pragma unroll
     for (int k = 0; k < 10; k++) s.gI[b - GRIP_BODY0][k] = ci[k];
-    if (M->body_parent[b] < GRIP_BODY0 && b + 1 < NRB && M->body_parent[b + 1] == b) {
+    if (B.parent < GRIP_BODY0 && (b & 1) == 0) {
 #pragma unroll
       for (int k = 0; k < 10; k++) ci[k] += up[k];
     }
-    double ax[3] = {(double)M->jnt_axis[b][0], (double)M->jnt_axis[b][1], (double)M->jnt_axis[b][2]};
-    double jp[3] = {(double)M->jnt_pos[b][0], (double)M->jnt_pos[b][1], (double)M->jnt_pos[b][2]};
+    double ax[3] = {(double)B.jnt_axis[0], (double)B.jnt_axis[1], (double)B.jnt_axis[2]};
+    double jp[3] = {(double)B.jnt_pos[0], (double)B.jnt_pos[1], (double)B.jnt_pos[2]};
     double u[3], a[3];
     dq_rot(u, q, ax);
     dq_rot(a, q, jp);
@@ -492,21 +524,29 @@
   MRE_SYNC();
 }
 
-MRE_DEV void connect_side_d(ModelP M, const Sm& s, int b, const float* a, double sign, double* x,
+struct HingeK { float ax[3], jp[3]; };
+MRE_DEV HingeK load_hinge(ModelP M, int b) {
+  const auto* R = &M->body_rec[b];
+  HingeK H;
+#pragma unroll
+  for (int k = 0; k < 3; k++) { H.ax[k] = R->jnt_axis[k]; H.jp[k] = R->jnt_pos[k]; }
+  return H;
+}
+MRE_DEV void connect_side_d(const Sm& s, int b, int par, const HingeK (&H)[2], const float* a, double sign, double* x,
                             double (*vec)[3]) {
   const double* pose = s.gpose[b - GRIP_BODY0];
   const double al[3] = {(double)a[0], (double)a[1], (double)a[2]};
   double t[3];
   dq_rot(t, pose + 3, al);
   for (int k = 0; k < 3; k++) x[k] = pose[k] + t[k];
-  const int par = M->body_parent[b];
+#pragma unroll
   for (int m = 0; m < 2; m++) {
     vec[m][0] = vec[m][1] = vec[m][2] = 0.0;
     const int c = m == 0 ? b : par;
     if (c < GRIP_BODY0) break;
     const double* cp = s.gpose[c - GRIP_BODY0];
-    const double ax[3] = {(double)M->jnt_axis[c][0], (double)M->jnt_axis[c][1], (double)M->jnt_axis[c][2]};
-    const double jp[3] = {(double)M->jnt_pos[c][0], (double)M->jnt_pos[c][1], (double)M->jnt_pos[c][2]};
+    const double ax[3] = {(double)H[m].ax[0], (double)H[m].ax[1], (double)H[m].ax[2]};
+    const double jp[3] = {(double)H[m].jp[0], (double)H[m].jp[1], (double)H[m].jp[2]};
     double u[3], ja[3];
     dq_rot(u, cp + 3, ax);
     dq_rot(ja, cp + 3, jp);
@@ -518,10 +558,17 @@
 }
 
 MRE_PHASE_FN void connect_rows_local(ModelP M, Sm& s, int l) {
-  if (l < 2 && M->eq_type[l] == 0) {
+  const auto* E = &M->eq_rec[l < 2 ? l : 0];
+  const int type = E->type, b1 = E->b1, b2 = E->b2, pb1 = E->pb1, pb2 = E->pb2;
+  float data[6];
+#pragma unroll
+  for (int k = 0; k < 6; k++) data[k] = E->data[k];
+  const HingeK H1[2] = {load_hinge(M, b1), load_hinge(M, pb1 >= GRIP_BODY0 ? pb1 : b1)};
+  const HingeK H2[2] = {load_hinge(M, b2), load_hinge(M, pb2 >= GRIP_BODY0 ? pb2 : b2)};
+  if (l < 2 && type == 0) {
     double x1[3], x2[3], v1[2][3], v2[2][3];
-    connect_side_d(M, s, M->eq_obj[l][0], M->eq_data[l], 1.0, x1, v1);
-    connect_side_d(M, s, M->eq_obj[l][1], M->eq_data[l] + 3, -1.0, x2, v2);
+    connect_side_d(s, b1, pb1, H1, data, 1.0, x1, v1);
+    connect_side_d(s, b2, pb2, H2, data + 3, -1.0, x2, v2);
     float* o = &s.qfrc_con[16 * l];
     for (int k = 0; k < 3; k++) {
       o[k] = (float)(x1[k] - x2[k]);
@@ -584,6 +631,7 @@
 }
 
 MRE_DEV void crb_mass_matrix(ModelP M, Sm& s, int l) {
+  const int tcp_site = M->opt_rec.tcp_site;
   {
     float acc[10];
 #pragma unroll
@@ -596,7 +644,9 @@
   }
   MRE_SYNC();
   for (int e = l; e < NMR; e += 64) {
-    const int i = M->M_i[e], j = M->M_j[e];
+    const auto* R = &M->m_rec[e];
+    const int i = R->i, j = R->j;
+    const float armature = R->armature;
     float v;
     if (i >= GRIP_BODY0 - 1) {
       const int root = GRIP_BODY0 - 1;
@@ -605,7 +655,7 @@
         for (int k = 0; k < 6; k++) cj[k] = s.gC[j - (GRIP_BODY0 - 1)][k];
       } else {
         float off[3], t[3], lin[3];
-        v3sub(off, s.site_xpos[M->tcp_site], s.com_robot);
+        v3sub(off, s.site_xpos[tcp_site], s.com_robot);
         v3cross(t, s.cdof[j], off);
         v3add(lin, s.cdof[j] + 3, t);
         m3tmulv(cj, s.xmat[root], s.cdof[j]);
@@ -614,10 +664,10 @@
       v = dot6(cj, s.gP[i - (GRIP_BODY0 - 1)]);
     } else {
       float buf[6];
-      mul_inert_vec(buf, s.crb[M->dof_body[i]], s.cdof[i]);
+      mul_inert_vec(buf, s.crb[i + 1], s.cdof[i]);
       v = dot6(s.cdof[j], buf);
     }
-    if (i == j) v += M->dof_armature[i];
+    if (i == j) v += armature;
     s.qM[e] = v;
   }
 }
@@ -751,6 +801,9 @@
 MRE_PHASE_FN void velocity_stage(ModelP M, Sm& s, int l) {
   constexpr int LINK7 = GRIP_BODY0 - 1;
   const bool rob = l >= 1 && l < NRB;
+  const auto* DR = &M->dof_rec[l < NV ? l : 0];
+  const int dof_b = DR->body, dof_pid = DR->propid, dof_da = DR->dofadr;
+  const float grav[3] = {M->opt_rec.gravity[0], M->opt_rec.gravity[1], M->opt_rec.gravity[2]};
   float cd[6] = {0.f, 0.f, 0.f, 0.f, 0.f, 0.f}, qv = 0.f;
   if (rob) {
 #pragma unroll
@@ -780,7 +833,7 @@
     const int b = l;
 #pragma unroll
     for (int t = 0; t < 6; t++) { cv[t] = 0.f; ca[t] = 0.f; }
-    const int da = M->body_dofadr[b];
+    const int da = NRV + 6 * (b - NRB);
 #pragma unroll
     for (int j = 0; j < 3; j++) cv[3 + j] += s.qvel[da + j];
     float cdot[3][6];
@@ -802,7 +855,7 @@
   float f[6] = {0.f, 0.f, 0.f, 0.f, 0.f, 0.f};
   if (l >= 1 && l < NB) {
     const int b = l;
-    ca[3] -= M->gravity[0]; ca[4] -= M->gravity[1]; ca[5] -= M->gravity[2];
+    ca[3] -= grav[0]; ca[4] -= grav[1]; ca[5] -= grav[2];
     if (l == LINK7) {
 #pragma unroll
       for (int t = 0; t < 6; t++) { s.scratch[t] = cv[t]; s.scratch[6 + t] = ca[t]; }
@@ -824,7 +877,7 @@
   for (int t = 0; t < 6; t++) tot[t] = dpp_row<0x101>(f[t]);
   MRE_SYNC();
   if (l < NV) {
-    const int b = M->dof_body[l];
+    const int b = dof_b;
     float c6[6];
     if (b < NRB) {
 #pragma unroll
@@ -832,9 +885,9 @@
     } else {
 #pragma unroll
       for (int t = 0; t < 6; t++) tot[t] = s.cfrc[b][t];
-      prop_cdof(s, b, l - M->body_dofadr[b], c6);
-    }
-    const bool act = body_is_active(M, s, b);
+      prop_cdof(s, b, l - dof_da, c6);
+    }
+    const bool act = prop_is_active(s, dof_pid);
     s.qfrc_bias[l] = act ? dot6(c6, tot) : 0.f;
   }
 }
@@ -869,11 +922,12 @@
   constexpr int LINK7 = GRIP_BODY0 - 1;
   const bool fin = l >= GRIP_BODY0 && l < NRB;
   const int i = fin ? l - GRIP_BODY0 : 0;
+  const int tcp_site = M->opt_rec.tcp_site;
   double V7[6], A7[6];
   {
     const float* R = s.xmat[LINK7];
     float r[3];
-    v3sub(r, s.site_xpos[M->tcp_site], s.com_robot);
+    v3sub(r, s.site_xpos[tcp_site], s.com_robot);
     const double rd[3] = {(double)r[0], (double)r[1], (double)r[2]};
     for (int h = 0; h < 2; h++) {
       const float* c = &s.scratch[6 * h];
@@ -894,7 +948,7 @@
 #pragma unroll
   for (int k = 0; k < 10; k++) I[k] = fin ? s.gI[i][k] : 0.0;
   const double qd = fin ? robot_v(s, l - 1) : 0.0;
-  const bool child = fin && M->body_parent[l] >= GRIP_BODY0;
+  const bool child = fin && (l & 1) != 0;
   double v[6], a0[6], sd[6];
   dcross_motion(sd, V7, S);
 #pragma unroll
@@ -931,12 +985,16 @@
 
 MRE_PHASE_FN unsigned arm_actuation(ModelP M, Sm& s, int l) {
   bool arm_clamped = false;
+  const auto* R = &M->dof_rec[l < 7 ? l : 0];
+  const float gain = R->act_gain, bias0 = R->act_bias0, bias1 = R->act_bias1, bias2 = R->act_bias2;
+  const float ctrl_lo = R->act_ctrl_lo, ctrl_hi = R->act_ctrl_hi, force_lo = R->act_force_lo, force_hi = R->act_force_hi;
+  const int forcelimited = R->act_forcelimited;
   if (l < 7) {
-    float fa = (float)((double)(M->act_gain[l] * clampf(s.ctrl[l], M->act_ctrlrange[l][0], M->act_ctrlrange[l][1]) + M->act_bias[l][0]) +
-                       (double)M->act_bias[l][1] * robot_q(s, l) + (double)M->act_bias[l][2] * robot_v(s, l));
-    if (M->act_forcelimited[l]) {
-      if (fa <= M->act_forcerange[l][0]) { fa = M->act_forcerange[l][0]; arm_clamped = true; }
-      if (fa >= M->act_forcerange[l][1]) { fa = M->act_forcerange[l][1]; arm_clamped = true; }
+    float fa = (float)((double)(gain * clampf(s.ctrl[l], ctrl_lo, ctrl_hi) + bias0) +
+                       (double)bias1 * robot_q(s, l) + (double)bias2 * robot_v(s, l));
+    if (forcelimited) {
+      if (fa <= force_lo) { fa = force_lo; arm_clamped = true; }
+      if (fa >= force_hi) { fa = force_hi; arm_clamped = true; }
     }
     s.qfrc_smooth[l] = fa;
   }
@@ -944,25 +1002,34 @@
 }
 
 MRE_PHASE_FN unsigned smooth_forces_assemble(ModelP M, Sm& s, int l, unsigned arm_mask) {
-  const double ten_len = (double)M->ten_coef[0] * robot_q(s, M->ten_dof[0]) + (double)M->ten_coef[1] * robot_q(s, M->ten_dof[1]);
-  const double ten_vel = (double)M->ten_coef[0] * robot_v(s, M->ten_dof[0]) + (double)M->ten_coef[1] * robot_v(s, M->ten_dof[1]);
-  const float cg = clampf(s.ctrl[NU - 1], M->act_ctrlrange[NU - 1][0], M->act_ctrlrange[NU - 1][1]);
-  float fg = (float)((double)(M->grip_gainprm * cg + M->grip_biasprm[0]) + (double)M->grip_biasprm[1] * ten_len +
-                     (double)M->grip_biasprm[2] * ten_vel);
+  const auto* O = &M->opt_rec;
+  const float ten_coef[2] = {O->ten_coef[0], O->ten_coef[1]};
+  const int ten_dof[2] = {O->ten_dof[0], O->ten_dof[1]};
+  const float grip_gainprm = O->grip_gainprm, grip_biasprm[3] = {O->grip_biasprm[0], O->grip_biasprm[1], O->grip_biasprm[2]};
+  const float grip_forcerange[2] = {O->grip_forcerange[0], O->grip_forcerange[1]};
+  const float grip_ctrlrange[2] = {O->grip_ctrlrange[0], O->grip_ctrlrange[1]};
+  const auto* DR = &M->dof_rec[l < NV ? l : 0];
+  const int dof_b = DR->body, dof_pid = DR->propid;
+  const float dof_damping = DR->damping, dof_stiffness = DR->jnt_stiffness, dof_springref = DR->jnt_springref;
+  const double ten_len = (double)ten_coef[0] * robot_q(s, ten_dof[0]) + (double)ten_coef[1] * robot_q(s, ten_dof[1]);
+  const double ten_vel = (double)ten_coef[0] * robot_v(s, ten_dof[0]) + (double)ten_coef[1] * robot_v(s, ten_dof[1]);
+  const float cg = clampf(s.ctrl[NU - 1], grip_ctrlrange[0], grip_ctrlrange[1]);
+  float fg = (float)((double)(grip_gainprm * cg + grip_biasprm[0]) + (double)grip_biasprm[1] * ten_len +
+                     (double)grip_biasprm[2] * ten_vel);
   bool clamped = false;
-  if (fg <= M->grip_forcerange[0]) { fg = M->grip_forcerange[0]; clamped = true; }
-  if (fg >= M->grip_forcerange[1]) { fg = M->grip_forcerange[1]; clamped = true; }
+  if (fg <= grip_forcerange[0]) { fg = grip_forcerange[0]; clamped = true; }
+  if (fg >= grip_forcerange[1]) { fg = grip_forcerange[1]; clamped = true; }
   if (l < NV) {
-    const int b = M->dof_body[l];
+    const int b = dof_b;
     float f = 0.f;
     if (b < NRB) {
-      double fd = -(double)M->jnt_stiffness[b] * (robot_q(s, l) - (double)M->jnt_springref[b]) - (double)M->dof_damping[l] * robot_v(s, l);
+      double fd = -(double)dof_stiffness * (robot_q(s, l) - (double)dof_springref) - (double)dof_damping * robot_v(s, l);
       if (l < 7) fd += (double)s.qfrc_smooth[l];
-      if (l == M->ten_dof[0]) fd += (double)M->ten_coef[0] * (double)fg;
-      if (l == M->ten_dof[1]) fd += (double)M->ten_coef[1] * (double)fg;
+      if (l == ten_dof[0]) fd += (double)ten_coef[0] * (double)fg;
+      if (l == ten_dof[1]) fd += (double)ten_coef[1] * (double)fg;
       f = (float)(fd - (double)s.qfrc_bias[l]);
     }
-    const bool act = body_is_active(M, s, b);
+    const bool act = prop_is_active(s, dof_pid);
     f = act ? (b < NRB ? f : f - s.qfrc_bias[l]) : 0.f;
     s.qfrc_smooth[l] = f;
     s.qacc_smooth[l] = f;
@@ -989,21 +1056,22 @@
 
 MRE_PHASE_FN void integrate_setup(ModelP M, Sm& s, int l, unsigned act_clamped) {
   const bool grip_clamped = (act_clamped >> (NU - 1)) & 1u;
-  const float h = M->timestep;
+  const float h = M->opt_rec.timestep, grip_bias2 = M->opt_rec.grip_biasprm[2];
   for (int e = l; e < NMR; e += 64) {
+    const auto* R = &M->m_rec[e];
+    const int i = R->i, j = R->j, ten = R->ten;
+    const float damping = R->damping, act_bias2 = R->act_bias2, ten_coef = R->ten_coef;
     float v = s.qM[e];
-    const int i = M->M_i[e];
-    if (i == M->M_j[e]) {
-      v += h * M->dof_damping[i];
-      if (i < 7 && ((act_clamped >> i) & 1u) == 0u) v -= h * M->act_bias[i][2];
+    if (i == j) {
+      v += h * damping;
+      if (i < 7 && ((act_clamped >> i) & 1u) == 0u) v -= h * act_bias2;
       if (!grip_clamped) {
-        if (i == M->ten_dof[0]) v -= h * M->grip_biasprm[2] * M->ten_coef[0] * M->ten_coef[0];
-        if (i == M->ten_dof[1]) v -= h * M->grip_biasprm[2] * M->ten_coef[1] * M->ten_coef[1];
+        if (ten >= 0) v -= h * grip_bias2 * ten_coef * ten_coef;
       }
     }
     mh_store(s)[e] = v;
 #ifdef MRE_NEWTON
-    if (i == M->M_j[e]) s.scratch[i] = (s.qM[e] - v) * s.qacc[i];
+    if (i == j) s.scratch[i] = (s.qM[e] - v) * s.qacc[i];
 #endif
   }
 #ifndef MRE_NEWTON
@@ -1013,10 +1081,23 @@
 }
 
 MRE_PHASE_FN void integrate(ModelP M, Sm& s, int l, unsigned flags, bool polished, float* clo) {
-  const float h = M->timestep;
+  const float h = M->opt_rec.timestep;
+  const auto* DR = &M->dof_rec[l < NV ? l : 0];
+  const int dof_b = DR->body, dof_pid = DR->propid;
+  const auto* BR = &M->body_rec[l < NB ? l : 0];
+  const int body_qa = BR->qposadr, body_da = BR->dofadr, body_pid = BR->propid;
   const bool freeze = (flags & F_FREEZE_ROBOT) != 0;
+  float vl_in = 0.f, ql_in[7] = {0.f, 0.f, 0.f, 0.f, 0.f, 0.f, 0.f};
+  if (clo != nullptr) {
+    if (l >= NRV && l < NV) vl_in = clo[(QFINE_CUBE_V - QFINE_CUBE_Q) + (l - NRV)];
+    if (l >= NRB && l < NB) {
+#pragma unroll
+      for (int k = 0; k < 7; k++) ql_in[k] = clo[7 * (l - NRB) + k];
+    }
+  }
+  keep_live(dof_pid); keep_live(body_pid); keep_live(body_qa); keep_live(body_da);
   if (l < NV) {
-    const int b = M->dof_body[l];
+    const int b = dof_b;
     if (b < NRB) {
       if (!freeze) {
 #ifdef MRE_NEWTON
@@ -1028,10 +1109,10 @@
         const float hi = (float)v;
         s.qvel[l] = hi; s.qlo[QFINE / 2 + l] = (float)(v - (double)hi);
       }
-    } else if (body_is_active(M, s, b)) {
+    } else if (prop_is_active(s, dof_pid)) {
       if (clo != nullptr) {
         float* const vl = clo + (QFINE_CUBE_V - QFINE_CUBE_Q) + (l - NRV);
-        const double v = (double)s.qvel[l] + (double)*vl + (double)h * (double)s.qacc[l];
+        const double v = (double)s.qvel[l] + (double)vl_in + (double)h * (double)s.qacc[l];
         const float hi = (float)v, lo = (float)(v - (double)hi);
         s.qvel[l] = hi; *vl = lo;
         s.scratch[l] = lo;
@@ -1042,24 +1123,24 @@
   }
   MRE_SYNC();
   if (l >= 1 && l < NB) {
-    const int b = l, qa = M->body_qposadr[b], da = M->body_dofadr[b];
+    const int b = l, qa = body_qa, da = body_da;
     if (b < NRB) {
       if (!freeze) {
         const double q = robot_q(s, qa) + (double)h * robot_v(s, da);
         const float hi = (float)q;
         s.qpos[qa] = hi; s.qlo[qa] = (float)(q - (double)hi);
       }
-    } else if (body_is_active(M, s, b) && clo != nullptr) {
+    } else if (prop_is_active(s, body_pid) && clo != nullptr) {
       float* const ql = clo + 7 * (b - NRB);
       double vv[6];
       for (int k = 0; k < 6; k++) vv[k] = (double)s.qvel[da + k] + (double)s.scratch[da + k];
       for (int k = 0; k < 3; k++) {
-        const double x = (double)s.qpos[qa + k] + (double)ql[k] + (double)h * vv[k];
+        const double x = (double)s.qpos[qa + k] + (double)ql_in[k] + (double)h * vv[k];
         const float hi = (float)x;
         s.qpos[qa + k] = hi; ql[k] = (float)(x - (double)hi);
       }
       double q0[4], qn[4];
-      for (int k = 0; k < 4; k++) q0[k] = (double)s.qpos[qa + 3 + k] + (double)ql[3 + k];
+      for (int k = 0; k < 4; k++) q0[k] = (double)s.qpos[qa + 3 + k] + (double)ql_in[3 + k];
       const double wn2 = vv[3] * vv[3] + vv[4] * vv[4] + vv[5] * vv[5];
       if (wn2 > 1e-60) {
         const double inv = rsq64(wn2), half = 0.5 * (double)h * wn2 * inv;
@@ -1080,7 +1161,7 @@
         const float hi = (float)x;
         s.qpos[qa + 3 + k] = hi; ql[3 + k] = (float)(x - (double)hi);
       }
-    } else if (body_is_active(M, s, b)) {
+    } else if (prop_is_active(s, body_pid)) {
       for (int k = 0; k < 3; k++) s.qpos[qa + k] += h * s.qvel[da + k];
       float w[3] = {s.qvel[da + 3], s.qvel[da + 4], s.qvel[da + 5]};
       const float ang = v3normalize(w) * h;
diff --git a/mujoco_robot_environments_amd/csrc/mre_math.h b/mujoco_robot_environments_amd/csrc/mre_math.h
--- a/mujoco_robot_environments_amd/csrc/mre_math.h
+++ b/mujoco_robot_environments_amd/csrc/mre_math.h
@@ -29,6 +29,9 @@
 namespace mre {
 
 constexpr float kMinVal = 1e-15f;
+
+MRE_DEV void keep_live(float x) { asm volatile("" ::"v"(x)); }
+MRE_DEV void keep_live(int x) { asm volatile("" ::"v"(x)); }
 
 MRE_DEV void v3copy(float* r, const float* a) { r[0] = a[0]; r[1] = a[1]; r[2] = a[2]; }
 MRE_DEV void v3zero(float* r) { r[0] = r[1] = r[2] = 0.f; }
diff --git a/mujoco_robot_environments_amd/csrc/mre_solver.h b/mujoco_robot_environments_amd/csrc/mre_solver.h
--- a/mujoco_robot_environments_amd/csrc/mre_solver.h
+++ b/mujoco_robot_environments_amd/csrc/mre_solver.h
@@ -287,11 +287,15 @@
 
 MRE_PHASE_FN void assemble_constraints(ModelP M, Sm& s, int l) {
   int lim = 0, lim_side = 0;
-  if (l >= 1 && l < NRB && M->jnt_limited[l]) {
+  const auto* BR = &M->body_rec[l < NRB ? l : 0];
+  const int jnt_limited = BR->jnt_limited;
+  const float jnt_range[2] = {BR->jnt_range[0], BR->jnt_range[1]};
+  if (l >= 1 && l < NRB && jnt_limited) {
     const double q = robot_q(s, l - 1);
-    if (q - (double)M->jnt_range[l][0] < 0.0) { lim = 1; lim_side = -1; }
-    else if ((double)M->jnt_range[l][1] - q < 0.0) { lim = 1; lim_side = 1; }
-  }
+    if (q - (double)jnt_range[0] < 0.0) { lim = 1; lim_side = -1; }
+    else if ((double)jnt_range[1] - q < 0.0) { lim = 1; lim_side = 1; }
+  }
+  keep_live(jnt_range[0]); keep_live(jnt_range[1]);
   const unsigned long long limm = __ballot(lim != 0);
   const int lim_idx = __popcll(limm & ((1ull << l) - 1ull));
   if (l == 0) s.nl = __popcll(limm);
@@ -354,65 +358,82 @@
   for (int i = l; i < nefc; i += 64) {
     int rs = HDR_NONE, pa = 0xF, pb = 0xF;
     float pos = 0.f, margin = 0.f, diag = 0.f, imp_pos = 0.f;
-    const float *solref, *solimp;
     bool fric_row = false;
     float R0scale = 1.0f;
+    const int eqi = i < 6 ? i / 3 : 2;
+    const int limb = (i >= 7 && i < 7 + nl) ? (s.lim_info[i - 7] & 0xFF) : 0;
+    const int rrec = i < 7 ? eqi : (i < 7 + nl ? ROWREC_JNT + limb : ROWREC_PAIR + s.con_pair[(i - 7 - nl) / 3]);
+    const auto* RR = &M->row_rec[rrec];
+    const float solref[2] = {RR->solref[0], RR->solref[1]};
+    const float solimp[5] = {RR->solimp[0], RR->solimp[1], RR->solimp[2], RR->solimp[3], RR->solimp[4]};
+    const float rec_margin = RR->margin, rec_gap = RR->gap, rec_friction = RR->friction, invw1 = RR->invw1, invw2 = RR->invw2;
+    const float lim_range[2] = {M->body_rec[limb].jnt_range[0], M->body_rec[limb].jnt_range[1]};
+    const float opt_timestep = M->opt_rec.timestep, opt_impratio = M->opt_rec.impratio;
+    const int opt_cone = M->opt_rec.cone;
     if (i < 7) {
       rs = i;
-      const int e = i < 6 ? i / 3 : 2;
-      solref = M->eq_solref[e]; solimp = M->eq_solimp[e];
+      const int e = eqi;
+      const auto* E = &M->eq_rec[e];
+      const int b1 = E->b1, b2 = E->b2;
+      const int root = E->root, pb1 = E->pb1, pb2 = E->pb2;
+      const float pc[5] = {E->data[0], E->data[1], E->data[2], E->data[3], E->data[4]};
+      const float q0_1 = E->qpos0_1, q0_2 = E->qpos0_2;
+      const int nchain = E->root_chain_len;
+      int chain[MAXCHAIN];
+#pragma unroll
+      for (int c = 0; c < MAXCHAIN; c++) chain[c] = E->root_chain[c];
       if (e < 2) {
-        const int b1 = M->eq_obj[e][0], b2 = M->eq_obj[e][1], k = i % 3;
-        int root = b1;
-        while (root >= GRIP0) root = M->body_parent[root];
+        const int k = i % 3;
         const float* loc = &s.qfrc_con[16 * e];
         const float* R = s.xmat[root];
         float cp[3];
         m3mulv(cp, R, loc);
         const float rk[3] = {R[3 * k], R[3 * k + 1], R[3 * k + 2]};
-        const int pb1 = M->body_parent[b1], pb2 = M->body_parent[b2];
         s.Jr[rs][b1 - 1] += v3dot(rk, loc + 4);
         if (pb1 >= GRIP0) s.Jr[rs][pb1 - 1] += v3dot(rk, loc + 7);
         s.Jr[rs][b2 - 1] += v3dot(rk, loc + 10);
         if (pb2 >= GRIP0) s.Jr[rs][pb2 - 1] += v3dot(rk, loc + 13);
         {
-          const int n = M->chain_len[root];
-          for (int c = 0; c < n; c++) {
-            const int j = M->chain_dof[root][c];
-            float t[3];
-            v3cross(t, s.cdof[j], cp);
-            s.Jr[rs][j] += sel3(t, k);
+#pragma unroll
+          for (int c = 0; c < MAXCHAIN; c++) {
+            if (c < nchain) {
+              const int j = chain[c];
+              float t[3];
+              v3cross(t, s.cdof[j], cp);
+              s.Jr[rs][j] += sel3(t, k);
+            }
           }
         }
         pos = sel3(cp, k);
         imp_pos = v3norm(cp);
-        diag = M->body_invweight0[b1][0] + M->body_invweight0[b2][0];
+        diag = invw1 + invw2;
       } else {
-        const int b1 = M->eq_obj[e][0], b2 = M->eq_obj[e][1];
         const int d1 = b1 - 1, d2 = b2 - 1;
-        const float* pc = M->eq_data[e];
-        const double dif64 = robot_q(s, d2) - (double)M->qpos0[d2];
-        pos = (float)(robot_q(s, d1) - (double)M->qpos0[d1] -
+        const double dif64 = robot_q(s, d2) - (double)q0_2;
+        pos = (float)(robot_q(s, d1) - (double)q0_1 -
                       ((double)pc[0] + dif64 * ((double)pc[1] + dif64 * ((double)pc[2] + dif64 * ((double)pc[3] + dif64 * (double)pc[4])))));
         const float dif = (float)dif64;
         const float deriv = pc[1] + dif * (2.f * pc[2] + dif * (3.f * pc[3] + dif * 4.f * pc[4]));
         s.Jr[rs][d1] += 1.f;
         s.Jr[rs][d2] -= deriv;
         imp_pos = pos;
-        diag = M->dof_invweight0[d1] + M->dof_invweight0[d2];
-      }
+        diag = invw1 + invw2;
+      }
+      keep_live(root); keep_live(pb1); keep_live(pb2); keep_live(nchain); keep_live(q0_1); keep_live(q0_2);
+#pragma unroll
+      for (int c = 0; c < 5; c++) keep_live(pc[c]);
+#pragma unroll
+      for (int c = 0; c < MAXCHAIN; c++) keep_live(chain[c]);
     } else if (i < 7 + nl) {
       rs = i;
       const int info = s.lim_info[i - 7], b = info & 0xFF, hi = (info >> 8) & 1;
       const double q = robot_q(s, b - 1);
-      pos = (float)(hi ? ((double)M->jnt_range[b][1] - q) : (q - (double)M->jnt_range[b][0]));
+      pos = (float)(hi ? ((double)lim_range[1] - q) : (q - (double)lim_range[0]));
       s.Jr[rs][b - 1] = hi ? -1.f : 1.f;
       imp_pos = pos;
-      diag = M->dof_invweight0[b - 1];
-      solref = M->jnt_solref[b]; solimp = M->jnt_solimp[b];
+      diag = invw1;
     } else {
       const int c = (i - 7 - nl) / 3, r = (i - 7 - nl) % 3;
-      const int pr = s.con_pair[c];
       const int b1 = s.con_b1[c], b2 = s.con_b2[c];
       const float* ax = &s.con_frame[c][3 * r];
       const float* p = s.con_pos[c];
@@ -421,11 +442,11 @@
       int slot = 0;
       float dg = 0.f;
       if (b1 > 0) {
-        if (b1 < NRB) { jac_robot(M, s, rs, b1, p, ax, -1.f); dg += M->body_invweight0[b1][0]; }
+        if (b1 < NRB) { jac_robot(M, s, rs, b1, p, ax, -1.f); dg += invw1; }
         else { pa = b1 - NRB; jac_prop(s, i, slot++, b1, p, ax, -1.f); dg += 1.0f / s.prop_mass[pa]; }
       }
       if (b2 > 0) {
-        if (b2 < NRB) { jac_robot(M, s, rs, b2, p, ax, 1.f); dg += M->body_invweight0[b2][0]; }
+        if (b2 < NRB) { jac_robot(M, s, rs, b2, p, ax, 1.f); dg += invw2; }
         else {
           const int pid = b2 - NRB;
           if (slot == 0) pa = pid; else pb = pid;
@@ -434,42 +455,43 @@
         }
       }
       diag = dg;
-      solref = M->pair_solref[pr]; solimp = M->pair_solimp[pr];
-      margin = M->pair_margin[pr] - M->pair_gap[pr];
+      margin = rec_margin - rec_gap;
       imp_pos = s.con_dist[c];
       if (r == 0) pos = s.con_dist[c];
       else {
         fric_row = true;
         pos = 0.f;
-        R0scale = 1.0f / fmaxf(M->impratio, kMinVal);
-      }
-      if (M->cone == 0) {
-        const float fr = M->pair_friction[pr][0];
+        R0scale = 1.0f / fmaxf(opt_impratio, kMinVal);
+      }
+      if (opt_cone == 0) {
+        const float fr = rec_friction;
         diag = dg * (1.f + fr * fr);
-        R0scale = 2.f * fr * fr / fmaxf(M->impratio, kMinVal);
-      }
-    }
+        R0scale = 2.f * fr * fr / fmaxf(opt_impratio, kMinVal);
+      }
+    }
+    keep_live(lim_range[0]); keep_live(lim_range[1]); keep_live(invw1); keep_live(invw2); keep_live(rec_friction);
+    keep_live(rec_margin); keep_live(rec_gap); keep_live(opt_impratio); keep_live(opt_cone);
     s.hdr[i] = rs | (pa << 8) | (pb << 12);
     const float imp = impedance(solimp, imp_pos, margin);
     float tc = solref[0];
     const float dr = solref[1], dmax = clampf(solimp[1], 0.0001f, 0.9999f);
     float K, B;
     if (tc > 0.f) {
-      tc = fmaxf(tc, 2.f * M->timestep);
+      tc = fmaxf(tc, 2.f * opt_timestep);
       K = 1.0f / (dmax * dmax * tc * tc * dr * dr);
       B = 2.0f / (dmax * tc);
     } else { K = -tc / (dmax * dmax); B = -dr / dmax; }
     if (fric_row) K = 0.f;
     float R = fmaxf((1.f - imp) * diag / imp, kMinVal) * R0scale;
-    if (M->cone == 0) R = fmaxf(R, kMinVal);
+    if (opt_cone == 0) R = fmaxf(R, kMinVal);
     const float vel = row_dot(s, i, s.qvel);
     const float efc_margin = fric_row ? 0.f : margin;
     const float aref = -B * vel - K * imp * (pos - efc_margin);
     rowR(s, i) = R; rowB(s, i) = aref;
 #ifdef MRE_NEWTON
-    if (i >= 7 + nl && (i - 7 - nl) % 3 == 0) s.con_fric[(i - 7 - nl) / 3] = M->pair_friction[s.con_pair[(i - 7 - nl) / 3]][0];
+    if (i >= 7 + nl && (i - 7 - nl) % 3 == 0) s.con_fric[(i - 7 - nl) / 3] = rec_friction;
 #else
-    if (i >= 7 + nl && (i - 7 - nl) % 3 == 0) s.blkrec[8 + (i - 7 - nl) / 3][15] = M->pair_friction[s.con_pair[(i - 7 - nl) / 3]][0];
+    if (i >= 7 + nl && (i - 7 - nl) % 3 == 0) s.blkrec[8 + (i - 7 - nl) / 3][15] = rec_friction;
 #endif
   }
   MRE_SYNC();
```
